# jkulhanek/viewformer

Measured on AMD Instinct MI355X. Metric: novel views/sec (encode->AR transformer->decode), 128px 6-ctx, higher is better.
Workload: dtype bf16

## Files before the change

### include/vf_hip.h

```cpp
#ifndef VF_HIP_H
#define VF_HIP_H

#include <stddef.h>
#include <stdint.h>

#ifdef __cplusplus
extern "C" {
#endif

#define VF_OK 0
#define VF_ERR_BAD_ARG (-1)
#define VF_ERR_UNSUPPORTED (-2)

int vf_abi_version(void);
size_t vf_sizeof_igemm_args(void);
size_t vf_sizeof_pack_desc(void);
const char* vf_build_arch(void);
int vf_build_flags(void);
const char* vf_build_flag_name(int i);
enum { VF_SEL_ATTN_DMA = 0,
       VF_SEL_GEMM_G256 = 1,
       VF_SEL_LN_BWD_TWO_ROWS = 2,
       VF_SEL_ATTN_Q32 = 3,
       VF_SEL_CONV_X3H_K32 = 4,
       VF_SEL_GEMM_TAIL = 5,
       VF_SEL_COUNT = 6 };
int vf_select(int which, int value);
int vf_selected(int which);

enum { VF_MODE_GEMM = 0, VF_MODE_CONV3_S1 = 1, VF_MODE_CONV3_S2PAD = 2, VF_MODE_CONV3_UP2 = 3 };
enum { VF_EPI_NONE = 0, VF_EPI_GELU_ERF = 1,
       VF_EPI_GELU_BWD = 2,
       VF_EPI_GELU_DUAL = 3 };

typedef struct vf_igemm_args {
    const float* x;
    const float* w_packed;
    const float* bias;
    const float* res;
    float* out;
    const float* pro_mean;
    const float* pro_scale;
    const float* pro_beta;
    int32_t pro_swish;
    int32_t pro_rows_per_img;
    int32_t mode;
    int32_t epilogue;
    int32_t M;
    int32_t Cin, Cout;
    int32_t Hin, Win, Hout, Wout;
    int32_t lda, ldc, ldr;
    int32_t batch;
    int64_t stride_x, stride_w, stride_out, stride_res;
    float* gn_part;
    int32_t gn_slots;
    int32_t reserved0;
    void* out_aux;
    float drop_rate;
    uint32_t drop_seed, drop_site;
    int32_t drop_row0;
} vf_igemm_args;

size_t vf_igemm_packed_floats(int K, int N, int taps);
int vf_igemm_pack_f32(const float* src, float* dst, int K, int N, int taps,
                      int64_t sk, int64_t sn, int64_t st, int batch, int64_t src_bstride, void* stream);
int vf_igemm_f32(const vf_igemm_args* args , void* stream);

int vf_conv_in_u8_f32(const uint8_t* img_u8, const float* img_f32, const float* w_oihw, const float* bias,
                      float* out, int n_img, int H, int W, int Cout, void* stream);
size_t vf_conv_in_x3h_packed_elems(int Cout);
int vf_conv_in_x3h_pack(const float* w_oihw, void* dst, int Cout, void* stream);
int vf_conv_in_x3h(const uint8_t* img_u8, const float* img_f32, const void* w_packed, const float* bias, float* out, float* gn_part,
                   int gn_slots, int n_img, int H, int W, int Cout, void* stream);

int vf_conv3_small_cout_f32(const float* x, const float* w_oihw, const float* bias, const float* pro_mean,
                            const float* pro_scale, const float* pro_beta, int pro_swish, float* out, int n_img, int H, int W,
                            int Cin, int Cout, int x_bf16, void* stream);

size_t vf_groupnorm_workspace_bytes(int n_img, int HW, int C);
int vf_groupnorm_stats_f32(const float* x, const float* gamma, int n_img, int HW, int C, int groups, float eps,
                           float* mean_c, float* scale_c, void* ws, void* stream);
int vf_groupnorm_finalize_f32(const float* part, const float* gamma, int n_img, int HW, int C, int groups, int nslots,
                              float eps, float* mean_c, float* scale_c, void* stream);
int vf_groupnorm_apply_f32(const float* x, const float* mean_c, const float* scale_c, const float* beta,
                           float* out, int n_img, int HW, int C, int swish, void* stream);

size_t vf_vq_packed_floats(int D, int Kc);
int vf_vq_pack_codebook_f32(const float* E , float* dst, int D, int Kc, void* stream);
int vf_colsumsq_f32(const float* E , float* e_sq , int D, int Kc, void* stream);
int vf_vq_argmin_f32(const float* z, const float* E_packed, const float* e_sq, int64_t M, int D, int Kc,
                     int64_t* idx, void* stream);
size_t vf_vq_filter_packed_bytes(int D, int Kc);
int vf_vq_filter_pack(const float* E , void* dst, int D, int Kc, void* stream);
int vf_vq_argmin_filtered_f32(const float* z, const void* packed, int64_t M, int D, int Kc, int64_t* idx, uint32_t* stats4,
                              void* stream);
int vf_codebook_gather_f32(const float* E , const int64_t* idx, float* out ,
                           int64_t M, int D, int Kc, void* stream);

int vf_attn_blockcausal_f32(const float* q, const float* k, const float* v, float* out,
                            int B, int H, int T, int L, int ldq, int ldk, int ldv, int ldo,
                            float scale, int skip_masked, int twin_view, void* stream);
int vf_attn_blockcausal_bf16_v2(const void* q, const void* k, const void* v, int in_bf16, void* out, int out_bf16, int B, int H, int T, int L,
                                int ldq, int ldk, int ldv, int ldo, float scale, int skip_masked, int twin_view, void* stream);
int vf_attn_blockcausal_fp8(const void* q, const void* k, const void* v, int in_bf16, void* out, int out_bf16, int B, int H, int T, int L,
                            int ldq, int ldk, int ldv, int ldo, float scale, int skip_masked, int twin_view, void* stream);
int vf_attn_blockcausal_x6(const float* q, const float* k, const float* v, float* out,
                           int B, int H, int T, int L, int ldq, int ldk, int ldv, int ldo,
                           float scale, int skip_masked, int twin_view, void* stream);
int vf_attn_prefix_bf16(const void* q, const void* k, const void* v, const void* kp, const void* vp, int in_bf16, void* out, int out_bf16,
                        int B, int H, int C, int N, int L, int dh, int ldq, int ldk, int ldv, int ldkp, int ldvp, int64_t prefix_stride,
                        int ldo, void* stream);
int vf_attn_prefix_f32eq(const float* q, const float* k, const float* v, const float* kp, const float* vp, float* out,
                         int B, int H, int C, int N, int L, int dh, int ldq, int ldk, int ldv, int ldkp, int ldvp, int64_t prefix_stride,
                         int ldo, void* stream);
int vf_attn_spatial_f32(const float* qkv, float* out, int n_img, int HW, int C, int64_t ld, int64_t ldo, float scale, void* stream);
int vf_attn_spatial_x3h(const float* qkv, float* out, int n_img, int HW, int C, int64_t ld, int64_t ldo, float scale, void* stream);
int vf_softmax_rows_f32(float* x, int64_t rows, int n, float scale, void* stream);

int vf_layernorm_f32(const float* x, const float* gamma, const float* beta, float* out,
                     int64_t rows, int d, float eps, void* stream);
int vf_layernorm_bf16out_f32(const float* x, const float* gamma, const float* beta, void* out_bf16, int64_t rows, int d, float eps,
                             void* stream);
int vf_embed_sum_f32(const int32_t* ids, const float* wte, const float* wpe, const float* add,
                     float* out, int64_t BS, int L, int d, int vocab, void* stream);
int vf_dense_small_k_gelu_f32(const float* x, const float* W, const float* b, float* out,
                              int64_t rows, int K, int N, int gelu, void* stream);
int vf_argmax_rows_f32(const float* x, int64_t rows, int n, int ld, int64_t* idx, void* stream);
int vf_lmhead_argmax_bf16(const void* h, int h_bf16, int64_t ldh, const void* w_packed, int64_t M, int K, int N, int64_t* idx,
                          float* max_logit, void* stream);
uint32_t vf_crc32c(const void* data, size_t n, uint32_t crc);
int vf_postprocess_u8(const float* x, uint8_t* out, int64_t n, void* stream);
int vf_resize_u8(const uint8_t* src, uint8_t* dst, int n_img, int Hin, int Win, int Hout, int Wout, int C, int bilinear, void* stream);
size_t vf_image_metrics_workspace_bytes(int n_img, int H, int W, int C);
int vf_image_metrics_u8(const uint8_t* a, const uint8_t* b, int n_img, int H, int W, int C, int64_t* sums, double* ssim, void* workspace,
                        void* stream);
size_t vf_camera_knn_workspace_bytes(int64_t N, int Q, int k);
int vf_camera_knn_f32(const float* db, int64_t N, const float* queries, int Q, int k, float pos_weight, int32_t* idx, float* dist,
                      void* workspace, void* stream);

size_t vf_gemm_bf16_packed_elems(int K, int N);
int vf_gemm_bf16_pack(const float* src, void* dst, int K, int N, int64_t sk, int64_t sn, int batch,
                      int64_t src_bstride, void* stream);
typedef struct vf_pack_desc {
    const float* src;
    void* dst;
    int32_t K, N;
    int64_t sk, sn;
} vf_pack_desc;
int vf_gemm_bf16_pack_multi(const vf_pack_desc* descs_device, int n, void* stream);
int vf_gemm_bf16(const vf_igemm_args* args , void* stream);
size_t vf_conv3_bf16_packed_elems(int Cin, int Cout);
int vf_conv3_bf16_pack(const float* w_oihw, void* dst, int Cin, int Cout, void* stream);
int vf_conv3_halo_bf16(const vf_igemm_args* args , void* stream);

int vf_conv3_halo_gn_slots(int Hout, int Wout);
size_t vf_conv3_x6_packed_elems(int Cin, int Cout);
int vf_conv3_x6_pack(const float* w_oihw, void* dst, int Cin, int Cout, void* stream);
int vf_conv3_halo_x6(const vf_igemm_args* args , void* stream);
size_t vf_conv3_x3h_packed_elems(int Cin, int Cout);
int vf_conv3_x3h_pack(const float* w_oihw, void* dst, int Cin, int Cout, void* stream);
int vf_conv3_halo_x3h(const vf_igemm_args* args , void* stream);
size_t vf_gemm_x3h_packed_elems(int K, int N);
int vf_gemm_x3h_pack(const float* src, void* dst, int K, int N, int64_t sk, int64_t sn, void* stream);
int vf_gemm_x3h(const vf_igemm_args* args , void* stream);
size_t vf_gemm_x6_packed_elems(int K, int N);
int vf_gemm_x6_pack(const float* src, void* dst, int K, int N, int64_t sk, int64_t sn, void* stream);
int vf_gemm_x6(const vf_igemm_args* args , void* stream);
int vf_sum_slabs_f32(const float* slabs, int nslabs, int64_t stride, int64_t n, float* dst, int accumulate, void* stream);

int vf_vq_ema_accumulate_f32(const float* z, const int64_t* idx, int64_t M, int D, int Kc, float* counts, float* embed_sum,
                             void* stream);
int vf_vq_ema_update_f32(const float* counts, const float* embed_sum, float* cluster_size_hidden, float* dw_hidden,
                         float* embeddings, int D, int Kc, float decay, float eps, float corr, void* stream);

int vf_gather_transpose_f32(const float* src, float* dst, int n_img, int Hin, int Win, int C, int Hout, int Wout, int stride, int oy,
                            int ox, int64_t ld_dst, void* stream);
size_t vf_conv3_wgrad_x6_rows(int Cin);
int vf_conv3_wgrad_x6(const float* x, const void* dy_packed, float* slabs, int n_img, int Hin, int Win, int Cin, int Hout, int Wout,
                      int Cout, int mode, int splits, void* stream);
int vf_upsample2_bwd_f32(const float* du, float* dx, int n_img, int H, int W, int C, void* stream);
size_t vf_groupnorm_bwd_workspace_bytes(int n_img, int HW, int C, int groups);
int vf_groupnorm_bwd_f32(const float* x, const float* da, const float* mean_c, const float* scale_c, const float* gamma,
                         const float* beta, float* dx, float* chan_sums, int n_img, int HW, int C, int groups, int swish,
                         int accumulate, void* ws, void* stream);
int vf_softmax_rows_bwd_f32(const float* p, float* dp, int64_t rows, int n, float scale, void* stream);
int vf_l1_loss_partials(int64_t n);
int vf_l1_loss_f32(const float* x, const float* y, float* dy, float* part, int64_t n, float grad_weight, void* stream);

int vf_lpips_scaling_f32(const float* x, float* y, int64_t npix, const float* shift3, const float* scale3, int backward, void* stream);
int vf_relu_f32(float* x, int64_t n, void* stream);
int vf_relu_bwd_f32(float* dy, const float* y, int64_t n, void* stream);
int vf_maxpool2_f32(const float* x, float* y, int n_img, int Hout, int Wout, int C, void* stream);
int vf_maxpool2_bwd_f32(const float* x, const float* dy, float* dx, int n_img, int Hout, int Wout, int C, void* stream);
int vf_lpips_head_blocks(int HW);
int vf_lpips_head_f32(const float* f0, const float* f1, const float* w, float* part, int n_img, int HW, int C, void* stream);
int vf_lpips_head_bwd_f32(const float* f0, const float* f1, const float* w, float* df1, int64_t npix, int C, float gscale,
                          int accumulate, void* stream);

int vf_attn_blockcausal_lse_f32(const float* q, const float* k, const float* v, float* out, float* lse,
                                int B, int H, int T, int L, int ldq, int ldk, int ldv, int ldo,
                                float scale, int skip_masked, int twin_view, float drop_rate, uint32_t drop_seed,
                                uint32_t drop_site, uint32_t drop_plane0, void* stream);
int vf_attn_bwd_prep_f32(const float* dout, const float* out, float* D, int B, int H, int T, int lddo, int ldo, void* stream);
int vf_attn_bwd_f32(const float* q, const float* k, const float* v, const float* dout, const float* lse, const float* D,
                    float* dq, float* dk, float* dv, int B, int H, int T, int L, int ldq, int ldk, int ldv, int lddo,
                    int lddq, int lddk, int lddv, float scale, int twin_view, float drop_rate, uint32_t drop_seed,
                    uint32_t drop_site, uint32_t drop_plane0, void* stream);
int vf_gemm_tn_bf16(const void* x_bf16, int ldx, const void* dy, int dy_is_bf16, int ldy, int M, int K, int N, int splits, float* w_slabs,
                    float* b_slabs, int64_t slab_stride, void* stream);
int vf_attn_blockcausal_bf16_lse(const void* q, const void* k, const void* v, void* out, float* lse, int B, int H, int T, int L,
                                 int ldq, int ldk, int ldv, int ldo, float scale, int twin_view, float drop_rate, uint32_t drop_seed,
                                 uint32_t drop_site, uint32_t drop_plane0, void* stream);
int vf_attn_bwd_prep_bf16(const void* dout, const void* out, float* D, int B, int H, int T, int lddo, int ldo, void* stream);
int vf_attn_bwd_bf16(const void* q, const void* k, const void* v, const void* dout, const float* lse, const float* D, void* dq, void* dk,
                     void* dv, int out_bf16 , int B, int H, int T, int L,
                     int ldq, int ldk, int ldv, int lddo, int lddq, int lddk, int lddv, float scale, int twin_view, float drop_rate,
                     uint32_t drop_seed, uint32_t drop_site, uint32_t drop_plane0, void* stream);
int vf_dropout_add_f32(const float* x, const float* res, float* out, int64_t rows, int cols, int64_t row0, float rate, uint32_t seed, uint32_t site,
                       void* stream);

int vf_transpose_f32(const float* src, float* dst, int rows, int cols, int64_t ld_src, int64_t ld_dst, int batch,
                     int64_t bs_src, int64_t bs_dst, void* stream);
int vf_transpose_bf16_f32(const void* src_bf16, float* dst, int rows, int cols, int64_t ld_src, int64_t ld_dst, int batch,
                          int64_t bs_src, int64_t bs_dst, void* stream);
size_t vf_colsum_workspace_bytes(int N);
int vf_colsum_f32(const float* x, float* out, int64_t M, int N, int64_t ld, int accumulate, void* ws, void* stream);
size_t vf_layernorm_bwd_workspace_bytes(int64_t rows, int d);
int vf_layernorm_bwd_f32(const float* dy, const float* x, const float* gamma, float* dx, float* dgamma, float* dbeta,
                         int64_t rows, int d, float eps, int accumulate, const float* res ,
                         void* dx_bf16 ,
                         float drop_rate, uint32_t drop_seed, uint32_t drop_site, int64_t drop_row0 , void* ws, void* stream);
int vf_gelu_f32(const float* u, float* f, int64_t n, void* stream);
int vf_gelu_bf16out_f32(const float* u, void* f_bf16, int64_t n, void* stream);
int vf_gelu_bwd_f32(const float* u, const float* df, float* du, int64_t n, void* stream);
int vf_gelu_bwd_bf16out_f32(const float* u, const float* df, void* du_bf16, int64_t n, void* stream);
int vf_softmax_mask_f32(float* s, int64_t batch, int T, int L, int mask_spec, float scale, void* stream);
int vf_softmax_mask_bwd_f32(const float* p, float* dp, int64_t batch, int T, int L, int mask_spec, float scale, void* stream);
int vf_softmax_ce_f32(const float* logits, const int32_t* target, const float* row_weight, float* loss, float* dlogits,
                      int64_t rows, int V, float label_smoothing, void* stream);
int vf_pose_mse_f32(const float* raw, const float* gt, const float* w_pos, const float* w_ori, const float* xyz_div, float* pos_loss,
                    float* ori_loss, float* draw, int64_t rows, int L, float position_multiplier, void* stream);
size_t vf_embed_bwd_workspace_bytes(int d, int vocab);
int vf_embed_bwd_f32(const float* dh, const int32_t* ids, float* dwte, float* dwpe, float* dadd, int64_t BS, int L, int d,
                     int vocab, void* workspace, void* stream);
int vf_dense_small_k_bwd_f32(const float* x, const float* dy, float* dW, float* db, int64_t rows, int K, int N, void* stream);
int vf_dense_small_n_f32(const float* x, const float* W, const float* b, float* out, int64_t rows, int K, int N, int64_t ldx, void* stream);
int vf_dense_small_n_wgrad_slabs(int64_t rows);
int vf_dense_small_n_wgrad_f32(const float* x, const float* dy, float* dW, float* ws, int64_t rows, int K, int N, int64_t ldx, int accumulate,
                               void* stream);
int vf_adamw_f32(float* param, const float* grad, float* m, float* v, int64_t n, float lr_decay, float lr_adam, float beta1,
                 float beta2, float eps, void* stream);
int vf_adamw_flat_f32(float* param, const float* grad, float* m, float* v, int64_t n, const int64_t* nodecay_ranges, int nranges,
                      float lr_decay, float lr_adam, float beta1, float beta2, float eps, void* stream);
typedef struct vf_adamw_pack_desc {
    int64_t offset;
    void* dst_kn;
    void* dst_nk;
    int32_t rows, cols;
    int32_t nodecay;
    int32_t reserved;
} vf_adamw_pack_desc;
size_t vf_sizeof_adamw_pack_desc(void);
int vf_adamw_pack_check(const vf_adamw_pack_desc* descs_host, int ndesc, int64_t n);
int vf_adamw_flat_pack_f32(float* param, const float* grad, float* m, float* v, int64_t n, const int64_t* nodecay_ranges, int nranges,
                           float lr_decay, float lr_adam, float beta1, float beta2, float eps, const vf_adamw_pack_desc* descs_device, int ndesc,
                           void* stream);
int vf_add_inplace_f32(float* a, const float* b, int64_t n, void* stream);
int vf_axpby_f32(float a, const float* x, float b, const float* y, float* out, int64_t n, void* stream);
int vf_clip_by_norm_f32(float* x, int64_t n, float clip, float* scratch1, void* stream);
int vf_clip_grad_norm_f32(float* x, int64_t n, float max_norm, float* scratch1, void* stream);

#ifdef __cplusplus
}
#endif
#endif
```

### viewformer_amd/_lib.py

```python
import ctypes
import os
from ctypes import c_int, c_int32, c_int64, c_float, c_void_p, c_size_t, c_char_p, POINTER

HERE = os.path.dirname(os.path.abspath(__file__))
LIB_PATH = os.environ.get('VF_HIP_LIB') or os.path.join(HERE, 'libvf_hip.so')


class VfIgemmArgs(ctypes.Structure):
    _fields_ = [
        ('x', c_void_p), ('w_packed', c_void_p), ('bias', c_void_p), ('res', c_void_p), ('out', c_void_p),
        ('pro_mean', c_void_p), ('pro_scale', c_void_p), ('pro_beta', c_void_p),
        ('pro_swish', c_int32), ('pro_rows_per_img', c_int32), ('mode', c_int32), ('epilogue', c_int32),
        ('M', c_int32), ('Cin', c_int32), ('Cout', c_int32),
        ('Hin', c_int32), ('Win', c_int32), ('Hout', c_int32), ('Wout', c_int32),
        ('lda', c_int32), ('ldc', c_int32), ('ldr', c_int32), ('batch', c_int32),
        ('stride_x', c_int64), ('stride_w', c_int64), ('stride_out', c_int64), ('stride_res', c_int64),
        ('gn_part', c_void_p), ('gn_slots', c_int32), ('reserved0', c_int32),
        ('out_aux', c_void_p),
        ('drop_rate', c_float), ('drop_seed', ctypes.c_uint32), ('drop_site', ctypes.c_uint32), ('drop_row0', c_int32),
    ]


SEL_ATTN_DMA, SEL_GEMM_G256, SEL_LN_BWD_TWO_ROWS, SEL_ATTN_Q32 = 0, 1, 2, 3
SEL_CONV_X3H_K32 = 4
SEL_GEMM_TAIL = 5
_ENV_SELECT = {'VF_ATTN_DMA': SEL_ATTN_DMA, 'VF_GEMM_G256': SEL_GEMM_G256, 'VF_LN_BWD_TWO_ROWS': SEL_LN_BWD_TWO_ROWS, 'VF_ATTN_Q32': SEL_ATTN_Q32,
               'VF_CONV_X3H_K32': SEL_CONV_X3H_K32, 'VF_GEMM_TAIL': SEL_GEMM_TAIL}

ADAMW_PACK_DESC_BYTES = 40
PACK_DESC_BYTES = 40
P = c_void_p
EXPORTS = {
    'vf_abi_version': (c_int, []),
    'vf_sizeof_igemm_args': (c_size_t, []),
    'vf_sizeof_pack_desc': (c_size_t, []),
    'vf_build_arch': (c_char_p, []),
    'vf_build_flags': (c_int, []),
    'vf_build_flag_name': (c_char_p, [c_int]),
    'vf_select': (c_int, [c_int, c_int]),
    'vf_selected': (c_int, [c_int]),
    'vf_igemm_packed_floats': (c_size_t, [c_int, c_int, c_int]),
    'vf_igemm_pack_f32': (c_int, [P, P, c_int, c_int, c_int, c_int64, c_int64, c_int64, c_int, c_int64, P]),
    'vf_igemm_f32': (c_int, [POINTER(VfIgemmArgs), P]),
    'vf_conv_in_u8_f32': (c_int, [P, P, P, P, P, c_int, c_int, c_int, c_int, P]),
    'vf_conv_in_x3h_packed_elems': (c_size_t, [c_int]),
    'vf_conv_in_x3h_pack': (c_int, [P, P, c_int, P]),
    'vf_conv_in_x3h': (c_int, [P, P, P, P, P, P, c_int, c_int, c_int, c_int, c_int, P]),
    'vf_crc32c': (ctypes.c_uint32, [P, c_size_t, ctypes.c_uint32]),
    'vf_conv3_small_cout_f32': (c_int, [P, P, P, P, P, P, c_int, P, c_int, c_int, c_int, c_int, c_int, c_int, P]),
    'vf_groupnorm_workspace_bytes': (c_size_t, [c_int, c_int, c_int]),
    'vf_groupnorm_stats_f32': (c_int, [P, P, c_int, c_int, c_int, c_int, c_float, P, P, P, P]),
    'vf_groupnorm_finalize_f32': (c_int, [P, P, c_int, c_int, c_int, c_int, c_int, c_float, P, P, P]),
    'vf_conv3_halo_gn_slots': (c_int, [c_int, c_int]),
    'vf_groupnorm_apply_f32': (c_int, [P, P, P, P, P, c_int, c_int, c_int, c_int, P]),
    'vf_vq_packed_floats': (c_size_t, [c_int, c_int]),
    'vf_vq_pack_codebook_f32': (c_int, [P, P, c_int, c_int, P]),
    'vf_colsumsq_f32': (c_int, [P, P, c_int, c_int, P]),
    'vf_vq_argmin_f32': (c_int, [P, P, P, c_int64, c_int, c_int, P, P]),
    'vf_vq_filter_packed_bytes': (c_size_t, [c_int, c_int]),
    'vf_vq_filter_pack': (c_int, [P, P, c_int, c_int, P]),
    'vf_vq_argmin_filtered_f32': (c_int, [P, P, c_int64, c_int, c_int, P, P, P]),
    'vf_gather_transpose_f32': (c_int, [P, P, c_int, c_int, c_int, c_int, c_int, c_int, c_int, c_int, c_int, c_int64, P]),
    'vf_upsample2_bwd_f32': (c_int, [P, P, c_int, c_int, c_int, c_int, P]),
    'vf_groupnorm_bwd_workspace_bytes': (c_size_t, [c_int, c_int, c_int, c_int]),
    'vf_groupnorm_bwd_f32': (c_int, [P, P, P, P, P, P, P, P, c_int, c_int, c_int, c_int, c_int, c_int, P, P]),
    'vf_softmax_rows_bwd_f32': (c_int, [P, P, c_int64, c_int, c_float, P]),
    'vf_l1_loss_partials': (c_int, [c_int64]),
    'vf_l1_loss_f32': (c_int, [P, P, P, P, c_int64, c_float, P]),
    'vf_conv3_wgrad_x6_rows': (c_size_t, [c_int]),
    'vf_conv3_wgrad_x6': (c_int, [P, P, P, c_int, c_int, c_int, c_int, c_int, c_int, c_int, c_int, c_int, P]),
    'vf_lpips_scaling_f32': (c_int, [P, P, c_int64, P, P, c_int, P]),
    'vf_relu_f32': (c_int, [P, c_int64, P]),
    'vf_relu_bwd_f32': (c_int, [P, P, c_int64, P]),
    'vf_maxpool2_f32': (c_int, [P, P, c_int, c_int, c_int, c_int, P]),
    'vf_maxpool2_bwd_f32': (c_int, [P, P, P, c_int, c_int, c_int, c_int, P]),
    'vf_lpips_head_blocks': (c_int, [c_int]),
    'vf_lpips_head_f32': (c_int, [P, P, P, P, c_int, c_int, c_int, P]),
    'vf_lpips_head_bwd_f32': (c_int, [P, P, P, P, c_int64, c_int, c_float, c_int, P]),
    'vf_vq_ema_accumulate_f32': (c_int, [P, P, c_int64, c_int, c_int, P, P, P]),
    'vf_vq_ema_update_f32': (c_int, [P, P, P, P, P, c_int, c_int, c_float, c_float, c_float, P]),
    'vf_codebook_gather_f32': (c_int, [P, P, P, c_int64, c_int, c_int, P]),
    'vf_attn_blockcausal_f32': (c_int, [P, P, P, P, c_int, c_int, c_int, c_int, c_int, c_int, c_int, c_int,
                                        c_float, c_int, c_int, P]),
    'vf_attn_blockcausal_bf16_v2': (c_int, [P, P, P, c_int, P, c_int] + [c_int] * 8 + [c_float, c_int, c_int, P]),
    'vf_attn_blockcausal_fp8': (c_int, [P, P, P, c_int, P, c_int] + [c_int] * 8 + [c_float, c_int, c_int, P]),
    'vf_attn_blockcausal_x6': (c_int, [P, P, P, P, c_int, c_int, c_int, c_int, c_int, c_int, c_int, c_int,
                                       c_float, c_int, c_int, P]),
    'vf_attn_prefix_bf16': (c_int, [P, P, P, P, P, c_int, P, c_int] + [c_int] * 11 + [c_int64, c_int, P]),
    'vf_attn_prefix_f32eq': (c_int, [P, P, P, P, P, P] + [c_int] * 11 + [c_int64, c_int, P]),
    'vf_attn_blockcausal_lse_f32': (c_int, [P, P, P, P, P, c_int, c_int, c_int, c_int, c_int, c_int, c_int, c_int,
                                            c_float, c_int, c_int, c_float, ctypes.c_uint32, ctypes.c_uint32, ctypes.c_uint32, P]),
    'vf_dropout_add_f32': (c_int, [P, P, P, c_int64, c_int, c_int64, c_float, ctypes.c_uint32, ctypes.c_uint32, P]),
    'vf_attn_bwd_prep_f32': (c_int, [P, P, P, c_int, c_int, c_int, c_int, c_int, P]),
    'vf_attn_bwd_f32': (c_int, [P, P, P, P, P, P, P, P, P, c_int, c_int, c_int, c_int, c_int, c_int, c_int, c_int, c_int,
                                c_int, c_int, c_float, c_int, c_float, ctypes.c_uint32, ctypes.c_uint32, ctypes.c_uint32, P]),
    'vf_gemm_tn_bf16': (c_int, [P, c_int, P, c_int, c_int, c_int, c_int, c_int, c_int, P, P, c_int64, P]),
    'vf_attn_blockcausal_bf16_lse': (c_int, [P, P, P, P, P, c_int, c_int, c_int, c_int, c_int, c_int, c_int, c_int, c_float, c_int,
                                             c_float, ctypes.c_uint32, ctypes.c_uint32, ctypes.c_uint32, P]),
    'vf_attn_bwd_prep_bf16': (c_int, [P, P, P, c_int, c_int, c_int, c_int, c_int, P]),
    'vf_attn_bwd_bf16': (c_int, [P, P, P, P, P, P, P, P, P, c_int, c_int, c_int, c_int, c_int, c_int, c_int, c_int, c_int, c_int, c_int, c_int,
                                 c_float, c_int, c_float, ctypes.c_uint32, ctypes.c_uint32, ctypes.c_uint32, P]),
    'vf_attn_spatial_f32': (c_int, [P, P, c_int, c_int, c_int, c_int64, c_int64, c_float, P]),
    'vf_attn_spatial_x3h': (c_int, [P, P, c_int, c_int, c_int, c_int64, c_int64, c_float, P]),
    'vf_softmax_rows_f32': (c_int, [P, c_int64, c_int, c_float, P]),
    'vf_layernorm_f32': (c_int, [P, P, P, P, c_int64, c_int, c_float, P]),
    'vf_layernorm_bf16out_f32': (c_int, [P, P, P, P, c_int64, c_int, c_float, P]),
    'vf_embed_sum_f32': (c_int, [P, P, P, P, P, c_int64, c_int, c_int, c_int, P]),
    'vf_dense_small_k_gelu_f32': (c_int, [P, P, P, P, c_int64, c_int, c_int, c_int, P]),
    'vf_lmhead_argmax_bf16': (c_int, [P, c_int, c_int64, P, c_int64, c_int, c_int, P, P, P]),
    'vf_argmax_rows_f32': (c_int, [P, c_int64, c_int, c_int, P, P]),
    'vf_postprocess_u8': (c_int, [P, P, c_int64, P]),
    'vf_resize_u8': (c_int, [P, P, c_int, c_int, c_int, c_int, c_int, c_int, c_int, P]),
    'vf_image_metrics_workspace_bytes': (c_size_t, [c_int, c_int, c_int, c_int]),
    'vf_image_metrics_u8': (c_int, [P, P, c_int, c_int, c_int, c_int, P, P, P, P]),
    'vf_camera_knn_workspace_bytes': (c_size_t, [c_int64, c_int, c_int]),
    'vf_camera_knn_f32': (c_int, [P, c_int64, P, c_int, c_int, c_float, P, P, P, P]),
    'vf_gemm_bf16_packed_elems': (c_size_t, [c_int, c_int]),
    'vf_gemm_bf16_pack': (c_int, [P, P, c_int, c_int, c_int64, c_int64, c_int, c_int64, P]),
    'vf_gemm_bf16_pack_multi': (c_int, [P, c_int, P]),
    'vf_gemm_bf16': (c_int, [POINTER(VfIgemmArgs), P]),
    'vf_conv3_bf16_packed_elems': (c_size_t, [c_int, c_int]),
    'vf_conv3_bf16_pack': (c_int, [P, P, c_int, c_int, P]),
    'vf_conv3_halo_bf16': (c_int, [POINTER(VfIgemmArgs), P]),
    'vf_conv3_x6_packed_elems': (c_size_t, [c_int, c_int]),
    'vf_conv3_x6_pack': (c_int, [P, P, c_int, c_int, P]),
    'vf_conv3_halo_x6': (c_int, [POINTER(VfIgemmArgs), P]),
    'vf_conv3_x3h_packed_elems': (c_size_t, [c_int, c_int]),
    'vf_conv3_x3h_pack': (c_int, [P, P, c_int, c_int, P]),
    'vf_conv3_halo_x3h': (c_int, [POINTER(VfIgemmArgs), P]),
    'vf_gemm_x3h_packed_elems': (c_size_t, [c_int, c_int]),
    'vf_gemm_x3h_pack': (c_int, [P, P, c_int, c_int, c_int64, c_int64, P]),
    'vf_gemm_x3h': (c_int, [POINTER(VfIgemmArgs), P]),
    'vf_gemm_x6_packed_elems': (c_size_t, [c_int, c_int]),
    'vf_gemm_x6_pack': (c_int, [P, P, c_int, c_int, c_int64, c_int64, P]),
    'vf_gemm_x6': (c_int, [POINTER(VfIgemmArgs), P]),
    'vf_sum_slabs_f32': (c_int, [P, c_int, c_int64, c_int64, P, c_int, P]),
    'vf_transpose_f32': (c_int, [P, P, c_int, c_int, c_int64, c_int64, c_int, c_int64, c_int64, P]),
    'vf_transpose_bf16_f32': (c_int, [P, P, c_int, c_int, c_int64, c_int64, c_int, c_int64, c_int64, P]),
    'vf_colsum_workspace_bytes': (c_size_t, [c_int]),
    'vf_colsum_f32': (c_int, [P, P, c_int64, c_int, c_int64, c_int, P, P]),
    'vf_layernorm_bwd_workspace_bytes': (c_size_t, [c_int64, c_int]),
    'vf_layernorm_bwd_f32': (c_int, [P, P, P, P, P, P, c_int64, c_int, c_float, c_int, P, P, c_float, ctypes.c_uint32, ctypes.c_uint32, c_int64, P, P]),
    'vf_gelu_f32': (c_int, [P, P, c_int64, P]),
    'vf_gelu_bf16out_f32': (c_int, [P, P, c_int64, P]),
    'vf_gelu_bwd_bf16out_f32': (c_int, [P, P, P, c_int64, P]),
    'vf_gelu_bwd_f32': (c_int, [P, P, P, c_int64, P]),
    'vf_softmax_mask_f32': (c_int, [P, c_int64, c_int, c_int, c_int, c_float, P]),
    'vf_softmax_mask_bwd_f32': (c_int, [P, P, c_int64, c_int, c_int, c_int, c_float, P]),
    'vf_softmax_ce_f32': (c_int, [P, P, P, P, P, c_int64, c_int, c_float, P]),
    'vf_pose_mse_f32': (c_int, [P, P, P, P, P, P, P, P, c_int64, c_int, c_float, P]),
    'vf_embed_bwd_workspace_bytes': (c_size_t, [c_int, c_int]),
    'vf_embed_bwd_f32': (c_int, [P, P, P, P, P, c_int64, c_int, c_int, c_int, P, P]),
    'vf_dense_small_k_bwd_f32': (c_int, [P, P, P, P, c_int64, c_int, c_int, P]),
    'vf_dense_small_n_f32': (c_int, [P, P, P, P, c_int64, c_int, c_int, c_int64, P]),
    'vf_dense_small_n_wgrad_slabs': (c_int, [c_int64]),
    'vf_dense_small_n_wgrad_f32': (c_int, [P, P, P, P, c_int64, c_int, c_int, c_int64, c_int, P]),
    'vf_adamw_f32': (c_int, [P, P, P, P, c_int64, c_float, c_float, c_float, c_float, c_float, P]),
    'vf_adamw_flat_f32': (c_int, [P, P, P, P, c_int64, P, c_int, c_float, c_float, c_float, c_float, c_float, P]),
    'vf_sizeof_adamw_pack_desc': (c_size_t, []),
    'vf_adamw_pack_check': (c_int, [P, c_int, c_int64]),
    'vf_adamw_flat_pack_f32': (c_int, [P, P, P, P, c_int64, P, c_int, c_float, c_float, c_float, c_float, c_float, P, c_int, P]),
    'vf_axpby_f32': (c_int, [c_float, P, c_float, P, P, c_int64, P]),
    'vf_add_inplace_f32': (c_int, [P, P, c_int64, P]),
    'vf_clip_by_norm_f32': (c_int, [P, c_int64, c_float, P, P]),
    'vf_clip_grad_norm_f32': (c_int, [P, c_int64, c_float, P, P]),
}

_lib = None


class VfError(RuntimeError):
    pass


def _bind(path):
    lib = ctypes.CDLL(path)
    for name, (res, args) in EXPORTS.items():
        fn = getattr(lib, name)
        fn.restype = res
        fn.argtypes = args
    return lib


def load_variant(path):
    return _bind(os.path.abspath(path))


class use:

    def __init__(self, handle):
        self.handle = handle

    def __enter__(self):
        global _lib
        load()
        self.prev, _lib = _lib, self.handle
        return self.handle

    def __exit__(self, *exc):
        global _lib
        _lib = self.prev
        return False


def load():
    global _lib
    if _lib is not None:
        return _lib
    if not os.path.exists(LIB_PATH):
        raise VfError(f'{LIB_PATH} not found — run `python -m viewformer_amd.build` (hipcc --offload-arch=gfx950). '
                      'There is no CPU/PyTorch fallback for the hot path.')
    lib = _bind(LIB_PATH)
    if int(lib.vf_sizeof_igemm_args()) != ctypes.sizeof(VfIgemmArgs):
        raise VfError(f'vf_igemm_args is {int(lib.vf_sizeof_igemm_args())} bytes in {LIB_PATH} and {ctypes.sizeof(VfIgemmArgs)} in '
                      'viewformer_amd/_lib.py: rebuild the library or update the mirror')
    if int(lib.vf_sizeof_pack_desc()) != PACK_DESC_BYTES:
        raise VfError(f'vf_pack_desc is {int(lib.vf_sizeof_pack_desc())} bytes in {LIB_PATH}, {PACK_DESC_BYTES} expected')
    if int(lib.vf_sizeof_adamw_pack_desc()) != ADAMW_PACK_DESC_BYTES:
        raise VfError(f'vf_adamw_pack_desc is {int(lib.vf_sizeof_adamw_pack_desc())} bytes in {LIB_PATH}, {ADAMW_PACK_DESC_BYTES} expected')
    for env, which in _ENV_SELECT.items():
        if os.environ.get(env) in ('0', '1'):
            lib.vf_select(which, int(os.environ[env]))
    _lib = lib
    return lib


def select(which, value):
    prev = load().vf_select(int(which), 1 if value else 0)
    if prev < 0:
        raise VfError(f'vf_select({which}, {value}): bad argument')
    return prev


def check(status: int, what: str):
    if status == 0:
        return
    if status < 0:
        msg = {-1: 'bad argument', -2: 'unsupported shape'}.get(status, 'error')
        raise VfError(f'{what}: {msg} ({status})')
    raise VfError(f'{what}: HIP error {status}')
```

### viewformer_amd/csrc/conv3_halo_x3h.hip

```cpp
#include <type_traits>
#include "halo_common.h"

namespace {

typedef _Float16 f16x8 __attribute__((ext_vector_type(8)));
typedef _Float16 f16x4 __attribute__((ext_vector_type(4)));

typedef unsigned u32x4_t __attribute__((ext_vector_type(4)));
__device__ __forceinline__ f16x8 wbuf_load(__amdgpu_buffer_rsrc_t r, unsigned voff, unsigned soff) {
    return __builtin_bit_cast(f16x8, __builtin_amdgcn_raw_buffer_load_b128(r, voff, soff, 0));
}

constexpr int CK = 32;
constexpr int P_LDB = 144;
constexpr int TH = 8, TW = 16;
constexpr int BN = 128;
constexpr int PLANE_BYTES = 2 * BN * 16;
constexpr int KS_BYTES = 2 * PLANE_BYTES;
constexpr int TAP_BYTES = 2 * KS_BYTES;
constexpr int TAIL_BYTES = 16;

template <bool UP2, bool PAIR = false>
struct Geo {
    static constexpr int PH = UP2 ? (TH / 2 + 2) : (TH + 2);
    static constexpr int PW = PAIR ? 20 : (UP2 ? (TW / 2 + 2) : (TW + 2));
    static constexpr int NPIX = PH * PW;
    static constexpr int SLOTS = (NPIX * 8 + 255) / 256;
    static constexpr int BUF = (NPIX + 1) * P_LDB;
};

__device__ __forceinline__ void split2(float x, _Float16& h, _Float16& l) {
    h = (_Float16)x;
    l = (_Float16)((x - (float)h) * 2048.f);
}

template <bool UP2, bool PRO, bool SWISH, bool PAIR = false>
__global__ __launch_bounds__(256, 2) void conv3_halo_x3h_kernel(vf_igemm_args p) {
    using G = Geo<UP2, PAIR>;
    extern __shared__ __attribute__((aligned(16))) unsigned char smem_h[];

    const int tid = threadIdx.x;
    const int lane = tid & 63;
    const int wave = __builtin_amdgcn_readfirstlane(tid >> 6);
    constexpr int MI = 4, NJ = 1;
    const int wave_m = 0, wave_n = wave;
    const int half = lane >> 5, l31 = lane & 31;

    const int nb = p.Cout / BN;
    const int tilesX = p.Wout / TW, tilesY = p.Hout / TH;
    int bid = (int)vf_xcd_bid();
    const int nblk = bid % nb; bid /= nb;
    int tx = 0, ty = 0, img;
    if (PAIR) { img = bid * 2; }
    else { tx = bid % tilesX; bid /= tilesX; ty = bid % tilesY; img = bid / tilesY; }
    const int n_img_total = p.M / (p.Hout * p.Wout);
    const int img1 = PAIR ? min(img + 1, n_img_total - 1) : img;
    const int pair_pix = (img1 - img) * p.Hin * p.Win;
    const int y0 = ty * TH, x0 = tx * TW;
    const int sy0 = UP2 ? (y0 / 2 - 1) : (y0 - 1);
    const int sx0 = UP2 ? (x0 / 2 - 1) : (x0 - 1);

    const float* __restrict__ X = p.x + (size_t)img * p.Hin * p.Win * p.Cin;
    const int nchunks = p.Cin / CK;
    const int last_stage = nchunks * 9 - 1;

    const int c4 = tid & 7;
    int s_off[G::SLOTS];
    unsigned ok_mask = 0, sel_mask = 0;
    const int lds0 = (tid >> 3) * P_LDB + c4 * 8;
    int lds_last = 0;
#pragma unroll
    for (int q = 0; q < G::SLOTS; ++q) {
        const int pix = (tid >> 3) + 32 * q;
        const int pixc = pix < G::NPIX ? pix : G::NPIX;
        const int pr = pixc / G::PW, pc0 = pixc - pr * G::PW;
        const int sel = PAIR ? (pc0 >= 10) : 0;
        const int pc = pc0 - 10 * sel;
        sel_mask |= (unsigned)sel << q;
        const int sy = sy0 + pr, sx = sx0 + pc;
        const bool ok = pix < G::NPIX && sy >= 0 && sy < p.Hin && sx >= 0 && sx < p.Win;
        ok_mask |= (unsigned)ok << q;
        s_off[q] = ok ? (sel * pair_pix + sy * p.Win + sx) * p.Cin + c4 * 4 : c4 * 4;
        if (q == G::SLOTS - 1) lds_last = pixc * P_LDB + c4 * 8;
    }

    f32x4 preg[G::SLOTS];
    f32x4 pmean, pscale, pbeta, pmean1, pscale1;
    const __amdgpu_buffer_rsrc_t x_rs = __builtin_amdgcn_make_buffer_rsrc(const_cast<float*>(X), 0, 0x7fffffff, 0x00020000);
    auto patch_load = [&](int chunk) {
#pragma unroll
        for (int q = 0; q < G::SLOTS; ++q)
            preg[q] = __builtin_bit_cast(f32x4, __builtin_amdgcn_raw_buffer_load_b128(x_rs, (unsigned)s_off[q] * 4u, (unsigned)(chunk * CK * 4), 0));
        if (PRO) {
            pmean = *reinterpret_cast<const f32x4*>(p.pro_mean + (size_t)img * p.Cin + chunk * CK + c4 * 4);
            pscale = *reinterpret_cast<const f32x4*>(p.pro_scale + (size_t)img * p.Cin + chunk * CK + c4 * 4);
            pbeta = *reinterpret_cast<const f32x4*>(p.pro_beta + chunk * CK + c4 * 4);
            if (PAIR) {
                pmean1 = *reinterpret_cast<const f32x4*>(p.pro_mean + (size_t)img1 * p.Cin + chunk * CK + c4 * 4);
                pscale1 = *reinterpret_cast<const f32x4*>(p.pro_scale + (size_t)img1 * p.Cin + chunk * CK + c4 * 4);
            }
        }
    };
    auto patch_store_slot = [&](int buf, int q) {
        unsigned char* dst = smem_h + buf * G::BUF + (q == G::SLOTS - 1 ? lds_last : lds0 + q * 32 * P_LDB);
        f16x4 oh, ol;
#pragma unroll
        for (int e = 0; e < 4; ++e) {
            float t = preg[q][e];
            if (PRO) {
                const float mu = (PAIR && ((sel_mask >> q) & 1u)) ? pmean1[e] : pmean[e];
                const float sc = (PAIR && ((sel_mask >> q) & 1u)) ? pscale1[e] : pscale[e];
                t = (t - mu) * sc + pbeta[e];
                if (SWISH) t = vf_swish_1ulp(t);
            }
            _Float16 h, l;
            split2(((ok_mask >> q) & 1u) ? t : 0.f, h, l);
            oh[e] = h; ol[e] = l;
        }
        *reinterpret_cast<f16x4*>(dst) = oh;
        *reinterpret_cast<f16x4*>(dst + 64) = ol;
    };

    const int trow = vf_perm_row(l31), tpx = vf_perm_px(l31);
    int a_base[MI], a_r[MI];
#pragma unroll
    for (int mi = 0; mi < MI; ++mi) {
        const int a0 = wave_m * 4 + mi * 2 + trow;
        a_r[mi] = a0;
        const int tcol = PAIR ? (tpx >> 3) * 10 + (tpx & 7) : tpx;
        a_base[mi] = (a0 * G::PW + tcol) * P_LDB + half * 16;
    }

    const unsigned char* __restrict__ Wb = reinterpret_cast<const unsigned char*>(p.w_packed) + (size_t)nblk * TAP_BYTES;
    const size_t tap_stride = (size_t)nb * TAP_BYTES;
    const int b_lane = (half * BN + wave_n * (32 * NJ) + l31) * 16;
    constexpr int BD = 2, RING = BD + 1;
    static_assert(18 % RING == 0, "ring indices must repeat per chunk");
    f16x8 bring[RING][2][NJ];
    f16x8 aring[2][MI][2];
    const int last_g = nchunks * 18 - 1;
    const __amdgpu_buffer_rsrc_t w_rs = __builtin_amdgcn_make_buffer_rsrc(const_cast<unsigned char*>(Wb), 0, 0x7fffffff, 0x00020000);
    auto b_load = [&](f16x8 (&dst)[2][NJ], int g) {
        g = min(g, last_g);
        const unsigned soff = (unsigned)((size_t)(g >> 1) * tap_stride + (g & 1) * KS_BYTES);
#pragma unroll
        for (int pl = 0; pl < 2; ++pl)
#pragma unroll
            for (int j = 0; j < NJ; ++j) dst[pl][j] = wbuf_load(w_rs, (unsigned)(b_lane + pl * PLANE_BYTES + j * 32 * 16), soff);
    };
    auto a_load = [&](f16x8 (&dst)[MI][2], const unsigned char* patch, int s) {
        const int tap = s >> 1, ks = s & 1;
        const int dy = tap / 3, dx = tap % 3;
#pragma unroll
        for (int mi = 0; mi < MI; ++mi) {
            int aoff;
            if (UP2) {
                const int pr = (a_r[mi] + dy + 1) >> 1, pc = (tpx + dx + 1) >> 1;
                aoff = (pr * G::PW + pc) * P_LDB + half * 16;
            } else {
                aoff = a_base[mi] + (dy * G::PW + dx) * P_LDB;
            }
#pragma unroll
            for (int pl = 0; pl < 2; ++pl) dst[mi][pl] = *reinterpret_cast<const f16x8*>(patch + aoff + pl * 64 + ks * 32);
        }
    };

    f32x16 acc[MI][NJ], accx[MI][NJ];
#pragma unroll
    for (int i = 0; i < MI; ++i)
#pragma unroll
        for (int j = 0; j < NJ; ++j)
#pragma unroll
            for (int r = 0; r < 16; ++r) { acc[i][j][r] = 0.f; accx[i][j][r] = 0.f; }

    patch_load(0);
#pragma unroll
    for (int g = 0; g < BD; ++g) b_load(bring[g], g);
#pragma unroll
    for (int q = 0; q < G::SLOTS; ++q) patch_store_slot(0, q);
    __syncthreads();

    for (int chunk = 0; chunk < nchunks; ++chunk) {
        const unsigned char* patch = smem_h + (chunk & 1) * G::BUF;
        b_load(bring[BD % RING], chunk * 18 + BD);
        const bool more = UP2 || PAIR || chunk + 1 < nchunks;
        if (more) patch_load(min(chunk + 1, nchunks - 1));
        a_load(aring[0], patch, 0);
#pragma unroll
        for (int s = 0; s < 18; ++s) {
            if (s > 0) b_load(bring[(s + BD) % RING], chunk * 18 + s + BD);
            if (s + 1 < 18) a_load(aring[(s + 1) & 1], patch, s + 1);
#pragma unroll
            for (int t = 0; t < 3; ++t) {
#pragma unroll
                for (int mi = 0; mi < MI; ++mi)
#pragma unroll
                    for (int j = 0; j < NJ; ++j) {
                        if (t == 0) accx[mi][j] = __builtin_amdgcn_mfma_f32_32x32x16_f16(aring[s & 1][mi][1], bring[s % RING][0][j], accx[mi][j], 0, 0, 0);
                        else if (t == 1) accx[mi][j] = __builtin_amdgcn_mfma_f32_32x32x16_f16(aring[s & 1][mi][0], bring[s % RING][1][j], accx[mi][j], 0, 0, 0);
                        else acc[mi][j] = __builtin_amdgcn_mfma_f32_32x32x16_f16(aring[s & 1][mi][0], bring[s % RING][0][j], acc[mi][j], 0, 0, 0);
                    }
            }
            __builtin_amdgcn_sched_barrier(0);
            if ((s & 1) && (s >> 1) < G::SLOTS && more) patch_store_slot((chunk + 1) & 1, s >> 1);
        }
        __syncthreads();
    }

    const float inv_s = *reinterpret_cast<const float*>(reinterpret_cast<const unsigned char*>(p.w_packed) + (size_t)nchunks * 9 * nb * TAP_BYTES);
#pragma unroll
    for (int i = 0; i < MI; ++i)
#pragma unroll
        for (int j = 0; j < NJ; ++j)
#pragma unroll
            for (int r = 0; r < 16; ++r) acc[i][j][r] = __builtin_fmaf(accx[i][j][r], 4.8828125e-4f, acc[i][j][r]) * inv_s;
    vf_halo_epilogue_t<PAIR, MI, NJ>(p, acc, img, img1, y0, x0, PAIR ? 0 : (ty * tilesX + tx) * 2, nblk, wave_m, wave_n, half, l31);
}


constexpr int S2_PH = 2 * TH + 1, S2_PW = 2 * TW + 1;
constexpr int S2_NPIX = S2_PH * S2_PW;
constexpr int S2_LDB = 80;
constexpr int S2_SLOTS = (S2_NPIX * 4 + 255) / 256;
constexpr int S2_BUF = (S2_NPIX + 1) * S2_LDB;

template <bool P8>
__global__ __launch_bounds__(256, 2) void conv3_s2_x3h_kernel(vf_igemm_args p) {
    extern __shared__ __attribute__((aligned(16))) unsigned char smem_h[];
    constexpr int PW = P8 ? 34 : S2_PW;
    constexpr int NPIX = S2_PH * PW;
    constexpr int SLOTS = (NPIX * 4 + 255) / 256;
    const int tid = threadIdx.x;
    const int lane = tid & 63;
    const int wave = __builtin_amdgcn_readfirstlane(tid >> 6);
    constexpr int MI = 4, NJ = 1;
    const int wave_m = 0, wave_n = wave;
    const int half = lane >> 5, l31 = lane & 31;

    const int nb = p.Cout / BN;
    const int tilesX = P8 ? 1 : p.Wout / TW, tilesY = P8 ? 1 : p.Hout / TH;
    int bid = (int)vf_xcd_bid();
    const int nblk = bid % nb; bid /= nb;
    const int tx = bid % tilesX; bid /= tilesX;
    const int ty = bid % tilesY;
    const int img = P8 ? (bid / tilesY) * 2 : bid / tilesY;
    const int n_img_total = p.M / (p.Hout * p.Wout);
    const int img1 = P8 ? min(img + 1, n_img_total - 1) : img;
    const int pair_pix = (img1 - img) * p.Hin * p.Win;
    const int y0 = ty * TH, x0 = tx * TW;
    const float* __restrict__ X = p.x + (size_t)img * p.Hin * p.Win * p.Cin;
    const int nchunks = p.Cin / 16;

    const int c4 = tid & 3;
    int s_off[SLOTS], s_lds[SLOTS];
    bool s_ok[SLOTS];
#pragma unroll
    for (int q = 0; q < SLOTS; ++q) {
        const int pix = (tid >> 2) + 64 * q;
        const int pixc = pix < NPIX ? pix : 0;
        const int pr = pixc / PW, pc0 = pixc - pr * PW;
        const int sel = P8 ? (pc0 >= 17) : 0;
        const int pc = pc0 - 17 * sel;
        const int sy = 2 * y0 + pr, sx = 2 * x0 + pc;
        const bool ok = pix < NPIX && sy < p.Hin && sx < p.Win;
        s_ok[q] = ok;
        s_off[q] = ok ? (sel * pair_pix + sy * p.Win + sx) * p.Cin + c4 * 4 : c4 * 4;
        int slot;
        if (P8) slot = pr * PW + ((pc & 1) ? 18 + sel * 8 + (pc >> 1) : sel * 9 + (pc >> 1));
        else slot = pr * PW + (pc & 1) * (TW + 1) + (pc >> 1);
        s_lds[q] = (pix < NPIX ? slot : NPIX) * S2_LDB + c4 * 8;
    }
    f32x4 preg[SLOTS];
    auto patch_load = [&](int chunk) {
#pragma unroll
        for (int q = 0; q < SLOTS; ++q) preg[q] = *reinterpret_cast<const f32x4*>(X + chunk * 16 + s_off[q]);
    };
    auto patch_park = [&]() {
#pragma unroll
        for (int q = 0; q < SLOTS; ++q) {
            f16x4 oh, ol;
#pragma unroll
            for (int e = 0; e < 4; ++e) {
                _Float16 h, l;
                split2(s_ok[q] ? preg[q][e] : 0.f, h, l);
                oh[e] = h; ol[e] = l;
            }
            unsigned char* dst = smem_h + s_lds[q];
            *reinterpret_cast<f16x4*>(dst) = oh;
            *reinterpret_cast<f16x4*>(dst + 32) = ol;
        }
    };

    const int trow = vf_perm_row(l31), tpx = vf_perm_px(l31);
    int a_base[MI], a_base_o[MI];
#pragma unroll
    for (int mi = 0; mi < MI; ++mi) {
        const int row2 = 2 * (wave_m * 4 + mi * 2 + trow) * PW;
        if (P8) {
            a_base[mi] = (row2 + (tpx >> 3) * 9 + (tpx & 7)) * S2_LDB + half * 16;
            a_base_o[mi] = (row2 + 18 + (tpx >> 3) * 8 + (tpx & 7)) * S2_LDB + half * 16;
        } else {
            a_base[mi] = (row2 + tpx) * S2_LDB + half * 16;
            a_base_o[mi] = a_base[mi] + (TW + 1) * S2_LDB;
        }
    }

    const unsigned char* __restrict__ Wb = reinterpret_cast<const unsigned char*>(p.w_packed) + (size_t)nblk * TAP_BYTES;
    const size_t tap_stride = (size_t)nb * TAP_BYTES;
    const int b_lane = (half * BN + wave_n * (32 * NJ) + l31) * 16;
    const int last_g = nchunks * 9 - 1;
    constexpr int S2_BR = 3;
    f16x8 bring[S2_BR][2][NJ];
    f16x8 aring[2][MI][2];
    auto b_load = [&](f16x8 (&dst)[2][NJ], int g) {
        g = min(g, last_g);
        const int c = g / 9, tap = g - c * 9;
        const unsigned char* src = Wb + (size_t)((c >> 1) * 9 + tap) * tap_stride + (c & 1) * KS_BYTES + b_lane;
#pragma unroll
        for (int pl = 0; pl < 2; ++pl)
#pragma unroll
            for (int j = 0; j < NJ; ++j) dst[pl][j] = *reinterpret_cast<const f16x8*>(src + pl * PLANE_BYTES + j * 32 * 16);
    };
    auto a_load = [&](f16x8 (&dst)[MI][2], int tap) {
        const int dy = tap / 3, dx = tap % 3;
        const int off = (dy * PW + (dx >> 1)) * S2_LDB;
#pragma unroll
        for (int mi = 0; mi < MI; ++mi)
#pragma unroll
            for (int pl = 0; pl < 2; ++pl) dst[mi][pl] = *reinterpret_cast<const f16x8*>(smem_h + ((dx & 1) ? a_base_o[mi] : a_base[mi]) + off + pl * 32);
    };

    f32x16 acc[MI][NJ], accx[MI][NJ];
#pragma unroll
    for (int i = 0; i < MI; ++i)
#pragma unroll
        for (int j = 0; j < NJ; ++j)
#pragma unroll
            for (int r = 0; r < 16; ++r) { acc[i][j][r] = 0.f; accx[i][j][r] = 0.f; }

    patch_load(0);
    b_load(bring[0], 0);
    if (S2_BR > 2) b_load(bring[1], 1);
    for (int chunk = 0; chunk < nchunks; ++chunk) {
        __syncthreads();
        patch_park();
        b_load(bring[(S2_BR - 1) % S2_BR], chunk * 9 + S2_BR - 1);
        if (chunk + 1 < nchunks) patch_load(min(chunk + 1, nchunks - 1));
        __syncthreads();
        a_load(aring[0], 0);
#pragma unroll
        for (int t = 0; t < 9; ++t) {
            if (t > 0) b_load(bring[(t + S2_BR - 1) % S2_BR], chunk * 9 + t + S2_BR - 1);
            if (t + 1 < 9) a_load(aring[(t + 1) & 1], t + 1);
#pragma unroll
            for (int mi = 0; mi < MI; ++mi)
#pragma unroll
                for (int j = 0; j < NJ; ++j) accx[mi][j] = __builtin_amdgcn_mfma_f32_32x32x16_f16(aring[t & 1][mi][1], bring[t % S2_BR][0][j], accx[mi][j], 0, 0, 0);
#pragma unroll
            for (int mi = 0; mi < MI; ++mi)
#pragma unroll
                for (int j = 0; j < NJ; ++j) accx[mi][j] = __builtin_amdgcn_mfma_f32_32x32x16_f16(aring[t & 1][mi][0], bring[t % S2_BR][1][j], accx[mi][j], 0, 0, 0);
#pragma unroll
            for (int mi = 0; mi < MI; ++mi)
#pragma unroll
                for (int j = 0; j < NJ; ++j) acc[mi][j] = __builtin_amdgcn_mfma_f32_32x32x16_f16(aring[t & 1][mi][0], bring[t % S2_BR][0][j], acc[mi][j], 0, 0, 0);
            __builtin_amdgcn_sched_barrier(0);
        }
    }
    const float inv_s = *reinterpret_cast<const float*>(reinterpret_cast<const unsigned char*>(p.w_packed) + (size_t)(p.Cin / CK) * 9 * nb * TAP_BYTES);
#pragma unroll
    for (int i = 0; i < MI; ++i)
#pragma unroll
        for (int j = 0; j < NJ; ++j)
#pragma unroll
            for (int r = 0; r < 16; ++r) acc[i][j][r] = __builtin_fmaf(accx[i][j][r], 4.8828125e-4f, acc[i][j][r]) * inv_s;
    vf_halo_epilogue_t<P8, MI, NJ, false>(p, acc, img, img1, y0, x0, P8 ? 0 : (ty * tilesX + tx) * 2, nblk, wave_m, wave_n, half, l31);
}



typedef float f32x4v __attribute__((ext_vector_type(4)));

template <bool PRO, bool SWISH>
__global__ __launch_bounds__(256, 2) void conv3_halo_x3h16_kernel(vf_igemm_args p) {
    using G = Geo<false, false>;
    extern __shared__ __attribute__((aligned(16))) unsigned char smem_h[];
    constexpr int RT = 8, CT = 2;

    const int tid = threadIdx.x;
    const int lane = tid & 63;
    const int wave = __builtin_amdgcn_readfirstlane(tid >> 6);
    const int lm = lane & 15, lg = lane >> 4;

    const int nb = p.Cout / BN;
    const int tilesX = p.Wout / TW, tilesY = p.Hout / TH;
    int bid = (int)vf_xcd_bid();
    const int nblk = bid % nb; bid /= nb;
    const int tx = bid % tilesX; bid /= tilesX;
    const int ty = bid % tilesY;
    const int img = bid / tilesY;
    const int y0 = ty * TH, x0 = tx * TW;
    const int sy0 = y0 - 1, sx0 = x0 - 1;
    const float* __restrict__ X = p.x + (size_t)img * p.Hin * p.Win * p.Cin;
    const int nchunks = p.Cin / CK;

    const int c4 = tid & 7;
    unsigned ok_mask = 0;
    const int c4s = (((c4 >> 1) & 1) * 2 + (c4 >> 2)) * 16 + (c4 & 1) * 8;
    const int lds0 = (tid >> 3) * P_LDB + c4s;
    int lds_last = 0;
    int pix0 = tid >> 3;
    auto slot_src = [&](int q, bool& ok) {
        const int pix = pix0 + 32 * q;
        const int pixc = min(pix, (int)G::NPIX);
        const int pr = (pixc * 3641) >> 16, pc = pixc - pr * G::PW;
        const int sy = sy0 + pr, sx = sx0 + pc;
        ok = (pix < G::NPIX) & ((unsigned)sy < (unsigned)p.Hin) & ((unsigned)sx < (unsigned)p.Win);
        const int off = (sy * p.Win + sx) * p.Cin;
        return (ok ? off : 0) + c4 * 4;
    };
#pragma unroll
    for (int q = 0; q < G::SLOTS; ++q) {
        bool ok;
        (void)slot_src(q, ok);
        ok_mask |= (unsigned)ok << q;
        if (q == G::SLOTS - 1) { const int pix = (tid >> 3) + 32 * q; lds_last = (pix < G::NPIX ? pix : G::NPIX) * P_LDB + c4s; }
    }
    unsigned char* __restrict__ raw_l = smem_h + 2 * G::BUF;
    const __amdgpu_buffer_rsrc_t x_rs = __builtin_amdgcn_make_buffer_rsrc(const_cast<float*>(X), 0, 0x7fffffff, 0x00020000);
    float* __restrict__ pro_l = reinterpret_cast<float*>(smem_h + 2 * G::BUF + G::SLOTS * 4096 - 1024);
    if (PRO) {
        for (int i = tid; i < p.Cin; i += 256) {
            pro_l[i] = p.pro_mean[(size_t)img * p.Cin + i];
            pro_l[p.Cin + i] = p.pro_scale[(size_t)img * p.Cin + i];
            pro_l[2 * p.Cin + i] = p.pro_beta[i];
        }
    }
    int pro_chunk = 0;
    auto patch_load = [&](int chunk) {
        asm volatile("" : "+v"(pix0));
#pragma unroll
        for (int q = 0; q < G::SLOTS; ++q) {
            bool ok;
            const int off = slot_src(q, ok);
            if (q == G::SLOTS - 1 && wave == 3) continue;
            __builtin_amdgcn_raw_ptr_buffer_load_lds(x_rs, (__attribute__((address_space(3))) void*)(raw_l + q * 4096 + wave * 1024), 16, (unsigned)off * 4u,
                                                     (unsigned)(chunk * CK * 4), 0, 0);
        }
        pro_chunk = chunk;
    };
    auto patch_store_slot = [&](int buf, int q) {
        unsigned char* dst = smem_h + buf * G::BUF + (q == G::SLOTS - 1 ? lds_last : lds0 + q * 32 * P_LDB);
        f32x4 pmean, pscale, pbeta;
        if (PRO) {
            const float* pl = pro_l + pro_chunk * CK + c4 * 4;
            pmean = *reinterpret_cast<const f32x4*>(pl);
            pscale = *reinterpret_cast<const f32x4*>(pl + p.Cin);
            pbeta = *reinterpret_cast<const f32x4*>(pl + 2 * p.Cin);
        }
        f32x4 raw = {0.f, 0.f, 0.f, 0.f};
        if (!(q == G::SLOTS - 1 && wave == 3)) raw = *reinterpret_cast<const f32x4*>(raw_l + q * 4096 + tid * 16);
        f16x4 oh, ol;
#pragma unroll
        for (int e = 0; e < 4; ++e) {
            float t = raw[e];
            if (PRO) {
                t = (t - pmean[e]) * pscale[e] + pbeta[e];
                if (SWISH) t = vf_swish_1ulp(t);
            }
            _Float16 h, l;
            split2(((ok_mask >> q) & 1u) ? t : 0.f, h, l);
            oh[e] = h; ol[e] = l;
        }
        *reinterpret_cast<f16x4*>(dst) = oh;
        *reinterpret_cast<f16x4*>(dst + 64) = ol;
    };

    const int lpix = lm < 4 ? 2 * lm : lm < 12 ? 2 * lm - 7 : 2 * lm - 16;
    const int a_lane = lpix * P_LDB + (((lg & 1) * 2) + (lg >> 1)) * 16;
    const unsigned char* __restrict__ Wb = reinterpret_cast<const unsigned char*>(p.w_packed) + (size_t)nblk * TAP_BYTES;
    const size_t tap_stride = (size_t)nb * TAP_BYTES;
    const int b_lane = ((lg >> 1) * 4 + (lg & 1)) * (BN * 16) + (wave * 32 + lm) * 16;
    const int last_tap = nchunks * 9 - 1;
    const __amdgpu_buffer_rsrc_t w_rs = __builtin_amdgcn_make_buffer_rsrc(const_cast<unsigned char*>(Wb), 0, 0x7fffffff, 0x00020000);
    f16x8 bring[2][4];
    constexpr int AR = 3;
    f16x8 aring[AR][2];
    auto b_load = [&](f16x8 (&dst)[4], int gtap) {
        const unsigned soff = (unsigned)((size_t)min(gtap, last_tap) * tap_stride);
#pragma unroll
        for (int pl = 0; pl < 2; ++pl)
#pragma unroll
            for (int ct = 0; ct < CT; ++ct) dst[pl * 2 + ct] = wbuf_load(w_rs, (unsigned)(b_lane + pl * PLANE_BYTES + ct * 256), soff);
    };
    auto a_load = [&](f16x8 (&dst)[2], const unsigned char* patch, int step) {
        const int tap = step >> 3, rt = step & 7;
        const int off = ((rt + tap / 3) * G::PW + tap % 3) * P_LDB;
        dst[0] = *reinterpret_cast<const f16x8*>(patch + a_lane + off);
        dst[1] = *reinterpret_cast<const f16x8*>(patch + a_lane + off + 64);
    };

    f32x4v acc[RT][CT], accx[RT][CT];
#pragma unroll
    for (int i = 0; i < RT; ++i)
#pragma unroll
        for (int j = 0; j < CT; ++j)
#pragma unroll
            for (int r = 0; r < 4; ++r) { acc[i][j][r] = 0.f; accx[i][j][r] = 0.f; }

    patch_load(0);
    b_load(bring[0], 0);
    asm volatile("s_waitcnt vmcnt(0)" ::: "memory");
    if (PRO) __syncthreads();
#pragma unroll
    for (int q = 0; q < G::SLOTS; ++q) patch_store_slot(0, q);
    __syncthreads();

    auto chunk_body = [&](int chunk, auto parity) {
        constexpr int P0 = decltype(parity)::value;
        const unsigned char* patch = smem_h + P0 * G::BUF;
        const bool more = chunk + 1 < nchunks;
        b_load(bring[(P0 + 1) & 1], chunk * 9 + 1);
        unsigned pad[G::SLOTS];
#pragma unroll
        for (int q = 0; q < G::SLOTS; ++q) pad[q] = __builtin_amdgcn_raw_buffer_load_b32(w_rs, (unsigned)(q * 256), 0u, 0);
        if (more) patch_load(chunk + 1);
#pragma unroll
        for (int i = 0; i < AR - 1; ++i) a_load(aring[i], patch, i);
#pragma unroll
        for (int t = 0; t < 9; ++t) {
            if (t > 0) b_load(bring[(P0 + t + 1) & 1], chunk * 9 + t + 1);
            if (t == 2) {
#pragma unroll
                for (int q = 0; q < G::SLOTS; ++q) asm volatile("" :: "v"(pad[q]));
            }
            const f16x8 (&B)[4] = bring[(P0 + t) & 1];
#pragma unroll
            for (int rt = 0; rt < RT; ++rt) {
                const int step = t * 8 + rt;
                if (step + AR - 1 < 72) a_load(aring[(step + AR - 1) % AR], patch, step + AR - 1);
                const f16x8 ah = aring[step % AR][0], al = aring[step % AR][1];
                accx[rt][0] = __builtin_amdgcn_mfma_f32_16x16x32_f16(al, B[0], accx[rt][0], 0, 0, 0);
                accx[rt][1] = __builtin_amdgcn_mfma_f32_16x16x32_f16(al, B[1], accx[rt][1], 0, 0, 0);
                acc[rt][0] = __builtin_amdgcn_mfma_f32_16x16x32_f16(ah, B[0], acc[rt][0], 0, 0, 0);
                acc[rt][1] = __builtin_amdgcn_mfma_f32_16x16x32_f16(ah, B[1], acc[rt][1], 0, 0, 0);
                accx[rt][0] = __builtin_amdgcn_mfma_f32_16x16x32_f16(ah, B[2], accx[rt][0], 0, 0, 0);
                accx[rt][1] = __builtin_amdgcn_mfma_f32_16x16x32_f16(ah, B[3], accx[rt][1], 0, 0, 0);
                __builtin_amdgcn_sched_barrier(0);
            }
            if (t >= 1 && t <= G::SLOTS && more) {
                if (t == 1) asm volatile("s_waitcnt vmcnt(8)" ::: "memory");
                patch_store_slot((P0 + 1) & 1, t - 1);
            }
        }
        __syncthreads();
    };
    for (int chunk = 0; chunk < nchunks; chunk += 2) {
        chunk_body(chunk, std::integral_constant<int, 0>{});
        chunk_body(chunk + 1, std::integral_constant<int, 1>{});
    }

    const float inv_s = *reinterpret_cast<const float*>(reinterpret_cast<const unsigned char*>(p.w_packed) + (size_t)nchunks * 9 * nb * TAP_BYTES);
    const __amdgpu_buffer_rsrc_t o_rs = __builtin_amdgcn_make_buffer_rsrc(p.out + (size_t)img * p.Hout * p.Wout * p.ldc, 0, 0x7fffffff, 0x00020000);
    const __amdgpu_buffer_rsrc_t r_rs = __builtin_amdgcn_make_buffer_rsrc(const_cast<float*>(p.res ? p.res + (size_t)img * p.Hout * p.Wout * p.ldr : p.out), 0, 0x7fffffff, 0x00020000);
    const bool Res = p.res != nullptr;
    const bool stats = p.gn_part != nullptr;
    const int cg = p.Cout >> 5;
    const int tile_slot = (ty * tilesX + tx) * 2;
    const int pbase = lg == 0 ? 0 : lg == 1 ? 1 : lg == 2 ? 9 : 8;
    auto spix = [&](int rt, int r) { return (y0 + rt) * p.Wout + x0 + 2 * r; };
#pragma unroll
    for (int rt = 0; rt < RT; ++rt)
#pragma unroll
        for (int ct = 0; ct < CT; ++ct)
#pragma unroll
            for (int r = 0; r < 4; ++r) acc[rt][ct][r] = __builtin_fmaf(accx[rt][ct][r], 4.8828125e-4f, acc[rt][ct][r]) * inv_s;
    __builtin_amdgcn_sched_barrier(0);
    float rr[CT][RT][4];
    if (Res) {
#pragma unroll
        for (int ct = 0; ct < CT; ++ct) {
            const int n = nblk * BN + wave * 32 + ct * 16 + lm;
            const unsigned rv = (unsigned)(pbase * p.ldr + n) * 4u;
#pragma unroll
            for (int rt = 0; rt < RT; ++rt)
#pragma unroll
                for (int r = 0; r < 4; ++r)
                    rr[ct][rt][r] = __builtin_bit_cast(float, __builtin_amdgcn_raw_buffer_load_b32(r_rs, rv, (unsigned)(spix(rt, r) * p.ldr) * 4u, 0));
        }
    }
#pragma unroll
    for (int ct = 0; ct < CT; ++ct) {
        const int n = nblk * BN + wave * 32 + ct * 16 + lm;
        const float bias = p.bias ? p.bias[n] : 0.f;
        const unsigned ov = (unsigned)(pbase * p.ldc + n) * 4u;
#pragma unroll
        for (int sl = 0; sl < 2; ++sl) {
            float s32 = 0.f, q32 = 0.f;
#pragma unroll
            for (int k = 0; k < 4; ++k) {
                const int rt = sl * 4 + k;
#pragma unroll
                for (int r = 0; r < 4; ++r) {
                    float v = acc[rt][ct][r] + bias;
                    if (Res) v += rr[ct][rt][r];
                    __builtin_amdgcn_raw_buffer_store_b32(__builtin_bit_cast(unsigned, v), o_rs, ov, (unsigned)(spix(rt, r) * p.ldc) * 4u, 0);
                    s32 += v;
                    q32 = __builtin_fmaf(v, v, q32);
                }
            }
            if (stats) {
                vf_gn_acc_t s = (vf_gn_acc_t)s32, q = (vf_gn_acc_t)q32;
                for (int o = 1; o < cg; o <<= 1) { s += __shfl_xor(s, o, 64); q += __shfl_xor(q, o, 64); }
                s += __shfl_xor(s, 16, 64); q += __shfl_xor(q, 16, 64);
                s += __shfl_xor(s, 32, 64); q += __shfl_xor(q, 32, 64);
                if (lg == 0 && (lm & (cg - 1)) == 0) {
                    float* dst = p.gn_part + ((((size_t)img * p.gn_slots) + tile_slot + sl) * 32 + n / cg) * 2;
                    dst[0] = (float)s;
                    dst[1] = (float)q;
                }
            }
        }
    }
}

__global__ void absmax_kernel(const float* __restrict__ w, long long n, unsigned* __restrict__ out) {
    float m = 0.f;
    for (long long i = blockIdx.x * (long long)blockDim.x + threadIdx.x; i < n; i += (long long)gridDim.x * blockDim.x) m = fmaxf(m, fabsf(w[i]));
    vf_block_max_atomic(m, out);
}

__global__ void pack_conv_x3h_kernel(const float* __restrict__ w, _Float16* __restrict__ dst, int Cin, int Cout, int nb, int nchunks,
                                     unsigned char* __restrict__ tail) {
    const float amax = __uint_as_float(*reinterpret_cast<const unsigned*>(tail + 4));
    const int ex = amax > 0.f ? ilogbf(amax) : 13;
    const float S = ldexpf(1.f, 13 - ex);
    if (blockIdx.x == 0 && threadIdx.x == 0) *reinterpret_cast<float*>(tail) = ldexpf(1.f, ex - 13);
    const long long total = (long long)nchunks * 9 * nb * CK * BN;
    for (long long idx = blockIdx.x * (long long)blockDim.x + threadIdx.x; idx < total; idx += (long long)gridDim.x * blockDim.x) {
        const int e = (int)(idx & 7);
        long long t = idx >> 3;
        const int nl = (int)(t % BN); t /= BN;
        const int half = (int)(t & 1);
        const int ks = (int)((t >> 1) & 1);
        t >>= 2;
        const int nblk = (int)(t % nb); t /= nb;
        const int tap = (int)(t % 9);
        const int chunk = (int)(t / 9);
        const int c = chunk * CK + ks * 16 + half * 8 + e;
        const int n = nblk * BN + nl;
        float v = 0.f;
        if (c < Cin && n < Cout) v = w[((size_t)n * Cin + c) * 9 + tap] * S;
        _Float16 h, l;
        split2(v, h, l);
        const size_t base = ((((size_t)(chunk * 9 + tap) * nb + nblk) * 2 + ks) * 2) * (2 * BN * 8) + ((size_t)half * BN + nl) * 8 + e;
        dst[base] = h;
        dst[base + 2 * BN * 8] = l;
    }
}

template <bool UP2, bool PRO, bool SWISH, bool PAIR>
int launch_halo(const vf_igemm_args& a, hipStream_t stream) {
    using G = Geo<UP2, PAIR>;
    const size_t smem = (size_t)2 * G::BUF;
    const int n_img = a.M / (a.Hout * a.Wout);
    const long long blocks = PAIR ? (long long)((n_img + 1) / 2) * (a.Cout / BN)
                                  : (long long)n_img * (a.Hout / TH) * (a.Wout / TW) * (a.Cout / BN);
    hipLaunchKernelGGL((conv3_halo_x3h_kernel<UP2, PRO, SWISH, PAIR>), dim3((unsigned)blocks), dim3(256), smem, stream, a);
    return vf_last_status();
}

static inline size_t vf_x3h16_lds_bytes(int pro_cin) { return (size_t)2 * Geo<false, false>::BUF + Geo<false, false>::SLOTS * 4096 - 1024 + (size_t)3 * pro_cin * 4; }

template <bool PRO, bool SWISH>
int launch_halo16(const vf_igemm_args& a, hipStream_t stream) {
    using G = Geo<false, false>;
    const int n_img = a.M / (a.Hout * a.Wout);
    const long long blocks = (long long)n_img * (a.Hout / TH) * (a.Wout / TW) * (a.Cout / BN);
    const size_t smem = vf_x3h16_lds_bytes(PRO ? a.Cin : 0);
    static unsigned long long attr_devs = 0;
    if (vf_attr_needed(&attr_devs)) {
        const hipError_t e = hipFuncSetAttribute(reinterpret_cast<const void*>(conv3_halo_x3h16_kernel<PRO, SWISH>), hipFuncAttributeMaxDynamicSharedMemorySize, 80 * 1024);
        if (e != hipSuccess) return (int)e;
        vf_attr_done(&attr_devs);
    }
    hipLaunchKernelGGL((conv3_halo_x3h16_kernel<PRO, SWISH>), dim3((unsigned)blocks), dim3(256), smem, stream, a);
    return vf_last_status();
}

template <bool UP2, bool PAIR>
int dispatch_pro(const vf_igemm_args& a, hipStream_t s) {
    if (!UP2 && !PAIR && (a.Cin / CK) % 2 == 0 && (!a.gn_part || a.Cout / 32 <= 16) && vf_x3h16_lds_bytes(a.pro_mean ? a.Cin : 0) <= 80 * 1024 &&
        vf_selected(VF_SEL_CONV_X3H_K32)) {
        if (!a.pro_mean) return launch_halo16<false, false>(a, s);
        return a.pro_swish ? launch_halo16<true, true>(a, s) : launch_halo16<true, false>(a, s);
    }
    if (!a.pro_mean) return launch_halo<UP2, false, false, PAIR>(a, s);
    return a.pro_swish ? launch_halo<UP2, true, true, PAIR>(a, s) : launch_halo<UP2, true, false, PAIR>(a, s);
}

}

extern "C" {

size_t vf_conv3_x3h_packed_elems(int Cin, int Cout) {
    if (Cin <= 0 || Cout <= 0) return 0;
    return (size_t)((Cin + CK - 1) / CK) * 9 * ((Cout + BN - 1) / BN) * CK * BN * 2 + TAIL_BYTES / 2;
}

int vf_conv3_x3h_pack(const float* w_oihw, void* dst, int Cin, int Cout, void* stream) {
    if (!w_oihw || !dst || Cin <= 0 || Cout <= 0) return VF_ERR_BAD_ARG;
    const int nb = (Cout + BN - 1) / BN, nchunks = (Cin + CK - 1) / CK;
    const long long total = (long long)nchunks * 9 * nb * CK * BN;
    unsigned char* tail = reinterpret_cast<unsigned char*>(dst) + (size_t)total * 2 * sizeof(_Float16);
    hipStream_t s = (hipStream_t)stream;
    if (hipMemsetAsync(tail, 0, TAIL_BYTES, s) != hipSuccess) return vf_last_status();
    const long long nw = (long long)Cout * Cin * 9;
    hipLaunchKernelGGL(absmax_kernel, dim3((unsigned)((nw + 2047) / 2048 > 128 ? 128 : (nw + 2047) / 2048)), dim3(256), 0, s, w_oihw, nw,
                       reinterpret_cast<unsigned*>(tail + 4));
    const int blocks = (int)((total + 255) / 256 > 4096 ? 4096 : (total + 255) / 256);
    hipLaunchKernelGGL(pack_conv_x3h_kernel, dim3(blocks), dim3(256), 0, s, w_oihw, (_Float16*)dst, Cin, Cout, nb, nchunks, tail);
    return vf_last_status();
}

int vf_conv3_halo_x3h(const vf_igemm_args* args, void* stream) {
    if (!args) return VF_ERR_BAD_ARG;
    const vf_igemm_args& a = *args;
    if (!a.x || !a.w_packed || !a.out || a.M <= 0) return VF_ERR_BAD_ARG;
    if (a.drop_rate != 0.f || a.out_aux) return VF_ERR_UNSUPPORTED;
    if (a.mode == VF_MODE_CONV3_S2PAD) {
        const bool p8 = a.Hout == 8 && a.Wout == 8;
        if (a.Cout % BN != 0 || a.Cin % CK != 0 || (!p8 && (a.Hout % TH != 0 || a.Wout % TW != 0)) || a.pro_mean) return VF_ERR_UNSUPPORTED;
        if (a.Hin != a.Hout * 2 || a.Win != a.Wout * 2 || a.M % (a.Hout * a.Wout) != 0) return VF_ERR_BAD_ARG;
        if (a.batch > 1 || a.epilogue != VF_EPI_NONE || a.ldc < a.Cout || (a.res && a.ldr < a.Cout)) return VF_ERR_BAD_ARG;
        if ((long long)a.Hin * a.Win * a.Cin >= (1ll << 31)) return VF_ERR_UNSUPPORTED;
        if (int st = vf_halo_gn_check(a)) return st;
        if (p8) {
            const long long blocks = (long long)((a.M / 64 + 1) / 2) * (a.Cout / BN);
            hipLaunchKernelGGL(conv3_s2_x3h_kernel<true>, dim3((unsigned)blocks), dim3(256), (size_t)(S2_PH * 34 + 1) * S2_LDB, (hipStream_t)stream, a);
            return vf_last_status();
        }
        const long long blocks = (long long)(a.M / (a.Hout * a.Wout)) * (a.Hout / TH) * (a.Wout / TW) * (a.Cout / BN);
        hipLaunchKernelGGL(conv3_s2_x3h_kernel<false>, dim3((unsigned)blocks), dim3(256), (size_t)S2_BUF, (hipStream_t)stream, a);
        return vf_last_status();
    }
    if (a.mode != VF_MODE_CONV3_S1 && a.mode != VF_MODE_CONV3_UP2) return VF_ERR_UNSUPPORTED;
    const bool pair = a.mode == VF_MODE_CONV3_S1 && a.Hout == 8 && a.Wout == 8;
    if (a.Cout % BN != 0 || a.Cin % CK != 0 || (!pair && (a.Hout % TH != 0 || a.Wout % TW != 0))) return VF_ERR_UNSUPPORTED;
    if (a.Hin <= 0 || a.Win <= 0 || a.M % (a.Hout * a.Wout) != 0) return VF_ERR_BAD_ARG;
    if (a.mode == VF_MODE_CONV3_S1 && (a.Hout != a.Hin || a.Wout != a.Win)) return VF_ERR_BAD_ARG;
    if (a.mode == VF_MODE_CONV3_UP2 && (a.Hout != a.Hin * 2 || a.Wout != a.Win * 2)) return VF_ERR_BAD_ARG;
    if (a.batch > 1 || a.epilogue != VF_EPI_NONE || a.ldc < a.Cout || (a.res && a.ldr < a.Cout)) return VF_ERR_BAD_ARG;
    if ((a.pro_mean || a.pro_scale || a.pro_beta) && !(a.pro_mean && a.pro_scale && a.pro_beta)) return VF_ERR_BAD_ARG;
    if ((long long)a.Hin * a.Win * a.Cin >= (1ll << 31)) return VF_ERR_UNSUPPORTED;
    if (int st = vf_halo_gn_check(a)) return st;
    hipStream_t s = (hipStream_t)stream;
    if (pair) return dispatch_pro<false, true>(a, s);
    return (a.mode == VF_MODE_CONV3_UP2) ? dispatch_pro<true, false>(a, s) : dispatch_pro<false, false>(a, s);
}

}
```

### viewformer_amd/csrc/conv_in_x3h.hip

```cpp
#include "halo_common.h"

namespace {

typedef _Float16 f16x8 __attribute__((ext_vector_type(8)));
typedef _Float16 f16x4 __attribute__((ext_vector_type(4)));

constexpr int TH = 8, TW = 16, BN = 128;
constexpr int PW = TW + 2, PH = TH + 2, NPIX = PH * PW;
constexpr int P_LDB = 16;
constexpr int PLANE_BYTES = 2 * BN * 16;
constexpr int KS_BYTES = 2 * PLANE_BYTES;
constexpr int BLK_BYTES = 3 * KS_BYTES;
constexpr int TAIL_BYTES = 16;

__device__ __forceinline__ void split2(float x, _Float16& h, _Float16& l) {
    h = (_Float16)x;
    l = (_Float16)((x - (float)h) * 2048.f);
}

template <bool U8>
__global__ __launch_bounds__(256) void conv_in_x3h_kernel(vf_igemm_args p, const unsigned char* __restrict__ img_u8) {
    __shared__ __attribute__((aligned(16))) unsigned char patch[NPIX * P_LDB];
    const int tid = threadIdx.x;
    const int lane = tid & 63;
    const int wave = __builtin_amdgcn_readfirstlane(tid >> 6);
    const int wave_m = wave >> 1, wave_n = wave & 1;
    const int half = lane >> 5, l31 = lane & 31;

    const int nb = p.Cout / BN;
    const int tilesX = p.Wout / TW, tilesY = p.Hout / TH;
    int bid = (int)vf_xcd_bid();
    const int nblk = bid % nb; bid /= nb;
    const int tx = bid % tilesX; bid /= tilesX;
    const int ty = bid % tilesY;
    const int img = bid / tilesY;
    const int y0 = ty * TH, x0 = tx * TW;

    if (tid < NPIX) {
        const int pr = tid / PW, pc = tid - pr * PW;
        const int sy = y0 - 1 + pr, sx = x0 - 1 + pc;
        const bool ok = sy >= 0 && sy < p.Hout && sx >= 0 && sx < p.Wout;
        const size_t px = ((size_t)img * p.Hout + (ok ? sy : 0)) * p.Wout + (ok ? sx : 0);
        f16x4 oh, ol;
#pragma unroll
        for (int c = 0; c < 3; ++c) {
            float v;
            if (U8) v = ((float)img_u8[px * 3 + c] * (1.0f / 255.0f)) * 2.0f - 1.0f;
            else v = p.x[px * 3 + c];
            _Float16 h, l;
            split2(ok ? v : 0.f, h, l);
            oh[c] = h; ol[c] = l;
        }
        oh[3] = (_Float16)0.f; ol[3] = (_Float16)0.f;
        *reinterpret_cast<f16x4*>(patch + tid * P_LDB) = oh;
        *reinterpret_cast<f16x4*>(patch + tid * P_LDB + 8) = ol;
    }

    const unsigned char* __restrict__ Wb = reinterpret_cast<const unsigned char*>(p.w_packed) + (size_t)nblk * BLK_BYTES +
                                           (half * BN + wave_n * 64 + l31) * 16;
    f16x8 b[3][2][2];
#pragma unroll
    for (int ks = 0; ks < 3; ++ks)
#pragma unroll
        for (int pl = 0; pl < 2; ++pl)
#pragma unroll
            for (int j = 0; j < 2; ++j) b[ks][pl][j] = *reinterpret_cast<const f16x8*>(Wb + ks * KS_BYTES + pl * PLANE_BYTES + j * 32 * 16);

    f32x16 acc[2][2], accx[2][2];
#pragma unroll
    for (int i = 0; i < 2; ++i)
#pragma unroll
        for (int j = 0; j < 2; ++j)
#pragma unroll
            for (int r = 0; r < 16; ++r) { acc[i][j][r] = 0.f; accx[i][j][r] = 0.f; }
    __syncthreads();

    const int trow = vf_perm_row(l31), tpx = vf_perm_px(l31);
#pragma unroll
    for (int ks = 0; ks < 3; ++ks) {
        const int g = ks * 2 + half;
        f16x8 a[2][2];
#pragma unroll
        for (int mi = 0; mi < 2; ++mi) {
            const int a0 = wave_m * 4 + mi * 2 + trow;
#pragma unroll
            for (int pl = 0; pl < 2; ++pl) {
                f16x4 lo = {(_Float16)0.f, (_Float16)0.f, (_Float16)0.f, (_Float16)0.f}, hi = lo;
                const int t0 = 2 * g, t1 = 2 * g + 1;
                if (t0 < 9) lo = *reinterpret_cast<const f16x4*>(patch + ((a0 + t0 / 3) * PW + tpx + t0 % 3) * P_LDB + pl * 8);
                if (t1 < 9) hi = *reinterpret_cast<const f16x4*>(patch + ((a0 + t1 / 3) * PW + tpx + t1 % 3) * P_LDB + pl * 8);
                a[mi][pl] = f16x8{lo[0], lo[1], lo[2], lo[3], hi[0], hi[1], hi[2], hi[3]};
            }
        }
#pragma unroll
        for (int mi = 0; mi < 2; ++mi)
#pragma unroll
            for (int j = 0; j < 2; ++j) accx[mi][j] = __builtin_amdgcn_mfma_f32_32x32x16_f16(a[mi][1], b[ks][0][j], accx[mi][j], 0, 0, 0);
#pragma unroll
        for (int mi = 0; mi < 2; ++mi)
#pragma unroll
            for (int j = 0; j < 2; ++j) accx[mi][j] = __builtin_amdgcn_mfma_f32_32x32x16_f16(a[mi][0], b[ks][1][j], accx[mi][j], 0, 0, 0);
#pragma unroll
        for (int mi = 0; mi < 2; ++mi)
#pragma unroll
            for (int j = 0; j < 2; ++j) acc[mi][j] = __builtin_amdgcn_mfma_f32_32x32x16_f16(a[mi][0], b[ks][0][j], acc[mi][j], 0, 0, 0);
    }

    const float inv_s = *reinterpret_cast<const float*>(reinterpret_cast<const unsigned char*>(p.w_packed) + (size_t)nb * BLK_BYTES);
#pragma unroll
    for (int i = 0; i < 2; ++i)
#pragma unroll
        for (int j = 0; j < 2; ++j)
#pragma unroll
            for (int r = 0; r < 16; ++r) acc[i][j][r] = __builtin_fmaf(accx[i][j][r], 4.8828125e-4f, acc[i][j][r]) * inv_s;
    vf_halo_epilogue<false>(p, acc, img, img, y0, x0, (ty * tilesX + tx) * 2, nblk, wave_m, wave_n, half, l31);
}

__global__ void absmax27_kernel(const float* __restrict__ w, long long n, unsigned* __restrict__ out) {
    float m = 0.f;
    for (long long i = blockIdx.x * (long long)blockDim.x + threadIdx.x; i < n; i += (long long)gridDim.x * blockDim.x) m = fmaxf(m, fabsf(w[i]));
    vf_block_max_atomic(m, out);
}

__global__ void pack_conv_in_x3h_kernel(const float* __restrict__ w, _Float16* __restrict__ dst, int Cout, int nb,
                                        unsigned char* __restrict__ tail) {
    const float amax = __uint_as_float(*reinterpret_cast<const unsigned*>(tail + 4));
    const int ex = amax > 0.f ? ilogbf(amax) : 13;
    const float S = ldexpf(1.f, 13 - ex);
    if (blockIdx.x == 0 && threadIdx.x == 0) *reinterpret_cast<float*>(tail) = ldexpf(1.f, ex - 13);
    const int total = nb * 3 * 2 * BN * 8;
    for (int idx = blockIdx.x * blockDim.x + threadIdx.x; idx < total; idx += gridDim.x * blockDim.x) {
        const int e = idx & 7;
        int t = idx >> 3;
        const int nl = t % BN; t /= BN;
        const int half = t & 1;
        const int ks = (t >> 1) % 3;
        const int nblk = (t >> 1) / 3;
        const int k = (ks * 2 + half) * 8 + e;
        const int tap = k >> 2, c = k & 3;
        const int n = nblk * BN + nl;
        float v = 0.f;
        if (tap < 9 && c < 3 && n < Cout) v = w[((size_t)n * 3 + c) * 9 + tap] * S;
        _Float16 h, l;
        split2(v, h, l);
        const size_t base = (((size_t)nblk * 3 + ks) * 2) * (2 * BN * 8) + ((size_t)half * BN + nl) * 8 + e;
        dst[base] = h;
        dst[base + 2 * BN * 8] = l;
    }
}

}

extern "C" {

size_t vf_conv_in_x3h_packed_elems(int Cout) {
    if (Cout <= 0 || Cout % BN) return 0;
    return (size_t)(Cout / BN) * 3 * 2 * 2 * BN * 8 + TAIL_BYTES / 2;
}

int vf_conv_in_x3h_pack(const float* w_oihw, void* dst, int Cout, void* stream) {
    if (!w_oihw || !dst || Cout <= 0) return VF_ERR_BAD_ARG;
    if (Cout % BN) return VF_ERR_UNSUPPORTED;
    const int nb = Cout / BN;
    unsigned char* tail = reinterpret_cast<unsigned char*>(dst) + (size_t)nb * BLK_BYTES;
    hipStream_t s = (hipStream_t)stream;
    if (hipMemsetAsync(tail, 0, TAIL_BYTES, s) != hipSuccess) return vf_last_status();
    hipLaunchKernelGGL(absmax27_kernel, dim3(16), dim3(256), 0, s, w_oihw, (long long)Cout * 27, reinterpret_cast<unsigned*>(tail + 4));
    hipLaunchKernelGGL(pack_conv_in_x3h_kernel, dim3(48), dim3(256), 0, s, w_oihw, (_Float16*)dst, Cout, nb, tail);
    return vf_last_status();
}

int vf_conv_in_x3h(const uint8_t* img_u8, const float* img_f32, const void* w_packed, const float* bias, float* out, float* gn_part,
                   int gn_slots, int n_img, int H, int W, int Cout, void* stream) {
    if ((!img_u8 && !img_f32) || !w_packed || !out || n_img <= 0 || H <= 0 || W <= 0 || Cout <= 0) return VF_ERR_BAD_ARG;
    if (H % TH || W % TW || Cout % BN) return VF_ERR_UNSUPPORTED;
    vf_igemm_args a = {};
    a.x = img_f32;
    a.w_packed = reinterpret_cast<const float*>(w_packed);
    a.bias = bias;
    a.out = out;
    a.mode = VF_MODE_CONV3_S1;
    a.M = n_img * H * W; a.Cin = 3; a.Cout = Cout;
    a.Hin = a.Hout = H; a.Win = a.Wout = W;
    a.lda = 3; a.ldc = Cout; a.ldr = Cout;
    a.batch = 1;
    a.gn_part = gn_part;
    a.gn_slots = gn_slots;
    if (int st = vf_halo_gn_check(a)) return st;
    const long long blocks = (long long)n_img * (H / TH) * (W / TW) * (Cout / BN);
    if (img_u8) hipLaunchKernelGGL(conv_in_x3h_kernel<true>, dim3((unsigned)blocks), dim3(256), 0, (hipStream_t)stream, a, img_u8);
    else hipLaunchKernelGGL(conv_in_x3h_kernel<false>, dim3((unsigned)blocks), dim3(256), 0, (hipStream_t)stream, a, img_u8);
    return vf_last_status();
}

}
```

### viewformer_amd/ops.py

```python
import ctypes
import os

import torch

from . import _lib
from ._lib import VfIgemmArgs, check

MODE_GEMM, MODE_CONV3_S1, MODE_CONV3_S2PAD, MODE_CONV3_UP2 = 0, 1, 2, 3
EPI_NONE, EPI_GELU, EPI_GELU_BWD, EPI_GELU_DUAL = 0, 1, 2, 3


def _stream():
    return ctypes.c_void_p(torch.cuda.current_stream().cuda_stream)


def _p(t):
    if t is None:
        return None
    return ctypes.c_void_p(t.data_ptr())


def _chk(t, dtype=torch.float32, name='tensor'):
    if not t.is_cuda:
        raise _lib.VfError(f'{name} must live on the GPU (no CPU fallback for the hot path)')
    if t.dtype != dtype:
        raise TypeError(f'{name} must be {dtype}, got {t.dtype}')
    return t


def _f32(t, name='tensor'):
    return _chk(t, torch.float32, name)


def packed_floats(K, N, taps=1):
    return int(_lib.load().vf_igemm_packed_floats(K, N, taps))


def pack(src, K, N, taps, sk, sn, st, batch=1, src_bstride=0, out=None):
    lib = _lib.load()
    n = packed_floats(K, N, taps)
    if out is None:
        out = torch.empty(batch * n, dtype=torch.float32, device=src.device)
    check(lib.vf_igemm_pack_f32(_p(_f32(src)), _p(out), K, N, taps, sk, sn, st, batch, src_bstride, _stream()),
          'vf_igemm_pack_f32')
    return out


def pack_conv_oihw(w):
    w = _f32(w).contiguous()
    cout, cin, kh, kw = w.shape
    taps = kh * kw
    return pack(w, cin, cout, taps, sk=taps, sn=cin * taps, st=1)


def pack_dense_kn(w):
    w = _f32(w).contiguous()
    k, n = w.shape
    return pack(w, k, n, 1, sk=n, sn=1, st=0)


def pack_dense_nk(w, n_rows=None):
    w = _f32(w).contiguous()
    n, k = w.shape
    n = n if n_rows is None else n_rows
    return pack(w, k, n, 1, sk=1, sn=k, st=0)


def pack_dense_kn_bf16(w):
    lib = _lib.load()
    w = _f32(w).contiguous()
    k, n = w.shape
    out = torch.empty(int(lib.vf_gemm_bf16_packed_elems(k, n)), dtype=torch.bfloat16, device=w.device)
    check(lib.vf_gemm_bf16_pack(_p(w), _p(out), k, n, n, 1, 1, 0, _stream()), 'vf_gemm_bf16_pack')
    return out


def pack_bf16_multi(items):
    import numpy as np
    lib = _lib.load()
    dt = np.dtype([('src', '<u8'), ('dst', '<u8'), ('K', '<i4'), ('N', '<i4'), ('sk', '<i8'), ('sn', '<i8')])
    assert dt.itemsize == _lib.PACK_DESC_BYTES
    a = np.zeros(len(items), dtype=dt)
    for i, (w, tr, out) in enumerate(items):
        _f32(w); _chk(out, torch.bfloat16)
        assert w.is_contiguous() and w.dim() == 2
        r, c = w.shape
        K, N, sk, sn = (c, r, 1, c) if tr else (r, c, c, 1)
        assert out.numel() >= int(lib.vf_gemm_bf16_packed_elems(K, N))
        a[i] = (w.data_ptr(), out.data_ptr(), K, N, sk, sn)
    descs = torch.from_numpy(a.view(np.uint8).copy()).to(items[0][0].device)
    n = len(items)

    def run(first=0, count=None):
        count = n - first if count is None else count
        if count <= 0:
            return
        assert 0 <= first and first + count <= n
        check(lib.vf_gemm_bf16_pack_multi(descs.data_ptr() + first * _lib.PACK_DESC_BYTES, count, _stream()), 'vf_gemm_bf16_pack_multi')
    run()
    return run


def pack_dense_nk_bf16(w, n_rows=None):
    lib = _lib.load()
    w = _f32(w).contiguous()
    n, k = w.shape
    n = n if n_rows is None else n_rows
    out = torch.empty(int(lib.vf_gemm_bf16_packed_elems(k, n)), dtype=torch.bfloat16, device=w.device)
    check(lib.vf_gemm_bf16_pack(_p(w), _p(out), k, n, 1, k, 1, 0, _stream()), 'vf_gemm_bf16_pack')
    return out


def pack_conv3_bf16(w_oihw):
    lib = _lib.load()
    w = _f32(w_oihw).contiguous()
    cout, cin = w.shape[:2]
    out = torch.empty(int(lib.vf_conv3_bf16_packed_elems(cin, cout)), dtype=torch.bfloat16, device=w.device)
    check(lib.vf_conv3_bf16_pack(_p(w), _p(out), cin, cout, _stream()), 'vf_conv3_bf16_pack')
    return out


def pack_conv3_x6(w_oihw):
    lib = _lib.load()
    w = _f32(w_oihw).contiguous()
    cout, cin = w.shape[:2]
    out = torch.empty(int(lib.vf_conv3_x6_packed_elems(cin, cout)), dtype=torch.bfloat16, device=w.device)
    check(lib.vf_conv3_x6_pack(_p(w), _p(out), cin, cout, _stream()), 'vf_conv3_x6_pack')
    return out


def pack_conv3_x3h(w_oihw):
    lib = _lib.load()
    w = _f32(w_oihw).contiguous()
    cout, cin = w.shape[:2]
    out = torch.empty(int(lib.vf_conv3_x3h_packed_elems(cin, cout)), dtype=torch.float16, device=w.device)
    check(lib.vf_conv3_x3h_pack(_p(w), _p(out), cin, cout, _stream()), 'vf_conv3_x3h_pack')
    return out


def conv3_x3h_supported(mode, Cin, Cout, Hout, Wout):
    if mode == MODE_CONV3_S2PAD and Hout == 8 and Wout == 8 and Cin % 32 == 0 and Cout % 128 == 0:
        return True
    return conv3_x6_supported(mode, Cin, Cout, Hout, Wout)


def pack_dense_kn_x6(w):
    lib = _lib.load()
    w = _f32(w).contiguous()
    k, n = w.shape
    out = torch.empty(int(lib.vf_gemm_x6_packed_elems(k, n)), dtype=torch.bfloat16, device=w.device)
    check(lib.vf_gemm_x6_pack(_p(w), _p(out), k, n, n, 1, _stream()), 'vf_gemm_x6_pack')
    return out


def pack_dense_nk_x6(w, n_rows=None):
    lib = _lib.load()
    w = _f32(w).contiguous()
    n, k = w.shape
    n = n if n_rows is None else n_rows
    out = torch.empty(int(lib.vf_gemm_x6_packed_elems(k, n)), dtype=torch.bfloat16, device=w.device)
    check(lib.vf_gemm_x6_pack(_p(w), _p(out), k, n, 1, k, _stream()), 'vf_gemm_x6_pack')
    return out


def pack_dense_kn_x3h(w):
    lib = _lib.load()
    w = _f32(w).contiguous()
    k, n = w.shape
    out = torch.empty(int(lib.vf_gemm_x3h_packed_elems(k, n)), dtype=torch.float16, device=w.device)
    check(lib.vf_gemm_x3h_pack(_p(w), _p(out), k, n, n, 1, _stream()), 'vf_gemm_x3h_pack')
    return out


def pack_dense_nk_x3h(w, n_rows=None):
    lib = _lib.load()
    w = _f32(w).contiguous()
    n, k = w.shape
    n = n if n_rows is None else n_rows
    out = torch.empty(int(lib.vf_gemm_x3h_packed_elems(k, n)), dtype=torch.float16, device=w.device)
    check(lib.vf_gemm_x3h_pack(_p(w), _p(out), k, n, 1, k, _stream()), 'vf_gemm_x3h_pack')
    return out


def gemm_x6_splitk(x, w_packed, M, Cin, Cout, dst, splits, lda=None, accumulate=True):
    lib = _lib.load()
    slabs = torch.empty((splits, M, Cout), dtype=torch.float32, device=x.device)
    igemm(x, w_packed, M, Cin, Cout, slabs, lda=lda, x6=True, split_k=splits, stride_out=M * Cout)
    check(lib.vf_sum_slabs_f32(_p(slabs), splits, M * Cout, M * Cout, _p(_f32(dst)), 1 if accumulate else 0, _stream()),
          'vf_sum_slabs_f32')
    return dst


def conv3_x6_supported(mode, Cin, Cout, Hout, Wout):
    if mode not in (MODE_CONV3_S1, MODE_CONV3_UP2, MODE_CONV3_S2PAD) or Cin % 32 or Cout % 128:
        return False
    return (Hout % 8 == 0 and Wout % 16 == 0) or (mode == MODE_CONV3_S1 and Hout == 8 and Wout == 8)


def gemm_bf16_splitk(x, w_packed, M, Cin, Cout, dst, splits, lda=None, accumulate=True):
    lib = _lib.load()
    ks = Cin // splits
    if splits < 1 or ks * splits != Cin or ks % 64:
        raise _lib.VfError(f'gemm_bf16_splitk: Cin = {Cin} does not split into {splits} ranges of whole 64-deep chunks')
    nb = (Cout + 127) // 128
    slabs = torch.empty((splits, M, Cout), dtype=torch.float32, device=x.device)
    igemm(x, w_packed, M, ks, Cout, slabs, lda=Cin if lda is None else lda, bf16=True, batch=splits, stride_x=ks,
          stride_w=(ks // 64) * nb * 64 * 128, stride_out=M * Cout)
    check(lib.vf_sum_slabs_f32(_p(slabs), splits, M * Cout, M * Cout, _p(_f32(dst)), 1 if accumulate else 0, _stream()),
          'vf_sum_slabs_f32')
    return dst


TN_TARGET_WORKGROUPS = 256
TN_TARGET_WORKGROUPS_BESIDE = 192


def gemm_tn_bf16_supported(x, M, K, N):
    return x.dtype == torch.bfloat16 and gemm_tn_bf16_shape_ok(M, K, N)


def gemm_tn_bf16_shape_ok(M, K, N):
    return K % 256 == 0 and N % 256 == 0 and M % 64 == 0 and M * K * 2 < 2 ** 31


def gemm_g256_shape_ok(M, K, N):
    return N % 256 == 0 and K % 64 == 0 and M >= 256 and M * K * 2 < 2 ** 31 and K * N * 2 < 2 ** 31


def gemm_drop_supported(M, K, N, row0=0):
    return gemm_g256_shape_ok(M, K, N) and row0 % 4 == 0 and ((M + row0 + 3) // 4) * N < 2 ** 32


def gemm_tn_bf16(x16, dy, M, K, N, dw, db=None, accumulate=True, beside_another_gemm=False):
    lib = _lib.load()
    _chk(x16, torch.bfloat16, 'x16')
    tiles = (K // 256) * (N // 256)
    target = TN_TARGET_WORKGROUPS_BESIDE if beside_another_gemm else TN_TARGET_WORKGROUPS
    splits = max(1, min(M // 64, target // tiles if tiles <= target else 1))
    rec = K * N + (N if db is not None else 0)
    ws = torch.empty((splits, rec), dtype=torch.float32, device=dy.device)
    y16 = dy.dtype == torch.bfloat16
    check(lib.vf_gemm_tn_bf16(_p(x16), x16.stride(0), _p(dy if y16 else _f32(dy)), 1 if y16 else 0, dy.stride(0), M, K, N, splits, _p(ws),
                              ws.data_ptr() + K * N * 4 if db is not None else None, rec, _stream()), 'vf_gemm_tn_bf16')
    acc = 1 if accumulate else 0
    _f32(dw)
    if db is not None and _f32(db).data_ptr() == dw.data_ptr() + K * N * 4 and dw.is_contiguous():
        check(lib.vf_sum_slabs_f32(_p(ws), splits, rec, rec, _p(dw), acc, _stream()), 'vf_sum_slabs_f32')
    else:
        check(lib.vf_sum_slabs_f32(_p(ws), splits, rec, K * N, _p(dw), acc, _stream()), 'vf_sum_slabs_f32')
        if db is not None:
            check(lib.vf_sum_slabs_f32(ws.data_ptr() + K * N * 4, splits, rec, N, _p(db), acc, _stream()), 'vf_sum_slabs_f32')
    return dw


def igemm(x, w_packed, M, Cin, Cout, out, bias=None, res=None, mode=MODE_GEMM, epilogue=EPI_NONE,
          pro=None, pro_swish=False, pro_rows_per_img=0, Hin=0, Win=0, Hout=0, Wout=0,
          lda=None, ldc=None, ldr=None, batch=1, stride_x=0, stride_w=0, stride_out=0, stride_res=0, bf16=False, x6=False, gn_part=None, split_k=0,
          x3h=False, a16=False, o16=False, out_aux=None, res16=False, drop=None, gelu_grad=False):
    lib = _lib.load()
    if not 0 <= M < 2 ** 31 or max(Cin, Cout, Hin, Win, Hout, Wout, batch) >= 2 ** 31:
        raise _lib.VfError(f'igemm: M = {M} rows do not fit the int32 fields of vf_igemm_args — split the launch '
                           '(VQGAN(max_images_per_call=...))')
    a = VfIgemmArgs()
    a.x = x.data_ptr()
    a.w_packed = w_packed.data_ptr()
    a.bias = bias.data_ptr() if bias is not None else None
    a.res = res.data_ptr() if res is not None else None
    a.out = out.data_ptr()
    if out_aux is not None:
        _chk(out_aux, torch.bfloat16, 'out_aux')
        if out_aux.shape != out.shape or not (out_aux.is_contiguous() or out_aux.stride() == out.stride()):
            raise _lib.VfError('out_aux must have the shape and row stride of out')
        a.out_aux = out_aux.data_ptr()
    if pro is not None:
        mean_c, scale_c, beta = pro
        a.pro_mean, a.pro_scale, a.pro_beta = mean_c.data_ptr(), scale_c.data_ptr(), beta.data_ptr()
    a.pro_swish = 1 if pro_swish else 0
    a.pro_rows_per_img = pro_rows_per_img
    a.mode, a.epilogue = mode, epilogue
    a.M, a.Cin, a.Cout = M, Cin, Cout
    a.Hin, a.Win, a.Hout, a.Wout = Hin, Win, Hout, Wout
    a.lda = Cin if lda is None else lda
    a.ldc = Cout if ldc is None else ldc
    a.ldr = (Cout if ldr is None else ldr)
    a.batch = batch
    a.stride_x, a.stride_w, a.stride_out, a.stride_res = stride_x, stride_w, stride_out, stride_res
    a.reserved0 = split_k
    if gn_part is not None:
        a.gn_part = _f32(gn_part).data_ptr()
        a.gn_slots = gn_part.shape[1]
    conv16 = False
    if a16 or o16:
        if not bf16 or mode not in (MODE_GEMM, MODE_CONV3_S1, MODE_CONV3_UP2):
            raise _lib.VfError('a16 / o16 need bf16=True and a GEMM or 3x3 stride-1 / upsample convolution')
        _chk(x, torch.bfloat16 if a16 else torch.float32, 'x')
        _chk(out, torch.bfloat16 if o16 else torch.float32, 'out')
        a.reserved0 = (1 if a16 else 0) | (2 if o16 else 0)
        conv16 = mode != MODE_GEMM
        if conv16:
            if a16 and not o16:
                raise _lib.VfError('the bf16 convolution takes bf16 activations in only together with bf16 out')
            if res is not None:
                _chk(res, torch.bfloat16 if o16 else torch.float32, 'res')
    if drop is not None and drop[0]:
        if not (bf16 and a16 and not o16 and mode == MODE_GEMM and epilogue == EPI_NONE):
            raise _lib.VfError('drop needs the bf16 GEMM with bf16 x, fp32 out and no epilogue function')
        a.drop_rate, a.drop_seed, a.drop_site = float(drop[0]), int(drop[1]) & 0xFFFFFFFF, int(drop[2])
        a.drop_row0 = int(drop[3]) if len(drop) > 3 else 0
    if res16:
        if not (a16 and o16 and epilogue == EPI_GELU_BWD and res is not None):
            raise _lib.VfError('res16 is the bf16 pre-activation of EPI_GELU_BWD (bf16 in, bf16 out)')
        _chk(res, torch.bfloat16, 'res')
        a.reserved0 |= 4
    if gelu_grad:
        if not ((epilogue == EPI_GELU_DUAL and a16 and o16) or (epilogue == EPI_GELU_BWD and res16)):
            raise _lib.VfError('gelu_grad: EPI_GELU_DUAL with bf16 in / out, or EPI_GELU_BWD with res16')
        a.reserved0 |= 8
    for t in ((None if a16 else x), (None if o16 else out), bias, (None if (res16 or conv16) else res)):
        if t is not None:
            _f32(t)
    if x3h:
        _chk(w_packed, torch.float16, 'w_packed')
        if mode == MODE_GEMM:
            check(lib.vf_gemm_x3h(ctypes.byref(a), _stream()), 'vf_gemm_x3h')
        else:
            check(lib.vf_conv3_halo_x3h(ctypes.byref(a), _stream()), 'vf_conv3_halo_x3h')
        return out
    if x6:
        _chk(w_packed, torch.bfloat16, 'w_packed')
        if mode == MODE_GEMM:
            check(lib.vf_gemm_x6(ctypes.byref(a), _stream()), 'vf_gemm_x6')
        else:
            check(lib.vf_conv3_halo_x6(ctypes.byref(a), _stream()), 'vf_conv3_halo_x6')
        return out
    if bf16:
        _chk(w_packed, torch.bfloat16, 'w_packed')
        if mode == MODE_GEMM:
            check(lib.vf_gemm_bf16(ctypes.byref(a), _stream()), 'vf_gemm_bf16')
        else:
            check(lib.vf_conv3_halo_bf16(ctypes.byref(a), _stream()), 'vf_conv3_halo_bf16')
        return out
    _f32(w_packed)
    check(lib.vf_igemm_f32(ctypes.byref(a), _stream()), 'vf_igemm_f32')
    return out


def conv3_small_cout_supported(mode, Cin, Cout, H, W):
    return mode == MODE_CONV3_S1 and 1 <= Cout <= 4 and Cin % 32 == 0 and Cin // 32 * 4608 <= 96 * 1024 and H % 8 == 0 and W % 32 == 0


def conv3_small_cout(x, w_oihw, bias, n_img, H, W, Cin, Cout, pro=None, pro_swish=True, out=None):
    lib = _lib.load()
    if out is None:
        out = torch.empty((n_img * H * W, Cout), dtype=torch.float32, device=x.device)
    pm, ps, pb = (None, None, None) if pro is None else pro
    x16 = x.dtype == torch.bfloat16
    check(lib.vf_conv3_small_cout_f32(_p(x if x16 else _f32(x)), _p(_f32(w_oihw)), _p(_f32(bias)) if bias is not None else None,
                                      _p(pm) if pm is not None else None, _p(ps) if ps is not None else None,
                                      _p(pb) if pb is not None else None, 1 if pro_swish else 0, _p(out), n_img, H, W, Cin, Cout,
                                      1 if x16 else 0, _stream()), 'vf_conv3_small_cout_f32')
    return out


def pack_conv_in_x3h(w_oihw):
    lib = _lib.load()
    w = _f32(w_oihw).contiguous()
    out = torch.empty(int(lib.vf_conv_in_x3h_packed_elems(w.shape[0])), dtype=torch.float16, device=w.device)
    check(lib.vf_conv_in_x3h_pack(_p(w), _p(out), w.shape[0], _stream()), 'vf_conv_in_x3h_pack')
    return out


def conv_in_x3h_supported(H, W, Cout):
    return H % 8 == 0 and W % 16 == 0 and Cout % 128 == 0


def conv_in(img, w_oihw, bias, n_img, H, W, Cout, out=None, wp3h=None, gn_part=None):
    lib = _lib.load()
    if out is None:
        out = torch.empty((n_img, H, W, Cout), dtype=torch.float32, device=img.device)
    if img.dtype == torch.uint8:
        u8, f32 = _p(_chk(img, torch.uint8)), None
    else:
        u8, f32 = None, _p(_f32(img))
    if wp3h is not None:
        _chk(wp3h, torch.float16, 'wp3h')
        check(lib.vf_conv_in_x3h(u8, f32, _p(wp3h), _p(bias), _p(out), _p(gn_part) if gn_part is not None else None,
                                 gn_part.shape[1] if gn_part is not None else 0, n_img, H, W, Cout, _stream()), 'vf_conv_in_x3h')
        return out
    if gn_part is not None:
        raise _lib.VfError('conv_in: fused GroupNorm statistics need the x3h form (wp3h)')
    check(lib.vf_conv_in_u8_f32(u8, f32, _p(_f32(w_oihw)), _p(bias), _p(out), n_img, H, W, Cout, _stream()),
          'vf_conv_in_u8_f32')
    return out


def groupnorm_stats(x, gamma, n_img, HW, C, groups=32, eps=1e-6):
    lib = _lib.load()
    mean_c = torch.empty((n_img, C), dtype=torch.float32, device=x.device)
    scale_c = torch.empty((n_img, C), dtype=torch.float32, device=x.device)
    ws = torch.empty(int(lib.vf_groupnorm_workspace_bytes(n_img, HW, C)), dtype=torch.uint8, device=x.device)
    check(lib.vf_groupnorm_stats_f32(_p(_f32(x)), _p(_f32(gamma)), n_img, HW, C, groups, eps, _p(mean_c), _p(scale_c),
                                     _p(ws), _stream()), 'vf_groupnorm_stats_f32')
    return mean_c, scale_c


def halo_gn_slots(Hout, Wout):
    return int(_lib.load().vf_conv3_halo_gn_slots(Hout, Wout))


def new_gn_part(n_img, Hout, Wout, device):
    return torch.empty((n_img, halo_gn_slots(Hout, Wout), 32, 2), dtype=torch.float32, device=device)


def groupnorm_finalize(part, gamma, n_img, HW, C, groups=32, eps=1e-6):
    lib = _lib.load()
    mean_c = torch.empty((n_img, C), dtype=torch.float32, device=part.device)
    scale_c = torch.empty((n_img, C), dtype=torch.float32, device=part.device)
    check(lib.vf_groupnorm_finalize_f32(_p(_f32(part)), _p(_f32(gamma)), n_img, HW, C, groups, part.shape[1], eps,
                                        _p(mean_c), _p(scale_c), _stream()), 'vf_groupnorm_finalize_f32')
    return mean_c, scale_c


def groupnorm_apply(x, mean_c, scale_c, beta, n_img, HW, C, swish, out=None):
    lib = _lib.load()
    if out is None:
        out = torch.empty_like(x)
    check(lib.vf_groupnorm_apply_f32(_p(_f32(x)), _p(mean_c), _p(scale_c), _p(_f32(beta)), _p(out), n_img, HW, C,
                                     1 if swish else 0, _stream()), 'vf_groupnorm_apply_f32')
    return out


def vq_pack_codebook(E):
    lib = _lib.load()
    E = _f32(E).contiguous()
    D, Kc = E.shape
    out = torch.empty(int(lib.vf_vq_packed_floats(D, Kc)), dtype=torch.float32, device=E.device)
    check(lib.vf_vq_pack_codebook_f32(_p(E), _p(out), D, Kc, _stream()), 'vf_vq_pack_codebook_f32')
    e_sq = torch.empty(Kc, dtype=torch.float32, device=E.device)
    check(lib.vf_colsumsq_f32(_p(E), _p(e_sq), D, Kc, _stream()), 'vf_colsumsq_f32')
    return out, e_sq


def vq_argmin(z_rows, E_packed, e_sq, D, Kc):
    lib = _lib.load()
    z_rows = _f32(z_rows)
    M = z_rows.numel() // D
    idx = torch.empty(M, dtype=torch.int64, device=z_rows.device)
    check(lib.vf_vq_argmin_f32(_p(z_rows), _p(E_packed), _p(e_sq), M, D, Kc, _p(idx), _stream()), 'vf_vq_argmin_f32')
    return idx


def vq_filter_supported(D, Kc):
    return int(_lib.load().vf_vq_filter_packed_bytes(D, Kc)) > 0


def vq_filter_pack(E):
    lib = _lib.load()
    E = _f32(E).contiguous()
    D, Kc = E.shape
    n = int(lib.vf_vq_filter_packed_bytes(D, Kc))
    if n == 0:
        raise _lib.VfError(f'vq_filter_pack: unsupported codebook shape D={D}, Kc={Kc} (need D == 256, Kc % 32 == 0, Kc <= 1024)')
    out = torch.empty(n, dtype=torch.uint8, device=E.device)
    check(lib.vf_vq_filter_pack(_p(E), _p(out), D, Kc, _stream()), 'vf_vq_filter_pack')
    return out


def vq_argmin_filtered(z_rows, blob, D, Kc, stats=None):
    lib = _lib.load()
    z_rows = _f32(z_rows)
    M = z_rows.numel() // D
    idx = torch.empty(M, dtype=torch.int64, device=z_rows.device)
    check(lib.vf_vq_argmin_filtered_f32(_p(z_rows), _p(_chk(blob, torch.uint8, 'blob')), M, D, Kc, _p(idx),
                                        _p(_chk(stats, torch.int32, 'stats')) if stats is not None else None, _stream()),
          'vf_vq_argmin_filtered_f32')
    return idx


def codebook_gather(E, idx, D, Kc):
    lib = _lib.load()
    idx = _chk(idx, torch.int64, 'codes').contiguous()
    M = idx.numel()
    out = torch.empty((M, D), dtype=torch.float32, device=idx.device)
    check(lib.vf_codebook_gather_f32(_p(_f32(E)), _p(idx), _p(out), M, D, Kc, _stream()), 'vf_codebook_gather_f32')
    return out


def attn_blockcausal(q, k, v, out, B, H, T, L, ldq, ldk, ldv, ldo, scale=1.0, skip_masked=True, twin_view=-1, bf16=False, x6=False,
                     fp8=False):
    lib = _lib.load()
    if fp8:
        bf16 = True
    if x6:
        check(lib.vf_attn_blockcausal_x6(_p(_f32(q)), _p(_f32(k)), _p(_f32(v)), _p(_f32(out)), B, H, T, L, ldq, ldk, ldv,
                                         ldo, scale, 1 if skip_masked else 0, twin_view, _stream()),
              'vf_attn_blockcausal_x6')
        return out
    if bf16:
        o16 = out.dtype == torch.bfloat16
        i16 = q.dtype == torch.bfloat16
        for t in (q, k, v):
            _chk(t, torch.bfloat16 if i16 else torch.float32, 'q/k/v')
        fn = lib.vf_attn_blockcausal_fp8 if fp8 else lib.vf_attn_blockcausal_bf16_v2
        check(fn(_p(q), _p(k), _p(v), 1 if i16 else 0, _p(out if o16 else _f32(out)), 1 if o16 else 0, B, H, T, L,
                 ldq, ldk, ldv, ldo, scale, 1 if skip_masked else 0, twin_view, _stream()), 'vf_attn_blockcausal_lp')
        return out
    check(lib.vf_attn_blockcausal_f32(_p(_f32(q)), _p(_f32(k)), _p(_f32(v)), _p(_f32(out)), B, H, T, L, ldq, ldk, ldv,
                                      ldo, scale, 1 if skip_masked else 0, twin_view, _stream()),
          'vf_attn_blockcausal_f32')
    return out


def attn_prefix(q, k, v, kp, vp, out, B, H, C, N, L, ldq, ldk, ldv, ldkp, ldvp, prefix_stride, ldo, bf16=False, dh=64):
    lib = _lib.load()
    if bf16:
        o16 = out.dtype == torch.bfloat16
        i16 = q.dtype == torch.bfloat16
        for t in (q, k, v, kp, vp):
            _chk(t, torch.bfloat16 if i16 else torch.float32, 'q/k/v/prefix')
        check(lib.vf_attn_prefix_bf16(_p(q), _p(k), _p(v), _p(kp), _p(vp), 1 if i16 else 0, _p(out if o16 else _f32(out)), 1 if o16 else 0,
                                      B, H, C, N, L, dh, ldq, ldk, ldv, ldkp, ldvp, prefix_stride, ldo, _stream()), 'vf_attn_prefix_bf16')
        return out
    check(lib.vf_attn_prefix_f32eq(_p(_f32(q)), _p(_f32(k)), _p(_f32(v)), _p(_f32(kp)), _p(_f32(vp)), _p(_f32(out)), B, H, C, N, L, dh,
                                   ldq, ldk, ldv, ldkp, ldvp, prefix_stride, ldo, _stream()), 'vf_attn_prefix_f32eq')
    return out


def attn_spatial_supported(HW, C):
    return (HW, C) in ((256, 256), (64, 512), (64, 256))


def attn_spatial(qkv, n_img, HW, C, scale, out=None, x3h=False):
    if out is None:
        out = torch.empty((n_img * HW, C), dtype=torch.float32, device=qkv.device)
    fn = _lib.load().vf_attn_spatial_x3h if x3h else _lib.load().vf_attn_spatial_f32
    check(fn(_p(_f32(qkv)), _p(_f32(out)), n_img, HW, C, qkv.stride(0), out.stride(0), scale, _stream()),
          'vf_attn_spatial_x3h' if x3h else 'vf_attn_spatial_f32')
    return out


def softmax_rows_(x, rows, n, scale=1.0):
    check(_lib.load().vf_softmax_rows_f32(_p(_f32(x)), rows, n, scale, _stream()), 'vf_softmax_rows_f32')
    return x


def layernorm(x, gamma, beta, rows, d, eps=1e-5, out=None, out_bf16=False):
    if out_bf16:
        out = torch.empty(x.shape, dtype=torch.bfloat16, device=x.device) if out is None else _chk(out, torch.bfloat16, 'out')
        check(_lib.load().vf_layernorm_bf16out_f32(_p(_f32(x)), _p(_f32(gamma)), _p(_f32(beta)), _p(out), rows, d, eps, _stream()),
              'vf_layernorm_bf16out_f32')
        return out
    if out is None:
        out = torch.empty_like(x)
    check(_lib.load().vf_layernorm_f32(_p(_f32(x)), _p(_f32(gamma)), _p(_f32(beta)), _p(out), rows, d, eps, _stream()),
          'vf_layernorm_f32')
    return out


def embed_sum(ids_i32, wte, wpe, add, BS, L, d, vocab):
    out = torch.empty((BS * L, d), dtype=torch.float32, device=wte.device)
    check(_lib.load().vf_embed_sum_f32(_p(_chk(ids_i32, torch.int32, 'ids')), _p(_f32(wte)), _p(_f32(wpe)),
                                       _p(_f32(add)), _p(out), BS, L, d, vocab, _stream()), 'vf_embed_sum_f32')
    return out


def dense_small_k(x, W, b, rows, K, N, gelu):
    out = torch.empty((rows, N), dtype=torch.float32, device=x.device)
    check(_lib.load().vf_dense_small_k_gelu_f32(_p(_f32(x)), _p(_f32(W)), _p(b), _p(out), rows, K, N,
                                                1 if gelu else 0, _stream()), 'vf_dense_small_k_gelu_f32')
    return out


def argmax_rows(x, rows, n, ld=None):
    idx = torch.empty(rows, dtype=torch.int64, device=x.device)
    check(_lib.load().vf_argmax_rows_f32(_p(_f32(x)), rows, n, n if ld is None else ld, _p(idx), _stream()),
          'vf_argmax_rows_f32')
    return idx


def lmhead_argmax_supported(K, N):
    return K in (128, 768) and N % 128 == 0


def lmhead_argmax_bf16(h, w_packed_bf16, M, K, N, want_max=False):
    idx = torch.empty(M, dtype=torch.int64, device=h.device)
    mx = torch.empty(M, dtype=torch.float32, device=h.device) if want_max else None
    h16 = h.dtype == torch.bfloat16
    _chk(h, torch.bfloat16 if h16 else torch.float32, 'h')
    check(_lib.load().vf_lmhead_argmax_bf16(_p(h), 1 if h16 else 0, h.stride(0), _p(_chk(w_packed_bf16, torch.bfloat16, 'w_packed')), M, K, N,
                                            _p(idx), _p(mx) if mx is not None else None, _stream()), 'vf_lmhead_argmax_bf16')
    return (idx, mx) if want_max else idx


def postprocess_u8(x):
    x = _f32(x).contiguous()
    out = torch.empty(x.shape, dtype=torch.uint8, device=x.device)
    check(_lib.load().vf_postprocess_u8(_p(x), _p(out), x.numel(), _stream()), 'vf_postprocess_u8')
    return out


def resize_u8(images, image_size, method=None):
    if method not in (None, 'nearest', 'bilinear'):
        raise ValueError("method must be None, 'nearest' or 'bilinear'")
    n, H, W, C = images.shape
    if W == image_size or H == image_size:
        return images
    if method is None:
        method = 'nearest' if image_size > H else 'bilinear'
    src = _chk(images.contiguous(), torch.uint8, 'images')
    out = torch.empty((n, image_size, image_size, C), dtype=torch.uint8, device=images.device)
    check(_lib.load().vf_resize_u8(_p(src), _p(out), n, H, W, image_size, image_size, C, 1 if method == 'bilinear' else 0, _stream()),
          'vf_resize_u8')
    return out


def image_metrics_u8(a, b):
    if a.shape != b.shape or a.dim() != 4:
        raise ValueError(f'image_metrics_u8: two [n,H,W,C] batches of one shape expected, got {tuple(a.shape)} and {tuple(b.shape)}')
    a = _chk(a, torch.uint8, 'a').contiguous()
    b = _chk(b, torch.uint8, 'b').contiguous()
    n, H, W, C = a.shape
    if n == 0:
        return torch.empty((0, 2), dtype=torch.int64, device=a.device), torch.empty(0, dtype=torch.float64, device=a.device)
    lib = _lib.load()
    ws =torch.empty(max(int(lib.vf_image_metrics_workspace_bytes(n, H, W, C)), 8), dtype=torch.uint8, device=a.device)
    sums = torch.empty((n, 2), dtype=torch.int64, device=a.device)
    ssim = torch.empty(n, dtype=torch.float64, device=a.device)
    check(lib.vf_image_metrics_u8(_p(a), _p(b), n, H, W, C, _p(sums), _p(ssim), _p(ws), _stream()), 'vf_image_metrics_u8')
    return sums, ssim


def camera_knn(db, queries, k, pos_weight=0.3, return_dist=False):
    if db.dim() != 2 or db.shape[1] != 7 or queries.dim() != 2 or queries.shape[1] != 7:
        raise ValueError(f'camera_knn: db [N,7] and queries [Q,7] expected, got {tuple(db.shape)} and {tuple(queries.shape)}')
    db = _f32(db, 'db').contiguous()
    queries = _f32(queries, 'queries').contiguous()
    N, Q, k = db.shape[0], queries.shape[0], int(k)
    idx = torch.empty((Q, k), dtype=torch.int32, device=db.device)
    dist = torch.empty((Q, k), dtype=torch.float32, device=db.device) if return_dist else None
    lib = _lib.load()
    ws = torch.empty(max(int(lib.vf_camera_knn_workspace_bytes(N, Q, k)), 8), dtype=torch.uint8, device=db.device)
    check(lib.vf_camera_knn_f32(_p(db), N, _p(queries), Q, k, float(pos_weight), _p(idx), _p(dist), _p(ws), _stream()), 'vf_camera_knn_f32')
    return (idx, dist) if return_dist else idx
```

### viewformer_amd/vqgan.py

```python
import re
from collections import OrderedDict

import os

import numpy as np
import torch

from . import ops
from .config import VQGANConfig
from .weights import vqgan_layout

_IGNORED = re.compile(r'(perceptual_loss\..*)|(loss\..*)')


class _Conv:
    __slots__ = ('wp', 'wp16', 'wp6', 'wp3h', 'bias', 'cin', 'cout', 'k', 'w_raw')


class VQGAN:
    def __init__(self, config: VQGANConfig = None, data_format: str = 'NCHW', device=None, max_images_per_call: int = 1024,
                 decoder_precision: str = 'f32', conv_arith: str = 'x3h', lookup: str = 'filter'):
        self.config = config or VQGANConfig()
        assert data_format in ('NCHW', 'NHWC')
        assert decoder_precision in ('f32', 'bf16') and conv_arith in ('f32', 'x6', 'x3h') and lookup in ('filter', 'exact')
        self.lookup = lookup
        self.decoder_precision = decoder_precision
        self.conv_arith = conv_arith
        self.data_format = data_format
        self.device = torch.device(device) if device is not None else None
        self.max_images_per_call = max_images_per_call
        self._enc_plan, self._dec_plan = vqgan_layout(self.config)
        self._sd = None
        self._conv = {}
        self._norm = {}
        self._qkv = {}
        self.training = False
        self.dense_x3h = os.environ.get('VF_VQ_DENSE_X3H', '1') != '0'

    def eval(self):
        return self

    def to(self, device):
        device = torch.device(device)
        if device.type != 'cuda':
            raise ops._lib.VfError('viewformer_amd.VQGAN runs on the GPU only (no CPU fallback)')
        self.device = device
        if self._sd_host is not None:
            self._upload()
        return self

    _sd_host = None

    def expected_keys(self):
        keys = []
        for kind, name, args in self._enc_plan + self._dec_plan:
            if kind in ('conv3', 'down', 'up'):
                keys += [name + '.weight', name + '.bias']
            elif kind == 'res':
                for p in ('norm1', 'conv1', 'norm2', 'conv2'):
                    keys += [f'{name}.{p}.weight', f'{name}.{p}.bias']
                if args[0] != args[1]:
                    keys += [f'{name}.nin_shortcut.weight', f'{name}.nin_shortcut.bias']
            elif kind == 'attn':
                for p in ('norm', 'q', 'k', 'v', 'proj_out'):
                    keys += [f'{name}.{p}.weight', f'{name}.{p}.bias']
            elif kind == 'norm_swish':
                keys += [name + '.weight', name + '.bias']
        keys += ['quant_conv.weight', 'quant_conv.bias', 'post_quant_conv.weight', 'post_quant_conv.bias',
                 'quantize.embeddings', 'quantize.ema_cluster_size_hidden', 'quantize.ema_dw_hidden', 'quantize.counter']
        return keys

    def load_state_dict(self, state_dict, strict: bool = True):
        sd = {k: v for k, v in state_dict.items() if not _IGNORED.match(k)}
        if strict:
            want = set(self.expected_keys())
            have = set(sd.keys())
            if want - have:
                raise RuntimeError(f'Missing keys: {want - have}')
            if have - want:
                raise RuntimeError(f'Unexpected keys: {have - want}')
        host = OrderedDict()
        for k, v in sd.items():
            if isinstance(v, torch.Tensor):
                v = v.detach().cpu().numpy()
            host[k] = np.ascontiguousarray(v)
        self._sd_host = host
        if self.device is not None:
            self._upload()
        return self

    def state_dict(self):
        return OrderedDict((k, torch.from_numpy(v)) for k, v in self._sd_host.items())

    def _upload(self):
        dev = self.device
        h = self._sd_host
        self._conv, self._norm, self._qkv = {}, {}, {}
        self._act16_cache = {}

        def dev_t(name):
            return torch.from_numpy(h[name]).to(dev, torch.float32).contiguous()

        def conv(name):
            w = dev_t(name + '.weight')
            c = _Conv()
            c.cout, c.cin, c.k = w.shape[0], w.shape[1], w.shape[2]
            c.bias = dev_t(name + '.bias')
            c.w_raw = w
            c.wp = ops.pack_conv_oihw(w) if c.cin % 32 == 0 else None
            c.wp16 = None
            c.wp6 = None
            c.wp3h = None
            split = self.conv_arith in ('x6', 'x3h')
            if self.conv_arith == 'x3h' and c.k == 3 and c.cin == 3 and c.cout % 128 == 0:
                c.wp3h = ops.pack_conv_in_x3h(w)
            if split and c.k == 3 and c.cin % 32 == 0 and c.cout % 128 == 0:
                c.wp6 = ops.pack_conv3_x6(w)
                if self.conv_arith == 'x3h':
                    c.wp3h = ops.pack_conv3_x3h(w)
            elif split and c.k == 1 and c.cin % 64 == 0 and c.cout >= 64:
                c.wp6 = ops.pack_dense_nk_x6(w.reshape(c.cout, c.cin))
                if self.conv_arith == 'x3h' and self.dense_x3h:
                    c.wp3h = ops.pack_dense_nk_x3h(w.reshape(c.cout, c.cin))
            if self.decoder_precision == 'bf16' and (name.startswith('decoder.') or name == 'post_quant_conv'):
                if c.k == 3 and c.cin % 32 == 0 and c.cout % 128 == 0:
                    c.wp16 = ops.pack_conv3_bf16(w)
                elif c.k == 1 and c.cin % 64 == 0:
                    c.wp16 = ops.pack_dense_nk_bf16(w.reshape(c.cout, c.cin))
            self._conv[name] = c

        def norm(name):
            self._norm[name] = (dev_t(name + '.weight'), dev_t(name + '.bias'))

        for kind, name, args in self._enc_plan + self._dec_plan:
            if kind in ('conv3', 'down', 'up'):
                conv(name)
            elif kind == 'res':
                norm(name + '.norm1'); conv(name + '.conv1'); norm(name + '.norm2'); conv(name + '.conv2')
                if args[0] != args[1]:
                    conv(name + '.nin_shortcut')
            elif kind == 'attn':
                norm(name + '.norm')
                c = args[0]
                w = torch.cat([dev_t(f'{name}.{p}.weight').reshape(c, c) for p in ('q', 'k', 'v')], 0)
                b = torch.cat([dev_t(f'{name}.{p}.bias') for p in ('q', 'k', 'v')], 0)
                if self.conv_arith == 'x3h' and self.dense_x3h and c % 64 == 0:
                    self._qkv[name] = (ops.pack_dense_nk_x3h(w), b)
                else:
                    self._qkv[name] = (ops.pack_dense_nk_x6(w) if self.conv_arith in ('x6', 'x3h') and c % 64 == 0 else ops.pack_dense_nk(w), b)
                conv(name + '.proj_out')
            elif kind == 'norm_swish':
                norm(name)
        conv('quant_conv')
        conv('post_quant_conv')
        self._E = dev_t('quantize.embeddings')
        self._E_packed, self._e_sq = ops.vq_pack_codebook(self._E)
        self._E_filter = (ops.vq_filter_pack(self._E) if self.lookup == 'filter' and ops.vq_filter_supported(*self._E.shape)
                          else None)
        torch.cuda.synchronize(dev)

    def _conv3(self, x, name, n, H, W, mode=ops.MODE_CONV3_S1, pro=None, pro_swish=True, res=None, o16=False):
        c = self._conv[name]
        a16 = x.dtype == torch.bfloat16
        if mode == ops.MODE_CONV3_S2PAD:
            Ho, Wo = H // 2, W // 2
        elif mode == ops.MODE_CONV3_UP2:
            Ho, Wo = H * 2, W * 2
        else:
            Ho, Wo = H, W
        if res is None and ops.conv3_small_cout_supported(mode, c.cin, c.cout, Ho, Wo):
            self._stats_of = None
            return ops.conv3_small_cout(x, c.w_raw, c.bias, n, H, W, c.cin, c.cout, pro=pro, pro_swish=pro_swish), Ho, Wo
        o16 = o16 or a16
        out = torch.empty((n * Ho * Wo, c.cout), dtype=torch.bfloat16 if o16 else torch.float32, device=x.device)
        bf16 = (c.wp16 is not None and mode in (ops.MODE_CONV3_S1, ops.MODE_CONV3_UP2) and Ho % 8 == 0 and Wo % 16 == 0)
        if o16 and not bf16:
            raise ops._lib.VfError(f'{name}: bf16 activations need the bf16 convolution arm (halo-kernel shape)')
        x3h = (not bf16 and c.wp3h is not None and ops.conv3_x3h_supported(mode, c.cin, c.cout, Ho, Wo)
               and not (mode == ops.MODE_CONV3_S2PAD and pro is not None))
        x6 = (not bf16 and not x3h and c.wp6 is not None and ops.conv3_x6_supported(mode, c.cin, c.cout, Ho, Wo)
              and not (mode == ops.MODE_CONV3_S2PAD and pro is not None))
        part = None
        if (bf16 or x6 or x3h) and self.fuse_gn_stats and c.cout in (128, 256, 512, 1024):
            part = ops.new_gn_part(n, Ho, Wo, x.device)
        ops.igemm(x, c.wp16 if bf16 else c.wp3h if x3h else c.wp6 if x6 else c.wp, n * Ho * Wo, c.cin, c.cout, out, bias=c.bias, res=res,
                  mode=mode, pro=pro, pro_swish=pro_swish, Hin=H, Win=W, Hout=Ho, Wout=Wo, bf16=bf16, x6=x6, x3h=x3h, gn_part=part,
                  a16=a16, o16=o16)
        self._stats_of = (out, part) if part is not None else None
        return out, Ho, Wo

    def _conv1(self, x, name, M, pro=None, pro_swish=False, rows_per_img=0, res=None):
        c = self._conv[name]
        a16 = x.dtype == torch.bfloat16
        out = torch.empty((M, c.cout), dtype=x.dtype, device=x.device)
        bf16 = c.wp16 is not None and pro is None
        if a16 and not (bf16 and res is None):
            raise ops._lib.VfError(f'{name}: bf16 activations need the plain bf16 GEMM')
        x3h = not bf16 and c.k == 1 and c.wp3h is not None
        x6 = not bf16 and not x3h and c.wp6 is not None
        ops.igemm(x, c.wp16 if bf16 else c.wp3h if x3h else c.wp6 if x6 else c.wp, M, c.cin, c.cout, out, bias=c.bias, res=res, pro=pro,
                  pro_swish=pro_swish, pro_rows_per_img=rows_per_img, bf16=bf16, x6=x6, x3h=x3h, a16=a16, o16=a16)
        return out

    def _gn(self, x, name, n, HW, C):
        gamma, beta = self._norm[name]
        if self._stats_of is not None and self._stats_of[0] is x:
            mean_c, scale_c = ops.groupnorm_finalize(self._stats_of[1], gamma, n, HW, C, 32, 1e-6)
        else:
            if x.dtype != torch.float32:
                raise ops._lib.VfError(f'{name}: a bf16 activation carries its GroupNorm statistics from the producing kernel (fuse_gn_stats)')
            mean_c, scale_c = ops.groupnorm_stats(x, gamma, n, HW, C, 32, 1e-6)
        return (mean_c, scale_c, beta)

    _stats_of = None
    decoder_act16 = 128
    fuse_gn_stats = True
    fused_attention = True

    def _res(self, x, name, n, H, W, cin, cout):
        p1 = self._gn(x, name + '.norm1', n, H * W, cin)
        h, _, _ = self._conv3(x, name + '.conv1', n, H, W, pro=p1)
        p2 = self._gn(h, name + '.norm2', n, H * W, cout)
        sc = x if cin == cout else self._conv1(x, name + '.nin_shortcut', n * H * W)
        out, _, _ = self._conv3(h, name + '.conv2', n, H, W, pro=p2, res=sc)
        return out

    def _attn(self, x, name, n, H, W, C):
        HW = H * W
        M = n * HW
        pro = self._gn(x, name + '.norm', n, HW, C)
        wp, b = self._qkv[name]
        qkv = torch.empty((M, 3 * C), dtype=torch.float32, device=x.device)
        ops.igemm(x, wp, M, C, 3 * C, qkv, bias=b, pro=pro, pro_swish=False, pro_rows_per_img=HW, x6=wp.dtype == torch.bfloat16,
                  x3h=wp.dtype == torch.float16)
        if self.fused_attention and ops.attn_spatial_supported(HW, C):
            a = ops.attn_spatial(qkv, n, HW, C, float(int(C) ** (-0.5)), x3h=self.conv_arith == 'x3h' and self.dense_x3h)
            return self._conv1(a, name + '.proj_out', M, res=x)
        q, k, v = qkv[:, :C], qkv[:, C:2 * C], qkv[:, 2 * C:]
        kp = ops.pack(k, C, HW, 1, sk=1, sn=3 * C, st=0, batch=n, src_bstride=HW * 3 * C)
        S = torch.empty((n, HW, HW), dtype=torch.float32, device=x.device)
        ops.igemm(q, kp, HW, C, HW, S, lda=3 * C, batch=n, stride_x=HW * 3 * C,
                  stride_w=ops.packed_floats(C, HW), stride_out=HW * HW)
        ops.softmax_rows_(S, n * HW, HW, float(int(C) ** (-0.5)))
        vp = ops.pack(v, HW, C, 1, sk=3 * C, sn=1, st=0, batch=n, src_bstride=HW * 3 * C)
        a = torch.empty((M, C), dtype=torch.float32, device=x.device)
        ops.igemm(S, vp, HW, HW, C, a, lda=HW, batch=n, stride_x=HW * HW, stride_w=ops.packed_floats(HW, C),
                  stride_out=HW * C)
        return self._conv1(a, name + '.proj_out', M, res=x)

    def _act16_plan_ok(self, plan, idx, H, W):
        key = (id(plan), idx, H, W)
        hit = self._act16_cache.get(key)
        if hit is not None:
            return hit

        def conv_ok(name, mode, h, w, feeds_norm=True):
            c = self._conv[name]
            ho, wo = (h * 2, w * 2) if mode == ops.MODE_CONV3_UP2 else (h, w)
            if ops.conv3_small_cout_supported(mode, c.cin, c.cout, ho, wo):
                return True
            return (c.wp16 is not None and ho % 8 == 0 and wo % 16 == 0 and (not feeds_norm or c.cout in (128, 256, 512, 1024)))

        ok = self.fuse_gn_stats and conv_ok(plan[idx][1], ops.MODE_CONV3_UP2, H // 2, W // 2)
        h, w = H, W
        for kind, name, args in plan[idx + 1:]:
            if not ok:
                break
            if kind == 'res':
                ok = conv_ok(name + '.conv1', ops.MODE_CONV3_S1, h, w) and conv_ok(name + '.conv2', ops.MODE_CONV3_S1, h, w)
                if ok and args[0] != args[1]:
                    sc = self._conv[name + '.nin_shortcut']
                    ok = sc.wp16 is not None and sc.k == 1
            elif kind == 'up':
                ok = conv_ok(name, ops.MODE_CONV3_UP2, h, w)
                h, w = h * 2, w * 2
            elif kind == 'conv3':
                ok = conv_ok(name, ops.MODE_CONV3_S1, h, w, feeds_norm=False)
            elif kind == 'norm_swish':
                ok = True
            else:
                ok = False
        self._act16_cache[key] = bool(ok)
        return bool(ok)

    def _run_plan(self, plan, x, n, H, W, first_is_image=False):
        for idx, (kind, name, args) in enumerate(plan):
            if kind == 'conv3':
                c = self._conv[name]
                if c.wp is None:
                    if c.wp3h is not None and ops.conv_in_x3h_supported(H, W, c.cout):
                        part = ops.new_gn_part(n, H, W, x.device) if self.fuse_gn_stats and c.cout in (128, 256, 512, 1024) else None
                        x = ops.conv_in(x, c.w_raw, c.bias, n, H, W, c.cout, wp3h=c.wp3h, gn_part=part).view(n * H * W, c.cout)
                        self._stats_of = (x, part) if part is not None else None
                    else:
                        x = ops.conv_in(x, c.w_raw, c.bias, n, H, W, c.cout).view(n * H * W, c.cout)
                        self._stats_of = None
                else:
                    x, H, W = self._conv3(x, name, n, H, W, pro=self._pending_pro, pro_swish=True)
                self._pending_pro = None
            elif kind == 'res':
                x = self._res(x, name, n, H, W, args[0], args[1])
            elif kind == 'attn':
                x = self._attn(x, name, n, H, W, args[0])
            elif kind == 'down':
                x, H, W = self._conv3(x, name, n, H, W, mode=ops.MODE_CONV3_S2PAD)
            elif kind == 'up':
                o16 = bool(self.decoder_act16 and self.decoder_precision == 'bf16' and self.fuse_gn_stats and name.startswith('decoder.')
                           and H * 2 >= max(32, int(self.decoder_act16)) and (H * 2) % 8 == 0 and (W * 2) % 16 == 0
                           and x.dtype != torch.bfloat16 and self._act16_plan_ok(plan, idx, H * 2, W * 2))
                x, H, W = self._conv3(x, name, n, H, W, mode=ops.MODE_CONV3_UP2, o16=o16)
            elif kind == 'norm_swish':
                self._pending_pro = self._gn(x, name, n, H * W, args[0])
        return x, H, W

    _pending_pro = None
    _act16_cache = None

    def _encode_nhwc(self, img):
        n, H, W, _ = img.shape
        x, h, w = self._run_plan(self._enc_plan, img.contiguous(), n, H, W)
        z = self._conv1(x, 'quant_conv', n * h * w)
        cfg = self.config
        if self._E_filter is not None:
            codes = ops.vq_argmin_filtered(z, self._E_filter, cfg.embed_dim, cfg.n_embed)
        else:
            codes = ops.vq_argmin(z, self._E_packed, self._e_sq, cfg.embed_dim, cfg.n_embed)
        return z, codes.view(n, h, w)

    def _decode_rows(self, q_rows, n, h, w):
        x = self._conv1(q_rows, 'post_quant_conv', n * h * w)
        x, H, W = self._run_plan(self._dec_plan, x, n, h, w)
        return x.view(n, H, W, self.config.out_ch)

    def _chunks(self, n):
        m = max(1, min(self.max_images_per_call, (2 ** 31 - 1) // max(1, self.config.image_size ** 2)))
        return [(i, min(n, i + m)) for i in range(0, n, m)]

    def _to_nhwc(self, x):
        if x.dtype == torch.uint8:
            return x
        return x.permute(0, 2, 3, 1) if self.data_format == 'NCHW' else x

    def encode(self, x):
        self._require_ready()
        x = self._to_nhwc(x.to(self.device))
        n = x.shape[0]
        if n == 0:
            t = x.shape[1] // self.config.stride
            return _LazyEncodeResult(self, torch.empty((0, self.config.embed_dim), dtype=torch.float32, device=self.device),
                                     torch.empty((0, t, t), dtype=torch.int64, device=self.device))
        zs, cs = [], []
        for a, b in self._chunks(n):
            z, c = self._encode_nhwc(x[a:b])
            zs.append(z)
            cs.append(c)
        z = torch.cat(zs, 0) if len(zs) > 1 else zs[0]
        codes = torch.cat(cs, 0) if len(cs) > 1 else cs[0]
        return _LazyEncodeResult(self, z, codes)

    def encode_codes(self, x):
        return self.encode(x)[-1]

    def decode_code(self, code_b):
        self._require_ready()
        cfg = self.config
        codes = code_b.to(self.device).to(torch.int64).contiguous()
        n, h, w = codes.shape
        if n == 0:
            s = self.config.stride
            out = torch.empty((0, h * s, w * s, self.config.out_ch), dtype=torch.float32, device=self.device)
            return out.permute(0, 3, 1, 2) if self.data_format == 'NCHW' else out
        outs = []
        for a, b in self._chunks(n):
            q = ops.codebook_gather(self._E, codes[a:b], cfg.embed_dim, cfg.n_embed)
            outs.append(self._decode_rows(q, b - a, h, w))
        out = torch.cat(outs, 0) if len(outs) > 1 else outs[0]
        return out.permute(0, 3, 1, 2) if self.data_format == 'NCHW' else out

    def decode(self, quant):
        self._require_ready()
        q = quant.to(self.device)
        q = q.permute(0, 2, 3, 1) if self.data_format == 'NCHW' else q
        n, h, w, d = q.shape
        out = self._decode_rows(q.contiguous().view(n * h * w, d), n, h, w)
        return out.permute(0, 3, 1, 2) if self.data_format == 'NCHW' else out

    def __call__(self, x):
        quant, diff, codes = self.encode(x)
        return self.decode(quant), diff, quant, codes

    forward = __call__

    def _require_ready(self):
        if self._sd_host is None:
            raise RuntimeError('VQGAN: load_state_dict() first')
        if self.device is None:
            raise RuntimeError('VQGAN: .to("cuda") first (GPU only)')


class _LazyEncodeResult(tuple):

    def __new__(cls, model, z, codes):
        self = super().__new__(cls, (None, None, codes))
        self._model, self._z, self._codes = model, z, codes
        self._qd = None
        return self

    def _quant_diff(self):
        if self._qd is None:
            m, cfg = self._model, self._model.config
            n, h, w = self._codes.shape
            if n == 0:
                quant = torch.empty((0, h, w, cfg.embed_dim), dtype=torch.float32, device=self._codes.device)
                self._qd = (quant.permute(0, 3, 1, 2) if m.data_format == 'NCHW' else quant,
                            torch.full((), float('nan'), device=self._codes.device))
                return self._qd
            q = ops.codebook_gather(m._E, self._codes, cfg.embed_dim, cfg.n_embed)
            z = self._z
            diff = (q - z).pow(2).mean()
            quant = (z + (q - z)).view(n, h, w, cfg.embed_dim)
            if m.data_format == 'NCHW':
                quant = quant.permute(0, 3, 1, 2)
            self._qd = (quant, diff)
        return self._qd

    def __getitem__(self, i):
        if isinstance(i, slice):
            return tuple(self[j] for j in range(*i.indices(3)))
        i = i if i >= 0 else 3 + i
        if i == 2:
            return self._codes
        return self._quant_diff()[i]

    def __iter__(self):
        yield self[0]
        yield self[1]
        yield self[2]
```

Baseline: 1146.

## Recompute conv_in inside the first res-block convolutions instead of re-reading it

Adds x3h halo-conv variants that recompute the encoder's conv_in output on the fly from the raw image. It can be used as the residual in conv2 (default 'res' mode) or as the input tile of conv1 (alternate mode, with a separate stats-only conv_in kernel feeding GroupNorm). In the default mode conv_in is still materialised for conv1 and norm1, but conv2 no longer reads that 128-channel activation back from memory for the residual. The epilogue is moved into a shared helper. The cost is extra conv_in arithmetic and LDS staging in the fused kernel, and added register and LDS pressure.

```diff
diff --git a/include/vf_hip.h b/include/vf_hip.h
--- a/include/vf_hip.h
+++ b/include/vf_hip.h
@@ -72,6 +72,8 @@
 int vf_conv_in_x3h_pack(const float* w_oihw, void* dst, int Cout, void* stream);
 int vf_conv_in_x3h(const uint8_t* img_u8, const float* img_f32, const void* w_packed, const float* bias, float* out, float* gn_part,
                    int gn_slots, int n_img, int H, int W, int Cout, void* stream);
+int vf_conv_in_x3h_stats(const uint8_t* img_u8, const float* img_f32, const void* w_packed, const float* bias, float* gn_part, int gn_slots,
+                         int n_img, int H, int W, int Cout, void* stream);
 
 int vf_conv3_small_cout_f32(const float* x, const float* w_oihw, const float* bias, const float* pro_mean,
                             const float* pro_scale, const float* pro_beta, int pro_swish, float* out, int n_img, int H, int W,
@@ -160,6 +162,10 @@
 size_t vf_conv3_x3h_packed_elems(int Cin, int Cout);
 int vf_conv3_x3h_pack(const float* w_oihw, void* dst, int Cin, int Cout, void* stream);
 int vf_conv3_halo_x3h(const vf_igemm_args* args , void* stream);
+int vf_conv3_halo_x3h_res_conv_in(const vf_igemm_args* args , const uint8_t* img_u8, const float* img_f32, const void* conv_in_packed,
+                                  const float* conv_in_bias, void* stream);
+int vf_conv3_halo_x3h_in_conv_in(const vf_igemm_args* args , const uint8_t* img_u8, const float* img_f32, const void* conv_in_packed,
+                                 const float* conv_in_bias, void* stream);
 size_t vf_gemm_x3h_packed_elems(int K, int N);
 int vf_gemm_x3h_pack(const float* src, void* dst, int K, int N, int64_t sk, int64_t sn, void* stream);
 int vf_gemm_x3h(const vf_igemm_args* args , void* stream);
diff --git a/viewformer_amd/_lib.py b/viewformer_amd/_lib.py
--- a/viewformer_amd/_lib.py
+++ b/viewformer_amd/_lib.py
@@ -46,6 +46,7 @@
     'vf_conv_in_x3h_packed_elems': (c_size_t, [c_int]),
     'vf_conv_in_x3h_pack': (c_int, [P, P, c_int, P]),
     'vf_conv_in_x3h': (c_int, [P, P, P, P, P, P, c_int, c_int, c_int, c_int, c_int, P]),
+    'vf_conv_in_x3h_stats': (c_int, [P, P, P, P, P, c_int, c_int, c_int, c_int, c_int, P]),
     'vf_crc32c': (ctypes.c_uint32, [P, c_size_t, ctypes.c_uint32]),
     'vf_conv3_small_cout_f32': (c_int, [P, P, P, P, P, P, c_int, P, c_int, c_int, c_int, c_int, c_int, c_int, P]),
     'vf_groupnorm_workspace_bytes': (c_size_t, [c_int, c_int, c_int]),
@@ -128,6 +129,8 @@
     'vf_conv3_x3h_packed_elems': (c_size_t, [c_int, c_int]),
     'vf_conv3_x3h_pack': (c_int, [P, P, c_int, c_int, P]),
     'vf_conv3_halo_x3h': (c_int, [POINTER(VfIgemmArgs), P]),
+    'vf_conv3_halo_x3h_res_conv_in': (c_int, [POINTER(VfIgemmArgs), P, P, P, P, P]),
+    'vf_conv3_halo_x3h_in_conv_in': (c_int, [POINTER(VfIgemmArgs), P, P, P, P, P]),
     'vf_gemm_x3h_packed_elems': (c_size_t, [c_int, c_int]),
     'vf_gemm_x3h_pack': (c_int, [P, P, c_int, c_int, c_int64, c_int64, P]),
     'vf_gemm_x3h': (c_int, [POINTER(VfIgemmArgs), P]),
diff --git a/viewformer_amd/csrc/conv3_halo_x3h.hip b/viewformer_amd/csrc/conv3_halo_x3h.hip
--- a/viewformer_amd/csrc/conv3_halo_x3h.hip
+++ b/viewformer_amd/csrc/conv3_halo_x3h.hip
@@ -1,5 +1,6 @@
 #include <type_traits>
 #include "halo_common.h"
+#include "conv_in_tile.h"
 
 namespace {
 
@@ -380,9 +381,11 @@
 
 
 typedef float f32x4v __attribute__((ext_vector_type(4)));
-
-template <bool PRO, bool SWISH>
-__global__ __launch_bounds__(256, 2) void conv3_halo_x3h16_kernel(vf_igemm_args p) {
+constexpr int CI_NONE = 0, CI_RES = 1, CI_IN = 2;
+constexpr int CI_REC_BYTES = vf_conv_in_lds_bytes(TH + 2, TW + 2);
+
+template <bool PRO, bool SWISH, int CI = CI_NONE>
+__global__ __launch_bounds__(256, 2) void conv3_halo_x3h16_kernel(vf_igemm_args p, vf_conv_in_src ci) {
     using G = Geo<false, false>;
     extern __shared__ __attribute__((aligned(16))) unsigned char smem_h[];
     constexpr int RT = 8, CT = 2;
@@ -428,14 +431,45 @@
     }
     unsigned char* __restrict__ raw_l = smem_h + 2 * G::BUF;
     const __amdgpu_buffer_rsrc_t x_rs = __builtin_amdgcn_make_buffer_rsrc(const_cast<float*>(X), 0, 0x7fffffff, 0x00020000);
-    float* __restrict__ pro_l = reinterpret_cast<float*>(smem_h + 2 * G::BUF + G::SLOTS * 4096 - 1024);
+    float* __restrict__ pro_l = reinterpret_cast<float*>(smem_h + 2 * G::BUF + (CI == CI_IN ? CI_REC_BYTES : G::SLOTS * 4096 - 1024));
     if (PRO) {
         for (int i = tid; i < p.Cin; i += 256) {
             pro_l[i] = p.pro_mean[(size_t)img * p.Cin + i];
             pro_l[p.Cin + i] = p.pro_scale[(size_t)img * p.Cin + i];
             pro_l[2 * p.Cin + i] = p.pro_beta[i];
-        }
-    }
+            if (CI == CI_IN) pro_l[3 * p.Cin + i] = ci.bias ? ci.bias[i] : 0.f;
+        }
+    }
+    vf_f16x8 ciw[2];
+    const float ci_inv_s = CI == CI_IN ? vf_conv_in_inv_s(ci, p.Cin) : 0.f;
+    int lane_v = lane;
+    auto ci_w_load = [&](int chunk, int k) { vf_conv_in_weights(ci, chunk * 2 + (k & 1), lane, ciw[0], ciw[1]); };
+    auto ci_tile_store = [&](int buf, int chunk, int k, const vf_f16x8 (&w)[2]) {
+        asm volatile("" : "+v"(lane_v));
+        const int l_m = lane_v & 15, l_g = lane_v >> 4;
+        const int pt = wave * 3 + (k >> 1), ct = k & 1;
+        const int pa = min(pt * 16 + l_m, (int)G::NPIX - 1);
+        const int par = (pa * 3641) >> 16;
+        const unsigned char* rec = raw_l + vf_conv_in_rec<TH + 2, TW + 2>(par, pa - par * G::PW, l_g);
+        const vf_f16x8 ah = *reinterpret_cast<const vf_f16x8*>(rec), al = *reinterpret_cast<const vf_f16x8*>(rec + 16);
+        const int cl = ct * 16 + l_m, ch = chunk * CK + cl;
+        const f32x4 o = vf_conv_in_tile(ah, al, w[0], w[1], ci_inv_s, pro_l[3 * p.Cin + ch]);
+        const float pmean = pro_l[ch], pscale = pro_l[p.Cin + ch], pbeta = pro_l[2 * p.Cin + ch];
+        unsigned char* dst = smem_h + buf * G::BUF + ((cl >> 3 & 1) * 2 + (cl >> 4)) * 16 + (cl & 7) * 2;
+#pragma unroll
+        for (int r = 0; r < 4; ++r) {
+            const int px = pt * 16 + l_g * 4 + r;
+            const int pr = (px * 3641) >> 16, pc = px - pr * G::PW;
+            const bool ok = (px < G::NPIX) & ((unsigned)(sy0 + pr) < (unsigned)p.Hin) & ((unsigned)(sx0 + pc) < (unsigned)p.Win);
+            float t = (o[r] - pmean) * pscale + pbeta;
+            if (SWISH) t = vf_swish_1ulp(t);
+            _Float16 h, l;
+            split2(ok ? t : 0.f, h, l);
+            unsigned char* d = dst + min(px, (int)G::NPIX) * P_LDB;
+            *reinterpret_cast<_Float16*>(d) = h;
+            *reinterpret_cast<_Float16*>(d + 64) = l;
+        }
+    };
     int pro_chunk = 0;
     auto patch_load = [&](int chunk) {
         asm volatile("" : "+v"(pix0));
@@ -508,12 +542,23 @@
 #pragma unroll
             for (int r = 0; r < 4; ++r) { acc[i][j][r] = 0.f; accx[i][j][r] = 0.f; }
 
-    patch_load(0);
-    b_load(bring[0], 0);
-    asm volatile("s_waitcnt vmcnt(0)" ::: "memory");
-    if (PRO) __syncthreads();
-#pragma unroll
-    for (int q = 0; q < G::SLOTS; ++q) patch_store_slot(0, q);
+    if (CI == CI_IN) {
+        vf_conv_in_park<TH + 2, TW + 2>(raw_l, ci, img, p.Hin, p.Win, sy0, sx0, tid);
+        b_load(bring[0], 0);
+        __syncthreads();
+        vf_f16x8 w0[2][2];
+#pragma unroll
+        for (int ct = 0; ct < 2; ++ct) vf_conv_in_weights(ci, ct, lane, w0[ct][0], w0[ct][1]);
+#pragma unroll
+        for (int k = 0; k < G::SLOTS; ++k) ci_tile_store(0, 0, k, w0[k & 1]);
+    } else {
+        patch_load(0);
+        b_load(bring[0], 0);
+        asm volatile("s_waitcnt vmcnt(0)" ::: "memory");
+        if (PRO) __syncthreads();
+#pragma unroll
+        for (int q = 0; q < G::SLOTS; ++q) patch_store_slot(0, q);
+    }
     __syncthreads();
 
     auto chunk_body = [&](int chunk, auto parity) {
@@ -522,18 +567,21 @@
         const bool more = chunk + 1 < nchunks;
         b_load(bring[(P0 + 1) & 1], chunk * 9 + 1);
         unsigned pad[G::SLOTS];
-#pragma unroll
-        for (int q = 0; q < G::SLOTS; ++q) pad[q] = __builtin_amdgcn_raw_buffer_load_b32(w_rs, (unsigned)(q * 256), 0u, 0);
-        if (more) patch_load(chunk + 1);
+        if (CI != CI_IN) {
+#pragma unroll
+            for (int q = 0; q < G::SLOTS; ++q) pad[q] = __builtin_amdgcn_raw_buffer_load_b32(w_rs, (unsigned)(q * 256), 0u, 0);
+            if (more) patch_load(chunk + 1);
+        }
 #pragma unroll
         for (int i = 0; i < AR - 1; ++i) a_load(aring[i], patch, i);
 #pragma unroll
         for (int t = 0; t < 9; ++t) {
             if (t > 0) b_load(bring[(P0 + t + 1) & 1], chunk * 9 + t + 1);
-            if (t == 2) {
+            if (t == 2 && CI != CI_IN) {
 #pragma unroll
                 for (int q = 0; q < G::SLOTS; ++q) asm volatile("" :: "v"(pad[q]));
             }
+            if (CI == CI_IN && t >= 1 && t <= G::SLOTS) ci_w_load(min(chunk + 1, nchunks - 1), t - 1);
             const f16x8 (&B)[4] = bring[(P0 + t) & 1];
 #pragma unroll
             for (int rt = 0; rt < RT; ++rt) {
@@ -549,8 +597,11 @@
                 __builtin_amdgcn_sched_barrier(0);
             }
             if (t >= 1 && t <= G::SLOTS && more) {
-                if (t == 1) asm volatile("s_waitcnt vmcnt(8)" ::: "memory");
-                patch_store_slot((P0 + 1) & 1, t - 1);
+                if (CI == CI_IN) ci_tile_store((P0 + 1) & 1, chunk + 1, t - 1, ciw);
+                else {
+                    if (t == 1) asm volatile("s_waitcnt vmcnt(8)" ::: "memory");
+                    patch_store_slot((P0 + 1) & 1, t - 1);
+                }
             }
         }
         __syncthreads();
@@ -561,12 +612,8 @@
     }
 
     const float inv_s = *reinterpret_cast<const float*>(reinterpret_cast<const unsigned char*>(p.w_packed) + (size_t)nchunks * 9 * nb * TAP_BYTES);
-    const __amdgpu_buffer_rsrc_t o_rs = __builtin_amdgcn_make_buffer_rsrc(p.out + (size_t)img * p.Hout * p.Wout * p.ldc, 0, 0x7fffffff, 0x00020000);
     const __amdgpu_buffer_rsrc_t r_rs = __builtin_amdgcn_make_buffer_rsrc(const_cast<float*>(p.res ? p.res + (size_t)img * p.Hout * p.Wout * p.ldr : p.out), 0, 0x7fffffff, 0x00020000);
-    const bool Res = p.res != nullptr;
-    const bool stats = p.gn_part != nullptr;
-    const int cg = p.Cout >> 5;
-    const int tile_slot = (ty * tilesX + tx) * 2;
+    const bool Res = CI == CI_RES || p.res != nullptr;
     const int pbase = lg == 0 ? 0 : lg == 1 ? 1 : lg == 2 ? 9 : 8;
     auto spix = [&](int rt, int r) { return (y0 + rt) * p.Wout + x0 + 2 * r; };
 #pragma unroll
@@ -577,7 +624,11 @@
             for (int r = 0; r < 4; ++r) acc[rt][ct][r] = __builtin_fmaf(accx[rt][ct][r], 4.8828125e-4f, acc[rt][ct][r]) * inv_s;
     __builtin_amdgcn_sched_barrier(0);
     float rr[CT][RT][4];
-    if (Res) {
+    if (CI == CI_RES) {
+        vf_conv_in_park<TH, TW>(smem_h, ci, img, p.Hout, p.Wout, y0, x0, tid);
+        __syncthreads();
+        vf_conv_in_wave_tile(smem_h, ci, p.Cout, nblk, wave, lane, rr);
+    } else if (Res) {
 #pragma unroll
         for (int ct = 0; ct < CT; ++ct) {
             const int n = nblk * BN + wave * 32 + ct * 16 + lm;
@@ -589,39 +640,7 @@
                     rr[ct][rt][r] = __builtin_bit_cast(float, __builtin_amdgcn_raw_buffer_load_b32(r_rs, rv, (unsigned)(spix(rt, r) * p.ldr) * 4u, 0));
         }
     }
-#pragma unroll
-    for (int ct = 0; ct < CT; ++ct) {
-        const int n = nblk * BN + wave * 32 + ct * 16 + lm;
-        const float bias = p.bias ? p.bias[n] : 0.f;
-        const unsigned ov = (unsigned)(pbase * p.ldc + n) * 4u;
-#pragma unroll
-        for (int sl = 0; sl < 2; ++sl) {
-            float s32 = 0.f, q32 = 0.f;
-#pragma unroll
-            for (int k = 0; k < 4; ++k) {
-                const int rt = sl * 4 + k;
-#pragma unroll
-                for (int r = 0; r < 4; ++r) {
-                    float v = acc[rt][ct][r] + bias;
-                    if (Res) v += rr[ct][rt][r];
-                    __builtin_amdgcn_raw_buffer_store_b32(__builtin_bit_cast(unsigned, v), o_rs, ov, (unsigned)(spix(rt, r) * p.ldc) * 4u, 0);
-                    s32 += v;
-                    q32 = __builtin_fmaf(v, v, q32);
-                }
-            }
-            if (stats) {
-                vf_gn_acc_t s = (vf_gn_acc_t)s32, q = (vf_gn_acc_t)q32;
-                for (int o = 1; o < cg; o <<= 1) { s += __shfl_xor(s, o, 64); q += __shfl_xor(q, o, 64); }
-                s += __shfl_xor(s, 16, 64); q += __shfl_xor(q, 16, 64);
-                s += __shfl_xor(s, 32, 64); q += __shfl_xor(q, 32, 64);
-                if (lg == 0 && (lm & (cg - 1)) == 0) {
-                    float* dst = p.gn_part + ((((size_t)img * p.gn_slots) + tile_slot + sl) * 32 + n / cg) * 2;
-                    dst[0] = (float)s;
-                    dst[1] = (float)q;
-                }
-            }
-        }
-    }
+    vf_t16_epilogue(p, acc, rr, Res, img, y0, x0, (ty * tilesX + tx) * 2, nblk, wave, lane);
 }
 
 __global__ void absmax_kernel(const float* __restrict__ w, long long n, unsigned* __restrict__ out) {
@@ -671,20 +690,21 @@
 }
 
 static inline size_t vf_x3h16_lds_bytes(int pro_cin) { return (size_t)2 * Geo<false, false>::BUF + Geo<false, false>::SLOTS * 4096 - 1024 + (size_t)3 * pro_cin * 4; }
-
-template <bool PRO, bool SWISH>
-int launch_halo16(const vf_igemm_args& a, hipStream_t stream) {
+static inline size_t vf_x3h16_ci_in_lds_bytes(int cin) { return (size_t)2 * Geo<false, false>::BUF + CI_REC_BYTES + (size_t)4 * cin * 4; }
+
+template <bool PRO, bool SWISH, int CI = CI_NONE>
+int launch_halo16(const vf_igemm_args& a, hipStream_t stream, const vf_conv_in_src& ci = {}) {
     using G = Geo<false, false>;
     const int n_img = a.M / (a.Hout * a.Wout);
     const long long blocks = (long long)n_img * (a.Hout / TH) * (a.Wout / TW) * (a.Cout / BN);
-    const size_t smem = vf_x3h16_lds_bytes(PRO ? a.Cin : 0);
+    const size_t smem = CI == CI_IN ? vf_x3h16_ci_in_lds_bytes(a.Cin) : vf_x3h16_lds_bytes(PRO ? a.Cin : 0);
     static unsigned long long attr_devs = 0;
     if (vf_attr_needed(&attr_devs)) {
-        const hipError_t e = hipFuncSetAttribute(reinterpret_cast<const void*>(conv3_halo_x3h16_kernel<PRO, SWISH>), hipFuncAttributeMaxDynamicSharedMemorySize, 80 * 1024);
+        const hipError_t e = hipFuncSetAttribute(reinterpret_cast<const void*>(conv3_halo_x3h16_kernel<PRO, SWISH, CI>), hipFuncAttributeMaxDynamicSharedMemorySize, 80 * 1024);
         if (e != hipSuccess) return (int)e;
         vf_attr_done(&attr_devs);
     }
-    hipLaunchKernelGGL((conv3_halo_x3h16_kernel<PRO, SWISH>), dim3((unsigned)blocks), dim3(256), smem, stream, a);
+    hipLaunchKernelGGL((conv3_halo_x3h16_kernel<PRO, SWISH, CI>), dim3((unsigned)blocks), dim3(256), smem, stream, a, ci);
     return vf_last_status();
 }
 
@@ -759,4 +779,32 @@
     return (a.mode == VF_MODE_CONV3_UP2) ? dispatch_pro<true, false>(a, s) : dispatch_pro<false, false>(a, s);
 }
 
-}
+static int conv_in_fused(const vf_igemm_args* args, const uint8_t* img_u8, const float* img_f32, const void* conv_in_packed, const float* conv_in_bias,
+                         void* stream, bool as_input) {
+    if (!args || (!img_u8 && !img_f32) || !conv_in_packed) return VF_ERR_BAD_ARG;
+    const vf_igemm_args& a = *args;
+    if ((as_input ? a.x != nullptr : !a.x) || !a.w_packed || !a.out || a.M <= 0 || (!as_input && a.res)) return VF_ERR_BAD_ARG;
+    if (a.drop_rate != 0.f || a.out_aux) return VF_ERR_UNSUPPORTED;
+    if (a.mode != VF_MODE_CONV3_S1 || a.Cout % BN != 0 || a.Cin % (2 * CK) != 0 || a.Hout % TH != 0 || a.Wout % TW != 0) return VF_ERR_UNSUPPORTED;
+    if (!(a.pro_mean && a.pro_scale && a.pro_beta && a.pro_swish) || !vf_selected(VF_SEL_CONV_X3H_K32)) return VF_ERR_UNSUPPORTED;
+    if (a.gn_part && a.Cout / 32 > 16) return VF_ERR_UNSUPPORTED;
+    if ((as_input ? vf_x3h16_ci_in_lds_bytes(a.Cin) : vf_x3h16_lds_bytes(a.Cin)) > 80 * 1024 || (as_input && a.Cin % BN != 0)) return VF_ERR_UNSUPPORTED;
+    if (a.Hin != a.Hout || a.Win != a.Wout || a.M % (a.Hout * a.Wout) != 0) return VF_ERR_BAD_ARG;
+    if (a.batch > 1 || a.epilogue != VF_EPI_NONE || a.ldc < a.Cout || (a.res && a.ldr < a.Cout)) return VF_ERR_BAD_ARG;
+    if ((long long)a.Hin * a.Win * a.Cin >= (1ll << 31)) return VF_ERR_UNSUPPORTED;
+    if (int st = vf_halo_gn_check(a)) return st;
+    const vf_conv_in_src ci = {img_u8, img_f32, conv_in_packed, conv_in_bias};
+    return as_input ? launch_halo16<true, true, CI_IN>(a, (hipStream_t)stream, ci) : launch_halo16<true, true, CI_RES>(a, (hipStream_t)stream, ci);
+}
+
+int vf_conv3_halo_x3h_res_conv_in(const vf_igemm_args* args, const uint8_t* img_u8, const float* img_f32, const void* conv_in_packed,
+                                  const float* conv_in_bias, void* stream) {
+    return conv_in_fused(args, img_u8, img_f32, conv_in_packed, conv_in_bias, stream, false);
+}
+
+int vf_conv3_halo_x3h_in_conv_in(const vf_igemm_args* args, const uint8_t* img_u8, const float* img_f32, const void* conv_in_packed,
+                                 const float* conv_in_bias, void* stream) {
+    return conv_in_fused(args, img_u8, img_f32, conv_in_packed, conv_in_bias, stream, true);
+}
+
+}
diff --git a/viewformer_amd/csrc/conv_in_tile.h b/viewformer_amd/csrc/conv_in_tile.h
--- /dev/null
+++ b/viewformer_amd/csrc/conv_in_tile.h
@@ -0,0 +1,150 @@
+#pragma once
+#include "halo_common.h"
+
+typedef _Float16 vf_f16x8 __attribute__((ext_vector_type(8)));
+
+struct vf_conv_in_src {
+    const unsigned char* u8;
+    const float* f32;
+    const void* w_packed;
+    const float* bias;
+};
+
+constexpr int VF_CI_REC = 32;
+constexpr int VF_CI_TILE_BYTES = 2 * 64 * 16;
+__host__ __device__ constexpr int vf_conv_in_lds_bytes(int rows, int cols) { return ((rows + 2) * cols + rows * cols) * VF_CI_REC; }
+
+__device__ __forceinline__ void vf_ci_split2(float x, _Float16& h, _Float16& l) {
+    h = (_Float16)x;
+    l = (_Float16)((x - (float)h) * 2048.f);
+}
+
+__device__ __forceinline__ float vf_conv_in_px(const vf_conv_in_src& s, int img, int H, int W, int sy, int sx, int c) {
+    if ((unsigned)sy >= (unsigned)H || (unsigned)sx >= (unsigned)W) return 0.f;
+    const size_t i = (((size_t)img * H + sy) * W + sx) * 3 + c;
+    if (s.u8) return ((float)s.u8[i] * (1.0f / 255.0f)) * 2.0f - 1.0f;
+    return s.f32[i];
+}
+
+template <int ROWS, int COLS>
+__device__ __forceinline__ void vf_conv_in_park(unsigned char* __restrict__ lds, const vf_conv_in_src& s, int img, int H, int W, int oy, int ox, int tid) {
+    constexpr int NROW = (ROWS + 2) * COLS, NREC = NROW + ROWS * COLS;
+    for (int j = tid; j < NREC; j += 256) {
+        const bool tail = j >= NROW;
+        const int jj = tail ? j - NROW : j;
+        const int r = jj / COLS, c = jj - r * COLS;
+        vf_f16x8 oh, ol;
+#pragma unroll
+        for (int e = 0; e < 8; ++e) {
+            float v = 0.f;
+            if (!tail) v = vf_conv_in_px(s, img, H, W, oy - 1 + r, ox - 1 + c + e / 3, e % 3);
+            else if (e < 3) v = vf_conv_in_px(s, img, H, W, oy - 1 + r + e, ox + 1 + c, 2);
+            _Float16 h, l;
+            vf_ci_split2(v, h, l);
+            oh[e] = h; ol[e] = l;
+        }
+        *reinterpret_cast<vf_f16x8*>(lds + j * VF_CI_REC) = oh;
+        *reinterpret_cast<vf_f16x8*>(lds + j * VF_CI_REC + 16) = ol;
+    }
+}
+
+template <int ROWS, int COLS>
+__device__ __forceinline__ int vf_conv_in_rec(int r, int c, int lg) {
+    return (lg < 3 ? (r + lg) * COLS + c : (ROWS + 2) * COLS + r * COLS + c) * VF_CI_REC;
+}
+
+__device__ __forceinline__ void vf_conv_in_weights(const vf_conv_in_src& s, int tile, int lane, vf_f16x8& bh, vf_f16x8& bl) {
+    const unsigned char* w = reinterpret_cast<const unsigned char*>(s.w_packed) + (size_t)tile * VF_CI_TILE_BYTES + lane * 16;
+    bh = *reinterpret_cast<const vf_f16x8*>(w);
+    bl = *reinterpret_cast<const vf_f16x8*>(w + 64 * 16);
+}
+__device__ __forceinline__ float vf_conv_in_inv_s(const vf_conv_in_src& s, int Cout) {
+    return *reinterpret_cast<const float*>(reinterpret_cast<const unsigned char*>(s.w_packed) + (size_t)(Cout / 16) * VF_CI_TILE_BYTES);
+}
+
+__device__ __forceinline__ f32x4 vf_conv_in_tile(vf_f16x8 ah, vf_f16x8 al, vf_f16x8 bh, vf_f16x8 bl, float inv_s, float bias) {
+    const f32x4 z = {0.f, 0.f, 0.f, 0.f};
+    f32x4 x = __builtin_amdgcn_mfma_f32_16x16x32_f16(al, bh, z, 0, 0, 0);
+    x = __builtin_amdgcn_mfma_f32_16x16x32_f16(ah, bl, x, 0, 0, 0);
+    f32x4 m = __builtin_amdgcn_mfma_f32_16x16x32_f16(ah, bh, z, 0, 0, 0);
+    f32x4 o;
+#pragma unroll
+    for (int r = 0; r < 4; ++r) {
+        o[r] = __builtin_fmaf(x[r], 4.8828125e-4f, m[r]) * inv_s + bias;
+        asm volatile("" : "+v"(o[r]));
+    }
+    return o;
+}
+
+constexpr int VF_T16_RT = 8, VF_T16_CT = 2;
+__device__ __forceinline__ int vf_t16_pix(int lm) { return lm < 4 ? 2 * lm : lm < 12 ? 2 * lm - 7 : 2 * lm - 16; }
+
+__device__ __forceinline__ void vf_conv_in_wave_tile(const unsigned char* __restrict__ lds, const vf_conv_in_src& s, int Cout, int nblk, int wave, int lane,
+                                                     float (&h)[VF_T16_CT][VF_T16_RT][4]) {
+    const int lm = lane & 15, lg = lane >> 4;
+    vf_f16x8 bh[VF_T16_CT], bl[VF_T16_CT];
+    float bias[VF_T16_CT];
+#pragma unroll
+    for (int ct = 0; ct < VF_T16_CT; ++ct) {
+        vf_conv_in_weights(s, nblk * 8 + wave * 2 + ct, lane, bh[ct], bl[ct]);
+        bias[ct] = s.bias ? s.bias[nblk * 128 + wave * 32 + ct * 16 + lm] : 0.f;
+    }
+    const float inv_s = vf_conv_in_inv_s(s, Cout);
+    const int a_lane = vf_conv_in_rec<8, 16>(0, vf_t16_pix(lm), lg);
+#pragma unroll
+    for (int rt = 0; rt < VF_T16_RT; ++rt) {
+        const vf_f16x8 ah = *reinterpret_cast<const vf_f16x8*>(lds + a_lane + rt * 16 * VF_CI_REC);
+        const vf_f16x8 al = *reinterpret_cast<const vf_f16x8*>(lds + a_lane + rt * 16 * VF_CI_REC + 16);
+#pragma unroll
+        for (int ct = 0; ct < VF_T16_CT; ++ct) {
+            const f32x4 o = vf_conv_in_tile(ah, al, bh[ct], bl[ct], inv_s, bias[ct]);
+#pragma unroll
+            for (int r = 0; r < 4; ++r) h[ct][rt][r] = o[r];
+        }
+    }
+}
+
+template <bool STORE = true>
+__device__ __forceinline__ void vf_t16_epilogue(const vf_igemm_args& p, const f32x4 (&acc)[VF_T16_RT][VF_T16_CT], const float (&rr)[VF_T16_CT][VF_T16_RT][4],
+                                                bool res, int img, int y0, int x0, int tile_slot, int nblk, int wave, int lane) {
+    constexpr int BN = 128;
+    const int lm = lane & 15, lg = lane >> 4;
+    const __amdgpu_buffer_rsrc_t o_rs = __builtin_amdgcn_make_buffer_rsrc(p.out + (STORE ? (size_t)img * p.Hout * p.Wout * p.ldc : 0), 0, 0x7fffffff, 0x00020000);
+    const bool stats = p.gn_part != nullptr;
+    const int cg = p.Cout >> 5;
+    const int pbase = lg == 0 ? 0 : lg == 1 ? 1 : lg == 2 ? 9 : 8;
+    auto spix = [&](int rt, int r) { return (y0 + rt) * p.Wout + x0 + 2 * r; };
+#pragma unroll
+    for (int ct = 0; ct < VF_T16_CT; ++ct) {
+        const int n = nblk * BN + wave * 32 + ct * 16 + lm;
+        const float bias = p.bias ? p.bias[n] : 0.f;
+        const unsigned ov = (unsigned)(pbase * p.ldc + n) * 4u;
+#pragma unroll
+        for (int sl = 0; sl < 2; ++sl) {
+            float s32 = 0.f, q32 = 0.f;
+#pragma unroll
+            for (int k = 0; k < 4; ++k) {
+                const int rt = sl * 4 + k;
+#pragma unroll
+                for (int r = 0; r < 4; ++r) {
+                    float v = acc[rt][ct][r] + bias;
+                    if (res) v += rr[ct][rt][r];
+                    if (STORE) __builtin_amdgcn_raw_buffer_store_b32(__builtin_bit_cast(unsigned, v), o_rs, ov, (unsigned)(spix(rt, r) * p.ldc) * 4u, 0);
+                    s32 += v;
+                    q32 = __builtin_fmaf(v, v, q32);
+                }
+            }
+            if (stats) {
+                vf_gn_acc_t s = (vf_gn_acc_t)s32, q = (vf_gn_acc_t)q32;
+                for (int o = 1; o < cg; o <<= 1) { s += __shfl_xor(s, o, 64); q += __shfl_xor(q, o, 64); }
+                s += __shfl_xor(s, 16, 64); q += __shfl_xor(q, 16, 64);
+                s += __shfl_xor(s, 32, 64); q += __shfl_xor(q, 32, 64);
+                if (lg == 0 && (lm & (cg - 1)) == 0) {
+                    float* dst = p.gn_part + ((((size_t)img * p.gn_slots) + tile_slot + sl) * 32 + n / cg) * 2;
+                    dst[0] = (float)s;
+                    dst[1] = (float)q;
+                }
+            }
+        }
+    }
+}
diff --git a/viewformer_amd/csrc/conv_in_x3h.hip b/viewformer_amd/csrc/conv_in_x3h.hip
--- a/viewformer_amd/csrc/conv_in_x3h.hip
+++ b/viewformer_amd/csrc/conv_in_x3h.hip
@@ -1,31 +1,16 @@
-#include "halo_common.h"
+#include "conv_in_tile.h"
 
 namespace {
 
-typedef _Float16 f16x8 __attribute__((ext_vector_type(8)));
-typedef _Float16 f16x4 __attribute__((ext_vector_type(4)));
-
 constexpr int TH = 8, TW = 16, BN = 128;
-constexpr int PW = TW + 2, PH = TH + 2, NPIX = PH * PW;
-constexpr int P_LDB = 16;
-constexpr int PLANE_BYTES = 2 * BN * 16;
-constexpr int KS_BYTES = 2 * PLANE_BYTES;
-constexpr int BLK_BYTES = 3 * KS_BYTES;
 constexpr int TAIL_BYTES = 16;
 
-__device__ __forceinline__ void split2(float x, _Float16& h, _Float16& l) {
-    h = (_Float16)x;
-    l = (_Float16)((x - (float)h) * 2048.f);
-}
-
-template <bool U8>
-__global__ __launch_bounds__(256) void conv_in_x3h_kernel(vf_igemm_args p, const unsigned char* __restrict__ img_u8) {
-    __shared__ __attribute__((aligned(16))) unsigned char patch[NPIX * P_LDB];
+template <bool STORE>
+__global__ __launch_bounds__(256) void conv_in_x3h_kernel(vf_igemm_args p, vf_conv_in_src src) {
+    __shared__ __attribute__((aligned(16))) unsigned char rec[vf_conv_in_lds_bytes(TH, TW)];
     const int tid = threadIdx.x;
     const int lane = tid & 63;
     const int wave = __builtin_amdgcn_readfirstlane(tid >> 6);
-    const int wave_m = wave >> 1, wave_n = wave & 1;
-    const int half = lane >> 5, l31 = lane & 31;
 
     const int nb = p.Cout / BN;
     const int tilesX = p.Wout / TW, tilesY = p.Hout / TH;
@@ -36,84 +21,18 @@
     const int img = bid / tilesY;
     const int y0 = ty * TH, x0 = tx * TW;
 
-    if (tid < NPIX) {
-        const int pr = tid / PW, pc = tid - pr * PW;
-        const int sy = y0 - 1 + pr, sx = x0 - 1 + pc;
-        const bool ok = sy >= 0 && sy < p.Hout && sx >= 0 && sx < p.Wout;
-        const size_t px = ((size_t)img * p.Hout + (ok ? sy : 0)) * p.Wout + (ok ? sx : 0);
-        f16x4 oh, ol;
+    vf_conv_in_park<TH, TW>(rec, src, img, p.Hout, p.Wout, y0, x0, tid);
+    __syncthreads();
+    float h[VF_T16_CT][VF_T16_RT][4];
+    vf_conv_in_wave_tile(rec, src, p.Cout, nblk, wave, lane, h);
+    f32x4 acc[VF_T16_RT][VF_T16_CT];
 #pragma unroll
-        for (int c = 0; c < 3; ++c) {
-            float v;
-            if (U8) v = ((float)img_u8[px * 3 + c] * (1.0f / 255.0f)) * 2.0f - 1.0f;
-            else v = p.x[px * 3 + c];
-            _Float16 h, l;
-            split2(ok ? v : 0.f, h, l);
-            oh[c] = h; ol[c] = l;
-        }
-        oh[3] = (_Float16)0.f; ol[3] = (_Float16)0.f;
-        *reinterpret_cast<f16x4*>(patch + tid * P_LDB) = oh;
-        *reinterpret_cast<f16x4*>(patch + tid * P_LDB + 8) = ol;
-    }
-
-    const unsigned char* __restrict__ Wb = reinterpret_cast<const unsigned char*>(p.w_packed) + (size_t)nblk * BLK_BYTES +
-                                           (half * BN + wave_n * 64 + l31) * 16;
-    f16x8 b[3][2][2];
+    for (int rt = 0; rt < VF_T16_RT; ++rt)
 #pragma unroll
-    for (int ks = 0; ks < 3; ++ks)
+        for (int ct = 0; ct < VF_T16_CT; ++ct)
 #pragma unroll
-        for (int pl = 0; pl < 2; ++pl)
-#pragma unroll
-            for (int j = 0; j < 2; ++j) b[ks][pl][j] = *reinterpret_cast<const f16x8*>(Wb + ks * KS_BYTES + pl * PLANE_BYTES + j * 32 * 16);
-
-    f32x16 acc[2][2], accx[2][2];
-#pragma unroll
-    for (int i = 0; i < 2; ++i)
-#pragma unroll
-        for (int j = 0; j < 2; ++j)
-#pragma unroll
-            for (int r = 0; r < 16; ++r) { acc[i][j][r] = 0.f; accx[i][j][r] = 0.f; }
-    __syncthreads();
-
-    const int trow = vf_perm_row(l31), tpx = vf_perm_px(l31);
-#pragma unroll
-    for (int ks = 0; ks < 3; ++ks) {
-        const int g = ks * 2 + half;
-        f16x8 a[2][2];
-#pragma unroll
-        for (int mi = 0; mi < 2; ++mi) {
-            const int a0 = wave_m * 4 + mi * 2 + trow;
-#pragma unroll
-            for (int pl = 0; pl < 2; ++pl) {
-                f16x4 lo = {(_Float16)0.f, (_Float16)0.f, (_Float16)0.f, (_Float16)0.f}, hi = lo;
-                const int t0 = 2 * g, t1 = 2 * g + 1;
-                if (t0 < 9) lo = *reinterpret_cast<const f16x4*>(patch + ((a0 + t0 / 3) * PW + tpx + t0 % 3) * P_LDB + pl * 8);
-                if (t1 < 9) hi = *reinterpret_cast<const f16x4*>(patch + ((a0 + t1 / 3) * PW + tpx + t1 % 3) * P_LDB + pl * 8);
-                a[mi][pl] = f16x8{lo[0], lo[1], lo[2], lo[3], hi[0], hi[1], hi[2], hi[3]};
-            }
-        }
-#pragma unroll
-        for (int mi = 0; mi < 2; ++mi)
-#pragma unroll
-            for (int j = 0; j < 2; ++j) accx[mi][j] = __builtin_amdgcn_mfma_f32_32x32x16_f16(a[mi][1], b[ks][0][j], accx[mi][j], 0, 0, 0);
-#pragma unroll
-        for (int mi = 0; mi < 2; ++mi)
-#pragma unroll
-            for (int j = 0; j < 2; ++j) accx[mi][j] = __builtin_amdgcn_mfma_f32_32x32x16_f16(a[mi][0], b[ks][1][j], accx[mi][j], 0, 0, 0);
-#pragma unroll
-        for (int mi = 0; mi < 2; ++mi)
-#pragma unroll
-            for (int j = 0; j < 2; ++j) acc[mi][j] = __builtin_amdgcn_mfma_f32_32x32x16_f16(a[mi][0], b[ks][0][j], acc[mi][j], 0, 0, 0);
-    }
-
-    const float inv_s = *reinterpret_cast<const float*>(reinterpret_cast<const unsigned char*>(p.w_packed) + (size_t)nb * BLK_BYTES);
-#pragma unroll
-    for (int i = 0; i < 2; ++i)
-#pragma unroll
-        for (int j = 0; j < 2; ++j)
-#pragma unroll
-            for (int r = 0; r < 16; ++r) acc[i][j][r] = __builtin_fmaf(accx[i][j][r], 4.8828125e-4f, acc[i][j][r]) * inv_s;
-    vf_halo_epilogue<false>(p, acc, img, img, y0, x0, (ty * tilesX + tx) * 2, nblk, wave_m, wave_n, half, l31);
+            for (int r = 0; r < 4; ++r) acc[rt][ct][r] = h[ct][rt][r];
+    vf_t16_epilogue<STORE>(p, acc, h, false, img, y0, x0, (ty * tilesX + tx) * 2, nblk, wave, lane);
 }
 
 __global__ void absmax27_kernel(const float* __restrict__ w, long long n, unsigned* __restrict__ out) {
@@ -122,31 +41,45 @@
     vf_block_max_atomic(m, out);
 }
 
-__global__ void pack_conv_in_x3h_kernel(const float* __restrict__ w, _Float16* __restrict__ dst, int Cout, int nb,
-                                        unsigned char* __restrict__ tail) {
+__global__ void pack_conv_in_x3h_kernel(const float* __restrict__ w, _Float16* __restrict__ dst, int Cout, unsigned char* __restrict__ tail) {
     const float amax = __uint_as_float(*reinterpret_cast<const unsigned*>(tail + 4));
     const int ex = amax > 0.f ? ilogbf(amax) : 13;
     const float S = ldexpf(1.f, 13 - ex);
     if (blockIdx.x == 0 && threadIdx.x == 0) *reinterpret_cast<float*>(tail) = ldexpf(1.f, ex - 13);
-    const int total = nb * 3 * 2 * BN * 8;
+    const int total = (Cout / 16) * 64 * 8;
     for (int idx = blockIdx.x * blockDim.x + threadIdx.x; idx < total; idx += gridDim.x * blockDim.x) {
         const int e = idx & 7;
-        int t = idx >> 3;
-        const int nl = t % BN; t /= BN;
-        const int half = t & 1;
-        const int ks = (t >> 1) % 3;
-        const int nblk = (t >> 1) / 3;
-        const int k = (ks * 2 + half) * 8 + e;
-        const int tap = k >> 2, c = k & 3;
-        const int n = nblk * BN + nl;
+        const int ln = (idx >> 3) & 63;
+        const int tile = idx >> 9;
+        const int lg = ln >> 4, n = tile * 16 + (ln & 15);
+        int tap = -1, c = 0;
+        if (lg < 3) { tap = lg * 3 + e / 3; c = e % 3; }
+        else if (e < 3) { tap = e * 3 + 2; c = 2; }
         float v = 0.f;
-        if (tap < 9 && c < 3 && n < Cout) v = w[((size_t)n * 3 + c) * 9 + tap] * S;
+        if (tap >= 0) v = w[((size_t)n * 3 + c) * 9 + tap] * S;
         _Float16 h, l;
-        split2(v, h, l);
-        const size_t base = (((size_t)nblk * 3 + ks) * 2) * (2 * BN * 8) + ((size_t)half * BN + nl) * 8 + e;
+        vf_ci_split2(v, h, l);
+        const size_t base = (size_t)tile * (VF_CI_TILE_BYTES / 2) + ln * 8 + e;
         dst[base] = h;
-        dst[base + 2 * BN * 8] = l;
+        dst[base + 64 * 8] = l;
     }
+}
+
+int conv_in_args(vf_igemm_args& a, const float* img_f32, float* out, float* gn_part, int gn_slots, int n_img, int H, int W, int Cout) {
+    if (n_img <= 0 || H <= 0 || W <= 0 || Cout <= 0) return VF_ERR_BAD_ARG;
+    if (H % TH || W % TW || Cout % BN) return VF_ERR_UNSUPPORTED;
+    if ((long long)n_img * H * W >= (1ll << 31)) return VF_ERR_UNSUPPORTED;
+    a = {};
+    a.x = img_f32;
+    a.out = out;
+    a.mode = VF_MODE_CONV3_S1;
+    a.M = n_img * H * W; a.Cin = 3; a.Cout = Cout;
+    a.Hin = a.Hout = H; a.Win = a.Wout = W;
+    a.lda = 3; a.ldc = Cout; a.ldr = Cout;
+    a.batch = 1;
+    a.gn_part = gn_part;
+    a.gn_slots = gn_slots;
+    return vf_halo_gn_check(a);
 }
 
 }
@@ -155,41 +88,39 @@
 
 size_t vf_conv_in_x3h_packed_elems(int Cout) {
     if (Cout <= 0 || Cout % BN) return 0;
-    return (size_t)(Cout / BN) * 3 * 2 * 2 * BN * 8 + TAIL_BYTES / 2;
+    return (size_t)(Cout / 16) * (VF_CI_TILE_BYTES / 2) + TAIL_BYTES / 2;
 }
 
 int vf_conv_in_x3h_pack(const float* w_oihw, void* dst, int Cout, void* stream) {
     if (!w_oihw || !dst || Cout <= 0) return VF_ERR_BAD_ARG;
     if (Cout % BN) return VF_ERR_UNSUPPORTED;
-    const int nb = Cout / BN;
-    unsigned char* tail = reinterpret_cast<unsigned char*>(dst) + (size_t)nb * BLK_BYTES;
+    unsigned char* tail = reinterpret_cast<unsigned char*>(dst) + (size_t)(Cout / 16) * VF_CI_TILE_BYTES;
     hipStream_t s = (hipStream_t)stream;
     if (hipMemsetAsync(tail, 0, TAIL_BYTES, s) != hipSuccess) return vf_last_status();
     hipLaunchKernelGGL(absmax27_kernel, dim3(16), dim3(256), 0, s, w_oihw, (long long)Cout * 27, reinterpret_cast<unsigned*>(tail + 4));
-    hipLaunchKernelGGL(pack_conv_in_x3h_kernel, dim3(48), dim3(256), 0, s, w_oihw, (_Float16*)dst, Cout, nb, tail);
+    hipLaunchKernelGGL(pack_conv_in_x3h_kernel, dim3(32), dim3(256), 0, s, w_oihw, (_Float16*)dst, Cout, tail);
     return vf_last_status();
 }
 
 int vf_conv_in_x3h(const uint8_t* img_u8, const float* img_f32, const void* w_packed, const float* bias, float* out, float* gn_part,
                    int gn_slots, int n_img, int H, int W, int Cout, void* stream) {
-    if ((!img_u8 && !img_f32) || !w_packed || !out || n_img <= 0 || H <= 0 || W <= 0 || Cout <= 0) return VF_ERR_BAD_ARG;
-    if (H % TH || W % TW || Cout % BN) return VF_ERR_UNSUPPORTED;
-    vf_igemm_args a = {};
-    a.x = img_f32;
-    a.w_packed = reinterpret_cast<const float*>(w_packed);
-    a.bias = bias;
-    a.out = out;
-    a.mode = VF_MODE_CONV3_S1;
-    a.M = n_img * H * W; a.Cin = 3; a.Cout = Cout;
-    a.Hin = a.Hout = H; a.Win = a.Wout = W;
-    a.lda = 3; a.ldc = Cout; a.ldr = Cout;
-    a.batch = 1;
-    a.gn_part = gn_part;
-    a.gn_slots = gn_slots;
-    if (int st = vf_halo_gn_check(a)) return st;
+    if ((!img_u8 && !img_f32) || !w_packed || !out) return VF_ERR_BAD_ARG;
+    vf_igemm_args a;
+    if (int st = conv_in_args(a, img_f32, out, gn_part, gn_slots, n_img, H, W, Cout)) return st;
+    const vf_conv_in_src src = {img_u8, img_f32, w_packed, bias};
     const long long blocks = (long long)n_img * (H / TH) * (W / TW) * (Cout / BN);
-    if (img_u8) hipLaunchKernelGGL(conv_in_x3h_kernel<true>, dim3((unsigned)blocks), dim3(256), 0, (hipStream_t)stream, a, img_u8);
-    else hipLaunchKernelGGL(conv_in_x3h_kernel<false>, dim3((unsigned)blocks), dim3(256), 0, (hipStream_t)stream, a, img_u8);
+    hipLaunchKernelGGL(conv_in_x3h_kernel<true>, dim3((unsigned)blocks), dim3(256), 0, (hipStream_t)stream, a, src);
+    return vf_last_status();
+}
+
+int vf_conv_in_x3h_stats(const uint8_t* img_u8, const float* img_f32, const void* w_packed, const float* bias, float* gn_part, int gn_slots,
+                         int n_img, int H, int W, int Cout, void* stream) {
+    if ((!img_u8 && !img_f32) || !w_packed || !gn_part) return VF_ERR_BAD_ARG;
+    vf_igemm_args a;
+    if (int st = conv_in_args(a, img_f32, nullptr, gn_part, gn_slots, n_img, H, W, Cout)) return st;
+    const vf_conv_in_src src = {img_u8, img_f32, w_packed, bias};
+    const long long blocks = (long long)n_img * (H / TH) * (W / TW) * (Cout / BN);
+    hipLaunchKernelGGL(conv_in_x3h_kernel<false>, dim3((unsigned)blocks), dim3(256), 0, (hipStream_t)stream, a, src);
     return vf_last_status();
 }
 
diff --git a/viewformer_amd/ops.py b/viewformer_amd/ops.py
--- a/viewformer_amd/ops.py
+++ b/viewformer_amd/ops.py
@@ -256,13 +256,13 @@
 def igemm(x, w_packed, M, Cin, Cout, out, bias=None, res=None, mode=MODE_GEMM, epilogue=EPI_NONE,
           pro=None, pro_swish=False, pro_rows_per_img=0, Hin=0, Win=0, Hout=0, Wout=0,
           lda=None, ldc=None, ldr=None, batch=1, stride_x=0, stride_w=0, stride_out=0, stride_res=0, bf16=False, x6=False, gn_part=None, split_k=0,
-          x3h=False, a16=False, o16=False, out_aux=None, res16=False, drop=None, gelu_grad=False):
+          x3h=False, a16=False, o16=False, out_aux=None, res16=False, drop=None, gelu_grad=False, res_conv_in=None, x_conv_in=None):
     lib = _lib.load()
     if not 0 <= M < 2 ** 31 or max(Cin, Cout, Hin, Win, Hout, Wout, batch) >= 2 ** 31:
         raise _lib.VfError(f'igemm: M = {M} rows do not fit the int32 fields of vf_igemm_args — split the launch '
                            '(VQGAN(max_images_per_call=...))')
     a = VfIgemmArgs()
-    a.x = x.data_ptr()
+    a.x = x.data_ptr() if x is not None else None
     a.w_packed = w_packed.data_ptr()
     a.bias = bias.data_ptr() if bias is not None else None
     a.res = res.data_ptr() if res is not None else None
@@ -321,11 +321,20 @@
             _f32(t)
     if x3h:
         _chk(w_packed, torch.float16, 'w_packed')
-        if mode == MODE_GEMM:
+        if res_conv_in is not None or x_conv_in is not None:
+            if res_conv_in is not None and x_conv_in is not None:
+                raise _lib.VfError('one launch recomputes conv_in as its input or as its residual, not both')
+            img, cwp, cb = res_conv_in or x_conv_in
+            u8, f32 = _image_ptrs(img)
+            name = 'vf_conv3_halo_x3h_res_conv_in' if res_conv_in is not None else 'vf_conv3_halo_x3h_in_conv_in'
+            check(getattr(lib, name)(ctypes.byref(a), u8, f32, _p(_chk(cwp, torch.float16, 'conv_in packing')), _p(_f32(cb)), _stream()), name)
+        elif mode == MODE_GEMM:
             check(lib.vf_gemm_x3h(ctypes.byref(a), _stream()), 'vf_gemm_x3h')
         else:
             check(lib.vf_conv3_halo_x3h(ctypes.byref(a), _stream()), 'vf_conv3_halo_x3h')
         return out
+    if res_conv_in is not None or x_conv_in is not None:
+        raise _lib.VfError('res_conv_in / x_conv_in need the x3h convolution')
     if x6:
         _chk(w_packed, torch.bfloat16, 'w_packed')
         if mode == MODE_GEMM:
@@ -374,14 +383,25 @@
     return H % 8 == 0 and W % 16 == 0 and Cout % 128 == 0
 
 
+def _image_ptrs(img):
+    if img.dtype == torch.uint8:
+        return _p(_chk(img, torch.uint8)), None
+    return None, _p(_f32(img))
+
+
+def conv_in_stats(img, bias, n_img, H, W, Cout, wp3h, gn_part):
+    lib = _lib.load()
+    u8, f32 = _image_ptrs(img)
+    check(lib.vf_conv_in_x3h_stats(u8, f32, _p(_chk(wp3h, torch.float16, 'wp3h')), _p(_f32(bias)), _p(_f32(gn_part)), gn_part.shape[1], n_img, H, W, Cout,
+                                   _stream()), 'vf_conv_in_x3h_stats')
+    return gn_part
+
+
 def conv_in(img, w_oihw, bias, n_img, H, W, Cout, out=None, wp3h=None, gn_part=None):
     lib = _lib.load()
     if out is None:
         out = torch.empty((n_img, H, W, Cout), dtype=torch.float32, device=img.device)
-    if img.dtype == torch.uint8:
-        u8, f32 = _p(_chk(img, torch.uint8)), None
-    else:
-        u8, f32 = None, _p(_f32(img))
+    u8, f32 = _image_ptrs(img)
     if wp3h is not None:
         _chk(wp3h, torch.float16, 'wp3h')
         check(lib.vf_conv_in_x3h(u8, f32, _p(wp3h), _p(bias), _p(out), _p(gn_part) if gn_part is not None else None,
diff --git a/viewformer_amd/vqgan.py b/viewformer_amd/vqgan.py
--- a/viewformer_amd/vqgan.py
+++ b/viewformer_amd/vqgan.py
@@ -159,9 +159,10 @@
                           else None)
         torch.cuda.synchronize(dev)
 
-    def _conv3(self, x, name, n, H, W, mode=ops.MODE_CONV3_S1, pro=None, pro_swish=True, res=None, o16=False):
+    def _conv3(self, x, name, n, H, W, mode=ops.MODE_CONV3_S1, pro=None, pro_swish=True, res=None, o16=False, res_conv_in=None, x_conv_in=None):
         c = self._conv[name]
-        a16 = x.dtype == torch.bfloat16
+        dev = (x if x is not None else x_conv_in[0]).device
+        a16 = x is not None and x.dtype == torch.bfloat16
         if mode == ops.MODE_CONV3_S2PAD:
             Ho, Wo = H // 2, W // 2
         elif mode == ops.MODE_CONV3_UP2:
@@ -172,7 +173,7 @@
             self._stats_of = None
             return ops.conv3_small_cout(x, c.w_raw, c.bias, n, H, W, c.cin, c.cout, pro=pro, pro_swish=pro_swish), Ho, Wo
         o16 = o16 or a16
-        out = torch.empty((n * Ho * Wo, c.cout), dtype=torch.bfloat16 if o16 else torch.float32, device=x.device)
+        out = torch.empty((n * Ho * Wo, c.cout), dtype=torch.bfloat16 if o16 else torch.float32, device=dev)
         bf16 = (c.wp16 is not None and mode in (ops.MODE_CONV3_S1, ops.MODE_CONV3_UP2) and Ho % 8 == 0 and Wo % 16 == 0)
         if o16 and not bf16:
             raise ops._lib.VfError(f'{name}: bf16 activations need the bf16 convolution arm (halo-kernel shape)')
@@ -182,10 +183,10 @@
               and not (mode == ops.MODE_CONV3_S2PAD and pro is not None))
         part = None
         if (bf16 or x6 or x3h) and self.fuse_gn_stats and c.cout in (128, 256, 512, 1024):
-            part = ops.new_gn_part(n, Ho, Wo, x.device)
+            part = ops.new_gn_part(n, Ho, Wo, dev)
         ops.igemm(x, c.wp16 if bf16 else c.wp3h if x3h else c.wp6 if x6 else c.wp, n * Ho * Wo, c.cin, c.cout, out, bias=c.bias, res=res,
                   mode=mode, pro=pro, pro_swish=pro_swish, Hin=H, Win=W, Hout=Ho, Wout=Wo, bf16=bf16, x6=x6, x3h=x3h, gn_part=part,
-                  a16=a16, o16=o16)
+                  a16=a16, o16=o16, **{k: (v[0], v[1].wp3h, v[1].bias) for k, v in (('res_conv_in', res_conv_in), ('x_conv_in', x_conv_in)) if v is not None})
         self._stats_of = (out, part) if part is not None else None
         return out, Ho, Wo
 
@@ -215,15 +216,34 @@
     _stats_of = None
     decoder_act16 = 128
     fuse_gn_stats = True
+    fuse_conv_in = 'res'
     fused_attention = True
 
-    def _res(self, x, name, n, H, W, cin, cout):
-        p1 = self._gn(x, name + '.norm1', n, H * W, cin)
-        h, _, _ = self._conv3(x, name + '.conv1', n, H, W, pro=p1)
+    def _res(self, x, name, n, H, W, cin, cout, conv_in=None):
+        if x is None:
+            img, c = conv_in
+            part = ops.conv_in_stats(img, c.bias, n, H, W, c.cout, c.wp3h, ops.new_gn_part(n, H, W, img.device))
+            gamma, beta = self._norm[name + '.norm1']
+            p1 = ops.groupnorm_finalize(part, gamma, n, H * W, cin, 32, 1e-6) + (beta,)
+            h, _, _ = self._conv3(None, name + '.conv1', n, H, W, pro=p1, x_conv_in=conv_in)
+        else:
+            p1 = self._gn(x, name + '.norm1', n, H * W, cin)
+            h, _, _ = self._conv3(x, name + '.conv1', n, H, W, pro=p1)
         p2 = self._gn(h, name + '.norm2', n, H * W, cout)
+        if conv_in is not None:
+            return self._conv3(h, name + '.conv2', n, H, W, pro=p2, res_conv_in=conv_in)[0]
         sc = x if cin == cout else self._conv1(x, name + '.nin_shortcut', n * H * W)
         out, _, _ = self._conv3(h, name + '.conv2', n, H, W, pro=p2, res=sc)
         return out
+
+    def _conv_in_fusable(self, plan, idx, H, W):
+        if not (self.fuse_conv_in and self.fuse_gn_stats and self.conv_arith == 'x3h' and idx + 1 < len(plan) and plan[idx + 1][0] == 'res'):
+            return False
+        c, (cin, cout) = self._conv[plan[idx][1]], plan[idx + 1][2][:2]
+        name = plan[idx + 1][1]
+        return (c.wp3h is not None and c.cout == 128 and cin == cout == 128 and H % 8 == 0 and W % 16 == 0
+                and self._conv[name + '.conv1'].wp3h is not None and self._conv[name + '.conv2'].wp3h is not None
+                and bool(ops._lib.load().vf_selected(ops._lib.SEL_CONV_X3H_K32)))
 
     def _attn(self, x, name, n, H, W, C):
         HW = H * W
@@ -284,11 +304,16 @@
         return bool(ok)
 
     def _run_plan(self, plan, x, n, H, W, first_is_image=False):
+        conv_in = None
         for idx, (kind, name, args) in enumerate(plan):
             if kind == 'conv3':
                 c = self._conv[name]
                 if c.wp is None:
-                    if c.wp3h is not None and ops.conv_in_x3h_supported(H, W, c.cout):
+                    if self._conv_in_fusable(plan, idx, H, W):
+                        conv_in = (x, c)
+                    if conv_in is not None and self.fuse_conv_in != 'res':
+                        x, self._stats_of = None, None
+                    elif c.wp3h is not None and ops.conv_in_x3h_supported(H, W, c.cout):
                         part = ops.new_gn_part(n, H, W, x.device) if self.fuse_gn_stats and c.cout in (128, 256, 512, 1024) else None
                         x = ops.conv_in(x, c.w_raw, c.bias, n, H, W, c.cout, wp3h=c.wp3h, gn_part=part).view(n * H * W, c.cout)
                         self._stats_of = (x, part) if part is not None else None
@@ -299,7 +324,7 @@
                     x, H, W = self._conv3(x, name, n, H, W, pro=self._pending_pro, pro_swish=True)
                 self._pending_pro = None
             elif kind == 'res':
-                x = self._res(x, name, n, H, W, args[0], args[1])
+                x, conv_in = self._res(x, name, n, H, W, args[0], args[1], conv_in=conv_in), None
             elif kind == 'attn':
                 x = self._attn(x, name, n, H, W, args[0])
             elif kind == 'down':
```

New measurement: 1145. No clear change (-0.1%).
